# manhofer/Line3Dpp

Measured on AMD Instinct MI355X. Metric: M segment-pair scores/sec, higher is better.
Workload: dtype f64

## Files before the change

line3dpp_amd/csrc/k_affinity.hip:

```cpp
#include "l3d_dev.h"
#include "l3d_kernels.h"

namespace l3d {

namespace {

__device__ __forceinline__ float dist_p2l(const HypRec& s, const double* P) {
    const d3 p1{s.P1[0], s.P1[1], s.P1[2]}, dir{s.dir[0], s.dir[1], s.dir[2]}, p{P[0], P[1], P[2]};
    const d3 v = p - p1;
    const d3 h{p1.x + (((dir.x * v.x) * dir.x + (dir.x * v.y) * dir.y) + (dir.x * v.z) * dir.z),
               p1.y + (((dir.y * v.x) * dir.x + (dir.y * v.y) * dir.y) + (dir.y * v.z) * dir.z),
               p1.z + (((dir.z * v.x) * dir.x + (dir.z * v.y) * dir.y) + (dir.z * v.z) * dir.z)};
    return (float)norm(h - p);
}

__device__ __forceinline__ float expf_ref(float y) { return (float)exp((double)y); }

__device__ __forceinline__ float sim_affinity(const HypRec& h1, const HypRec& h2, float k1, float md1, float k2,
                                              float md2, float med_scene_depth_lines, float two_sigA_sqr) {
    if (h1.length < kEps || h2.length < kEps) return 0.0f;
    const float dot_p = (float)dot(d3{h1.dir[0], h1.dir[1], h1.dir[2]}, d3{h2.dir[0], h2.dir[1], h2.dir[2]});
    float angle = (float)(acos((double)fmaxf(fminf(dot_p, 1.0f), -1.0f)) / M_PI * 180.0f);
    if (angle > 90.0f) angle = 180.0f - angle;
    const float y_a = -angle * angle / two_sigA_sqr;
    float cutoff1 = md1, cutoff2 = md2;
    if (med_scene_depth_lines > kEps) {
        cutoff1 = fminf(cutoff1, med_scene_depth_lines);
        cutoff2 = fminf(cutoff2, med_scene_depth_lines);
    }
    const float d11 = dist_p2l(h2, h1.P1), d12 = dist_p2l(h2, h1.P2);
    const float d21 = dist_p2l(h1, h2.P1), d22 = dist_p2l(h1, h2.P2);
    const float sig11 = (h1.m.dp1 > cutoff1) ? cutoff1 * k1 : h1.m.dp1 * k1;
    const float sig12 = (h1.m.dp2 > cutoff1) ? cutoff1 * k1 : h1.m.dp2 * k1;
    const float reg11 = 2.0f * sig11 * sig11, reg12 = 2.0f * sig12 * sig12;
    const float sig21 = (h2.m.dp1 > cutoff2) ? cutoff2 * k2 : h2.m.dp1 * k2;
    const float sig22 = (h2.m.dp2 > cutoff2) ? cutoff2 * k2 : h2.m.dp2 * k2;
    const float reg21 = 2.0f * sig21 * sig21, reg22 = 2.0f * sig22 * sig22;
    const float y_p1 = fminf(-d11 * d11 / reg11, -d12 * d12 / reg12);
    const float y_p2 = fminf(-d21 * d21 / reg21, -d22 * d22 / reg22);
    return expf_ref(fminf(y_a, fminf(y_p1, y_p2)));
}

}

__global__ void k_aff_sim(uint32_t N, uint32_t lo, uint32_t hi, const uint32_t* __restrict__ surv_sg,
                          const uint32_t* __restrict__ surv_tg,
                          const int32_t* __restrict__ hyp_of_seg, const HypRec* __restrict__ hyps,
                          const ViewAff* __restrict__ va, const float* __restrict__ medians,
                          const float* __restrict__ msdl_ptr, float two_sigA_sqr, float* __restrict__ simv,
                          int32_t* __restrict__ cand_a, int32_t* __restrict__ cand_b) {
    const uint32_t c = blockIdx.x * blockDim.x + threadIdx.x;
    if (c >= N) return;
    const int32_t ha = hyp_of_seg[surv_sg[c]], hb = hyp_of_seg[surv_tg[c]];
    cand_a[c] = ha;
    cand_b[c] = hb;
    if (c < lo || c >= hi) return;
    float sim = 0.0f;
    if (ha >= 0 && hb >= 0) {
        const uint32_t v1 = hyps[ha].view, v2 = hyps[hb].view;
        sim = sim_affinity(hyps[ha], hyps[hb], va[v1].k, medians[v1], va[v2].k, medians[v2], *msdl_ptr, two_sigA_sqr);
    }
    simv[c] = sim;
}

__global__ void k_aff_flag(uint32_t N, const uint32_t* __restrict__ surv_off, const uint32_t* __restrict__ surv_sg,
                           const uint32_t* __restrict__ surv_tg, const float* __restrict__ simv,
                           const int32_t* __restrict__ cand_a, const int32_t* __restrict__ cand_b,
                           uint32_t* __restrict__ flag, uint32_t* __restrict__ first_touch, uint32_t H,
                           uint32_t* __restrict__ touch_flag) {
    const uint32_t c = blockIdx.x * blockDim.x + threadIdx.x;
    if (c < H) first_touch[c] = kEmpty;
    if (c < N) { touch_flag[2 * c] = 0; touch_flag[2 * c + 1] = 0; }
    if (c == 0) touch_flag[2 * (size_t)N] = 0;
    if (c >= N) return;
    uint32_t f = 0;
    if (simv[c] > kMinAffinity) {
        f = 1;
        if (cand_b[c] < cand_a[c]) {
            const uint32_t sg = surv_sg[c], tg = surv_tg[c];
            for (uint32_t i = surv_off[tg]; i < surv_off[tg + 1]; ++i) {
                if (surv_tg[i] == sg) {
                    if (simv[i] > kMinAffinity) f = 0;
                    break;
                }
            }
        }
    }
    flag[c] = f;
}

__global__ void k_fill_u32(uint32_t* p, uint32_t n, uint32_t val) {
    const uint32_t i = blockIdx.x * blockDim.x + threadIdx.x;
    if (i < n) p[i] = val;
}

__global__ void k_aff_touch(uint32_t N, const uint32_t* __restrict__ flag, const uint32_t* __restrict__ epos,
                            const int32_t* __restrict__ cand_a, const int32_t* __restrict__ cand_b,
                            uint32_t* __restrict__ first_touch) {
    const uint32_t c = blockIdx.x * blockDim.x + threadIdx.x;
    if (c >= N || !flag[c]) return;
    const uint32_t k = epos[c];
    atomicMin(&first_touch[cand_a[c]], 2u * k);
    atomicMin(&first_touch[cand_b[c]], 2u * k + 1u);
}

__global__ void k_aff_mark(uint32_t H, const uint32_t* __restrict__ first_touch, uint32_t* __restrict__ touch_flag) {
    const uint32_t h = blockIdx.x * blockDim.x + threadIdx.x;
    if (h >= H) return;
    const uint32_t p = first_touch[h];
    if (p != kEmpty) touch_flag[p] = 1u;
}

struct CLEdgeDev { int32_t i, j; float w; };
struct Seg2D { uint32_t cam, seg; };

__global__ void k_aff_emit(uint32_t N, const uint32_t* __restrict__ flag, const uint32_t* __restrict__ epos,
                           const int32_t* __restrict__ cand_a, const int32_t* __restrict__ cand_b,
                           const float* __restrict__ simv, const uint32_t* __restrict__ first_touch,
                           const uint32_t* __restrict__ touch_rank, const HypRec* __restrict__ hyps,
                           CLEdgeDev* __restrict__ edges, Seg2D* __restrict__ local2global) {
    const uint32_t c = blockIdx.x * blockDim.x + threadIdx.x;
    if (c >= N || !flag[c]) return;
    const uint32_t k = epos[c];
    const int32_t ha = cand_a[c], hb = cand_b[c];
    const uint32_t ta = first_touch[ha], tb = first_touch[hb];
    const int32_t id1 = (int32_t)touch_rank[ta], id2 = (int32_t)touch_rank[tb];
    const float w = simv[c];
    edges[2 * k] = CLEdgeDev{id1, id2, w};
    edges[2 * k + 1] = CLEdgeDev{id2, id1, w};
    if (ta == 2u * k) local2global[id1] = Seg2D{hyps[ha].m.src_cam, hyps[ha].m.src_seg};
    if (tb == 2u * k + 1u) local2global[id2] = Seg2D{hyps[hb].m.src_cam, hyps[hb].m.src_seg};
}

__device__ __forceinline__ float dist_p2l_2d(const d3& line, double px, double py) {
    const float den = sqrtf((float)(line.x * line.x + line.y * line.y));
    return (float)fabs(((line.x * px + line.y * py) + line.z) / (double)den);
}
__device__ __forceinline__ bool on_seg_2d(double p1x, double p1y, double p2x, double p2y, double xx, double xy) {
    return ((p1x - xx) * (p2x - xx) + (p1y - xy) * (p2y - xy)) < kEps;
}
template <int PASS>
__global__ __launch_bounds__(256) void k_collin(const ViewDev* __restrict__ views, const uint32_t* __restrict__ seg_base,
                                                float collin_t, uint32_t* __restrict__ cnt,
                                                const uint32_t* __restrict__ coll_off, uint32_t* __restrict__ coll_idx) {
    __shared__ float4 tile[256];
    const ViewDev& v = views[blockIdx.y];
    const uint32_t M = v.M;
    if (blockIdx.x * blockDim.x >= M) return;
    const uint32_t r = blockIdx.x * blockDim.x + threadIdx.x;
    const bool act = r < M;
    const float4 l1 = act ? v.seg4[r] : make_float4(0, 0, 0, 0);
    const d3 p0{(double)l1.x, (double)l1.y, 1.0}, p1{(double)l1.z, (double)l1.w, 1.0};
    const d3 line1 = cross(p0, p1);
    uint32_t n = 0;
    uint32_t* out = (PASS == 1 && act) ? coll_idx + coll_off[seg_base[blockIdx.y] + r] : nullptr;
    for (uint32_t c0 = 0; c0 < M; c0 += 256) {
        __syncthreads();
        if (c0 + threadIdx.x < M) tile[threadIdx.x] = v.seg4[c0 + threadIdx.x];
        __syncthreads();
        const uint32_t ce = min(256u, M - c0);
        if (!act) continue;
        for (uint32_t k = 0; k < ce; ++k) {
            const uint32_t c = c0 + k;
            if (c == r) continue;
            const float4 l2 = tile[k];
            const d3 q0{(double)l2.x, (double)l2.y, 1.0}, q1{(double)l2.z, (double)l2.w, 1.0};
            if (on_seg_2d(p0.x, p0.y, p1.x, p1.y, q0.x, q0.y) || on_seg_2d(p0.x, p0.y, p1.x, p1.y, q1.x, q1.y) ||
                on_seg_2d(q0.x, q0.y, q1.x, q1.y, p0.x, p0.y) || on_seg_2d(q0.x, q0.y, q1.x, q1.y, p1.x, p1.y))
                continue;
            const d3 line2 = cross(q0, q1);
            const float d1 = fmaxf(dist_p2l_2d(line1, q0.x, q0.y), dist_p2l_2d(line1, q1.x, q1.y));
            const float d2 = fmaxf(dist_p2l_2d(line2, p0.x, p0.y), dist_p2l_2d(line2, p1.x, p1.y));
            if (fmaxf(d1, d2) < collin_t) {
                if (PASS == 1) out[n] = c;
                ++n;
            }
        }
    }
    if (PASS == 0 && act) cnt[seg_base[blockIdx.y] + r] = n;
}

template <int MODE>
__global__ void k_aff_coll_count(uint32_t n_items, const uint32_t* __restrict__ surv_tg, const float* __restrict__ simv,
                                 const HypRec* __restrict__ hyps, const uint32_t* __restrict__ seg_base,
                                 const uint32_t* __restrict__ coll_off, uint32_t* __restrict__ cnt) {
    const uint32_t t = blockIdx.x * blockDim.x + threadIdx.x;
    if (t >= n_items) return;
    uint32_t g;
    if (MODE == 0) { if (!(simv[t] > kMinAffinity)) { cnt[t] = 0; return; } g = surv_tg[t]; }
    else g = seg_base[hyps[t].view] + hyps[t].m.src_seg;
    cnt[t] = coll_off[g + 1] - coll_off[g];
}
template <int MODE>
__global__ void k_aff_coll_sim(uint32_t n_items, const uint32_t* __restrict__ surv_sg, const uint32_t* __restrict__ surv_tg,
                               const int32_t* __restrict__ hyp_of_seg, const HypRec* __restrict__ hyps,
                               const ViewDev* __restrict__ views, const uint32_t* __restrict__ seg_base,
                               const uint32_t* __restrict__ gseg_view, const uint32_t* __restrict__ coll_off,
                               const uint32_t* __restrict__ coll_idx, const uint32_t* __restrict__ item_off,
                               const ViewAff* __restrict__ va, const float* __restrict__ medians,
                               const float* __restrict__ msdl_ptr, float two_sigA_sqr, uint32_t* __restrict__ out_seg,
                               float* __restrict__ out_sim) {
    const uint32_t t = blockIdx.x * blockDim.x + threadIdx.x;
    if (t >= n_items) return;
    const uint32_t ob = item_off[t], on = item_off[t + 1] - ob;
    if (!on) return;
    int32_t ha; uint32_t g;
    if (MODE == 0) { ha = hyp_of_seg[surv_sg[t]]; g = surv_tg[t]; }
    else { ha = (int32_t)t; g = seg_base[hyps[t].view] + hyps[t].m.src_seg; }
    const uint32_t vi = gseg_view[g], base = seg_base[vi], cb = coll_off[g];
    for (uint32_t k = 0; k < on; ++k) {
        const uint32_t x = base + coll_idx[cb + k];
        const int32_t hb = hyp_of_seg[x];
        float sim = 0.0f;
        if (ha >= 0 && hb >= 0) {
            const uint32_t v1 = hyps[ha].view, v2 = hyps[hb].view;
            sim = sim_affinity(hyps[ha], hyps[hb], va[v1].k, medians[v1], va[v2].k, medians[v2], *msdl_ptr, two_sigA_sqr);
        }
        out_seg[ob + k] = x;
        out_sim[ob + k] = sim;
    }
}

static inline dim3 grid1(uint32_t n, uint32_t b = 256) { return dim3((n + b - 1) / b); }

hipError_t launch_aff_sim(uint32_t N, uint32_t lo, uint32_t hi, const uint32_t* surv_sg, const uint32_t* surv_tg, const int32_t* hyp_of_seg,
                          const HypRec* hyps, const ViewAff* va, const float* medians, const float* msdl,
                          float two_sigA_sqr, float* simv, int32_t* ca, int32_t* cb, hipStream_t st) {
    if (!N) return hipSuccess;
    hipLaunchKernelGGL(k_aff_sim, grid1(N, 128), dim3(128), 0, st, N, lo, hi, surv_sg, surv_tg, hyp_of_seg, hyps, va, medians,
                       msdl, two_sigA_sqr, simv, ca, cb);
    return hipGetLastError();
}
hipError_t launch_aff_flag(uint32_t N, const uint32_t* surv_off, const uint32_t* surv_sg, const uint32_t* surv_tg,
                           const float* simv, const int32_t* ca, const int32_t* cb, uint32_t* flag,
                           uint32_t* first_touch, uint32_t H, uint32_t* touch_flag, hipStream_t st) {
    if (!N) return hipSuccess;
    hipLaunchKernelGGL(k_aff_flag, grid1(std::max(N, H)), dim3(256), 0, st, N, surv_off, surv_sg, surv_tg, simv, ca, cb,
                       flag, first_touch, H, touch_flag);
    return hipGetLastError();
}
hipError_t launch_fill_u32(uint32_t* p, uint32_t n, uint32_t val, hipStream_t st) {
    if (!n) return hipSuccess;
    hipLaunchKernelGGL(k_fill_u32, grid1(n), dim3(256), 0, st, p, n, val);
    return hipGetLastError();
}
hipError_t launch_aff_touch(uint32_t N, const uint32_t* flag, const uint32_t* epos, const int32_t* ca,
                            const int32_t* cb, uint32_t* first_touch, hipStream_t st) {
    if (!N) return hipSuccess;
    hipLaunchKernelGGL(k_aff_touch, grid1(N), dim3(256), 0, st, N, flag, epos, ca, cb, first_touch);
    return hipGetLastError();
}
hipError_t launch_aff_mark(uint32_t H, const uint32_t* first_touch, uint32_t* touch_flag, hipStream_t st) {
    if (!H) return hipSuccess;
    hipLaunchKernelGGL(k_aff_mark, grid1(H), dim3(256), 0, st, H, first_touch, touch_flag);
    return hipGetLastError();
}
hipError_t launch_aff_emit(uint32_t N, const uint32_t* flag, const uint32_t* epos, const int32_t* ca,
                           const int32_t* cb, const float* simv, const uint32_t* first_touch,
                           const uint32_t* touch_rank, const HypRec* hyps, void* edges, void* local2global,
                           hipStream_t st) {
    if (!N) return hipSuccess;
    hipLaunchKernelGGL(k_aff_emit, grid1(N), dim3(256), 0, st, N, flag, epos, ca, cb, simv, first_touch, touch_rank,
                       hyps, (CLEdgeDev*)edges, (Seg2D*)local2global);
    return hipGetLastError();
}

}

namespace l3d {
hipError_t launch_collin(int pass, const ViewDev* views, uint32_t n_views, uint32_t max_M, const uint32_t* seg_base,
                         float collin_t, uint32_t* cnt, const uint32_t* coll_off, uint32_t* coll_idx, hipStream_t st) {
    if (!n_views || !max_M) return hipSuccess;
    const dim3 g((max_M + 255) / 256, n_views);
    if (pass == 0) hipLaunchKernelGGL((k_collin<0>), g, dim3(256), 0, st, views, seg_base, collin_t, cnt, coll_off, coll_idx);
    else hipLaunchKernelGGL((k_collin<1>), g, dim3(256), 0, st, views, seg_base, collin_t, cnt, coll_off, coll_idx);
    return hipGetLastError();
}
hipError_t launch_aff_coll_count(int mode, uint32_t n_items, const uint32_t* surv_tg, const float* simv,
                                 const HypRec* hyps, const uint32_t* seg_base, const uint32_t* coll_off, uint32_t* cnt,
                                 hipStream_t st) {
    if (!n_items) return hipSuccess;
    const dim3 g((n_items + 255) / 256);
    if (mode == 0) hipLaunchKernelGGL((k_aff_coll_count<0>), g, dim3(256), 0, st, n_items, surv_tg, simv, hyps, seg_base, coll_off, cnt);
    else hipLaunchKernelGGL((k_aff_coll_count<1>), g, dim3(256), 0, st, n_items, surv_tg, simv, hyps, seg_base, coll_off, cnt);
    return hipGetLastError();
}
hipError_t launch_aff_coll_sim(int mode, uint32_t n_items, const uint32_t* surv_sg, const uint32_t* surv_tg,
                               const int32_t* hyp_of_seg, const HypRec* hyps, const ViewDev* views,
                               const uint32_t* seg_base, const uint32_t* gseg_view, const uint32_t* coll_off,
                               const uint32_t* coll_idx, const uint32_t* item_off, const ViewAff* va,
                               const float* medians, const float* msdl, float two_sigA_sqr, uint32_t* out_seg,
                               float* out_sim, hipStream_t st) {
    if (!n_items) return hipSuccess;
    const dim3 g((n_items + 127) / 128);
    if (mode == 0)
        hipLaunchKernelGGL((k_aff_coll_sim<0>), g, dim3(128), 0, st, n_items, surv_sg, surv_tg, hyp_of_seg, hyps, views,
                           seg_base, gseg_view, coll_off, coll_idx, item_off, va, medians, msdl, two_sigA_sqr, out_seg, out_sim);
    else
        hipLaunchKernelGGL((k_aff_coll_sim<1>), g, dim3(128), 0, st, n_items, surv_sg, surv_tg, hyp_of_seg, hyps, views,
                           seg_base, gseg_view, coll_off, coll_idx, item_off, va, medians, msdl, two_sigA_sqr, out_seg, out_sim);
    return hipGetLastError();
}
}


namespace l3d {
namespace { __global__ void k_warm_affinity() {} }
hipError_t warm_affinity(hipStream_t st) {
    hipLaunchKernelGGL(k_warm_affinity, dim3(1), dim3(64), 0, st);
    return hipGetLastError();
}
}
```

line3dpp_amd/csrc/k_lists.hip:

```cpp
#include <algorithm>
#include <cstdlib>
#include <type_traits>

#include "l3d_dev.h"
#include "l3d_kernels.h"
#include "l3d_lists.h"

constexpr uint32_t kLists4Grid = 512;

namespace l3d {

namespace {

#define L3D_LDS __attribute__((address_space(3)))

__device__ __forceinline__ uint32_t lane_id() { return threadIdx.x & 63u; }

template <int WPL>
__device__ __forceinline__ void group_barrier() {
    if (WPL == 1) {
        __builtin_amdgcn_fence(__ATOMIC_RELEASE, "wavefront");
        __builtin_amdgcn_wave_barrier();
        __builtin_amdgcn_fence(__ATOMIC_ACQUIRE, "wavefront");
    } else {
        __syncthreads();
    }
}

template <int WPL>
__device__ __forceinline__ uint32_t group_scan(uint32_t v, uint32_t& total, uint32_t* red);
template <int WPL>
__device__ __forceinline__ uint32_t group_count(bool f, uint32_t& total, uint32_t* red) {
    if (WPL == 1) {
        const uint64_t m = __builtin_amdgcn_ballot_w64(f);
        total = (uint32_t)__popcll(m);
        return (uint32_t)__popcll(m & ((1ull << lane_id()) - 1ull));
    }
    return group_scan<WPL>(f ? 1u : 0u, total, red);
}

template <int WPL>
__device__ __forceinline__ uint32_t group_scan(uint32_t v, uint32_t& total, uint32_t* red) {
    const uint32_t lane = lane_id();
    uint32_t x = v;
#pragma unroll
    for (int d = 1; d < 64; d <<= 1) { const uint32_t y = __shfl_up(x, d); if (lane >= (uint32_t)d) x += y; }
    if (WPL == 1) {
        total = __shfl(x, 63);
        return x - v;
    }
    const uint32_t wave = threadIdx.x >> 6;
    __syncthreads();
    if (lane == 63) red[wave] = x;
    __syncthreads();
    uint32_t before = 0, tot = 0;
#pragma unroll
    for (uint32_t w = 0; w < (uint32_t)WPL; ++w) { const uint32_t c = red[w]; before += w < wave ? c : 0u; tot += c; }
    total = tot;
    return before + x - v;
}

template <int WPL>
__device__ __forceinline__ uint32_t group_max(uint32_t v, uint32_t* red) {
    uint32_t x = v;
#pragma unroll
    for (int d = 32; d > 0; d >>= 1) x = max(x, (uint32_t)__shfl_xor(x, d));
    if (WPL == 1) return x;
    const uint32_t wave = threadIdx.x >> 6;
    __syncthreads();
    if (lane_id() == 0) red[wave] = x;
    __syncthreads();
    uint32_t m = 0;
#pragma unroll
    for (uint32_t w = 0; w < (uint32_t)WPL; ++w) m = max(m, red[w]);
    return m;
}

__device__ __forceinline__ uint32_t f2ord(float f) {
    const uint32_t u = __float_as_uint(f);
    return (u & 0x80000000u) ? ~u : (u | 0x80000000u);
}
__device__ __forceinline__ float ord2f(uint32_t o) {
    return __uint_as_float((o & 0x80000000u) ? (o & 0x7FFFFFFFu) : ~o);
}

__device__ __forceinline__ bool sim_decide(const d3 dira, bool zeroa, float adp1, float adp2, float reg1, float reg2,
                                           const d3 dirb, bool zerob, float bdp1, float bdp2, const SimConst sc) {
    if (zeroa || zerob) return false;
    const float d1 = adp1 - bdp1, d2 = adp2 - bdp2;
// ... 862 lines not shown
                __hip_atomic_store(&positive[h.ref], (uint8_t)1, __ATOMIC_RELAXED, __HIP_MEMORY_SCOPE_AGENT);
                changed[sweep] = 1;
                break;
            }
        }
    }
}

constexpr uint32_t kMaxReplicas = 16;
__global__ void k_hyp_scores(const ListPools lp, const uint8_t* __restrict__ positive,
                             const uint32_t* __restrict__ gseg_view, Slot* __restrict__ slots,
                             const uint8_t* __restrict__ pair_present, uint32_t* __restrict__ max_score_bits) {
    const uint32_t pool = lp.pool0 + blockIdx.y, k = blockIdx.x * blockDim.x + threadIdx.x;
    const bool active = !(lp.flags[0] | lp.flags[2]) && k < min(lp.cnt[pool * 16 + 1], lp.hcap);
    float score3D = 0.0f;
    uint32_t view = kEmpty;
    if (active) {
        HypHdr& h = lp.hyps[pool * lp.hcap + k];
        const bool inv = (h.pair_flags & kHypInv) != 0;
        const bool exists = !inv || positive[h.ref] != 0;
        float cur = 0.0f;
        uint32_t cur_cam = kEmpty;
        if (exists) {
            const uint32_t n = h.edge_cnt, e0 = h.edge_begin;
            for (uint32_t e = 0; e < n; e += 4) {
                EdgeRec ed[4]; bool ok[4];
#pragma unroll
                for (uint32_t i = 0; i < 4; ++i) ed[i] = lp.edges[e0 + min(e + i, n - 1)];
#pragma unroll
                for (uint32_t i = 0; i < 4; ++i) ok[i] = e + i < n && (!(ed[i].j_cam & kEdgeInv) || positive[ed[i].ref_j] != 0);
#pragma unroll
                for (uint32_t i = 0; i < 4; ++i) {
                    if (!ok[i]) continue;
                    if (ed[i].tv_j == cur_cam) {
                        if (ed[i].sim > cur) { score3D -= cur; score3D += ed[i].sim; cur = ed[i].sim; }
                    } else {
                        score3D += ed[i].sim; cur = ed[i].sim; cur_cam = ed[i].tv_j;
                    }
                }
            }
        }
        h.score3D = score3D;
        h.state = exists ? kHypExists : 0u;
        if (exists && !inv && (!pair_present || pair_present[h.pair_flags & 0x7FFFFFFFu])) slots[h.ref].score3D = score3D;
        view = gseg_view[h.g];
    }
    uint64_t todo = __builtin_amdgcn_ballot_w64(score3D > 0.0f);
    while (todo) {
        const uint32_t leader = (uint32_t)__builtin_ctzll(todo);
        const uint32_t lv = __builtin_amdgcn_readlane(view, leader);
        const bool mine = score3D > 0.0f && view == lv;
        float mx = mine ? score3D : 0.0f;
#pragma unroll
        for (int d = 32; d > 0; d >>= 1) mx = fmaxf(mx, __shfl_xor(mx, d));
        if (lane_id() == leader) {
            uint32_t* p = &max_score_bits[lv * kMaxReplicas + (pool & (kMaxReplicas - 1))];
            if (__float_as_uint(mx) > *(volatile uint32_t*)p) atomicMax(p, __float_as_uint(mx));
        }
        todo &= ~__builtin_amdgcn_ballot_w64(mine);
    }
}

__global__ void k_hyp_filter(const ListPools lp, const uint32_t* __restrict__ gseg_view,
                             const uint32_t* __restrict__ max_score_bits, uint32_t* __restrict__ kept_cnt,
                             unsigned long long* __restrict__ best_pack) {
    const uint32_t pool = lp.pool0 + blockIdx.y, k = blockIdx.x * blockDim.x + threadIdx.x;
    if ((lp.flags[0] | lp.flags[2]) || k >= min(lp.cnt[pool * 16 + 1], lp.hcap)) return;
    HypHdr& h = lp.hyps[pool * lp.hcap + k];
    uint32_t mx = 0;
    {
        const uint32_t* p = max_score_bits + (size_t)gseg_view[h.g] * kMaxReplicas;
#pragma unroll
        for (uint32_t r = 0; r < kMaxReplicas; ++r) mx = max(mx, p[r]);
    }
    const float lim = kMinBestScorePerc * __uint_as_float(mx);
    const float s = h.score3D;
    if ((h.state & kHypExists) && s > 0.0f && s > lim) {
        h.state |= kHypKeep;
        atomicAdd(&kept_cnt[h.g], 1u);
        atomicMax(&best_pack[h.g], ((unsigned long long)__float_as_uint(s) << 32) | (0xFFFFFFFFu - h.canon));
    }
}

__global__ void k_seg_filter(uint32_t g0, uint32_t g1, const uint32_t* __restrict__ kept_cnt,
                             const unsigned long long* __restrict__ best_pack, unsigned long long* __restrict__ cnt64) {
    const uint32_t g = g0 + blockIdx.x * blockDim.x + threadIdx.x;
    if (g >= g1) return;
    const bool ok = __uint_as_float((uint32_t)(best_pack[g] >> 32)) > kMinBestScore3D;
    cnt64[g] = ok ? ((1ull << 32) | kept_cnt[g]) : 0ull;
}

__device__ __forceinline__ void make_match(const ViewDev* views, const PairDesc* pairs, uint32_t view, uint32_t seg,
                                           const HypHdr& h, Match& m, uint32_t& tgt_view, uint32_t& tgt_seg) {
    const bool inv = (h.pair_flags & kHypInv) != 0;
    const PairDesc& pd = pairs[h.pair_flags & 0x7FFFFFFFu];
    tgt_view = inv ? pd.src : pd.tgt;
    tgt_seg = h.tgt_seg;
    m.src_cam = views[view].cam; m.src_seg = seg;
    m.tgt_cam = views[tgt_view].cam; m.tgt_seg = tgt_seg;
    m.overlap = h.overlap; m.score3D = h.score3D;
    m.dp1 = h.dp1; m.dp2 = h.dp2;
    m.dq1 = h.oq1; m.dq2 = h.oq2;
}

__global__ void k_seg_write(uint32_t g0, uint32_t g1, unsigned long long base64, const ViewDev* __restrict__ views, const PairDesc* __restrict__ pairs,
                            const uint32_t* __restrict__ seg_base, const uint32_t* __restrict__ gseg_view,
                            const unsigned long long* __restrict__ off64s, const unsigned long long* __restrict__ best_pack,
                            const uint32_t* __restrict__ seg_of_g, const ListPools lp, const Slot* __restrict__ slots,
                            uint32_t* __restrict__ surv_off, uint32_t* __restrict__ hyp_off, Match* __restrict__ surv,
                            uint32_t* __restrict__ surv_tg, uint32_t* __restrict__ surv_sg,
                            int32_t* __restrict__ hyp_of_seg, HypRec* __restrict__ hyps, float* __restrict__ depths) {
    const uint32_t t = blockIdx.x * blockDim.x + threadIdx.x;
    const bool pass_ok = !(lp.flags[0] | lp.flags[2]);
    if (t <= g1 - g0) {
        const uint32_t gs = g0 + t;
        const unsigned long long o = off64s[gs] + base64;
        surv_off[gs] = (uint32_t)o; hyp_off[gs] = (uint32_t)(o >> 32);
        if (gs < g1) hyp_of_seg[gs] = ((off64s[gs + 1] >> 32) != (off64s[gs] >> 32) && pass_ok) ? (int32_t)(uint32_t)(o >> 32) : -1;
    }
    if (!pass_ok) return;
    const uint32_t pq = t / lp.hcap, k = t - pq * lp.hcap, pool = lp.pool0 + pq;
    if (pq >= lp.npools || k >= min(lp.cnt[pool * 16 + 1], lp.hcap)) return;
    const uint32_t hi = pool * lp.hcap + k;
    const HypHdr& h = lp.hyps[hi];
    if (!(h.state & kHypKeep)) return;
    const uint32_t g = h.g;
    if ((off64s[g + 1] >> 32) == (off64s[g] >> 32)) return;
    const unsigned long long o = off64s[g] + base64;
    const uint32_t view = gseg_view[g], seg = g - seg_base[view];
    const SegHdr sh = lp.segs[seg_of_g[g]];
    uint32_t w = (uint32_t)o;
    for (uint32_t y = sh.hyp_begin; y < hi; ++y) w += (lp.hyps[y].state & kHypKeep) ? 1u : 0u;
    Match m; uint32_t tv, tseg;
    make_match(views, pairs, view, seg, h, m, tv, tseg);
    surv_tg[w] = seg_base[tv] + tseg;
    surv_sg[w] = g;
    surv[w] = m;
    if (h.canon == 0xFFFFFFFFu - (uint32_t)best_pack[g]) {
        const uint32_t hx = (uint32_t)(o >> 32);
        const ViewDev& v = views[view];
        HypRec r;
        const SegX& sx = v.segx[seg];
        const Seg3 s3 = unproject(v.C, sx.r1, sx.r2, h.dp1, h.dp2);
        r.P1[0] = s3.P1.x; r.P1[1] = s3.P1.y; r.P1[2] = s3.P1.z;
        r.P2[0] = s3.P2.x; r.P2[1] = s3.P2.y; r.P2[2] = s3.P2.z;
        r.dir[0] = s3.dir.x; r.dir[1] = s3.dir.y; r.dir[2] = s3.dir.z;
        r.length = s3.length;
        r.valid = s3.length > 0.0f ? 1u : 0u;
        r.m = m;
        r.view = view; r.pad = 0;
        hyps[hx] = r;
        depths[2 * hx] = h.dp1;
        depths[2 * hx + 1] = h.dp2;
    }
}

std::atomic<uint64_t> g_csr_global_launches{0};

hipError_t launch_pair_csr(const PairDesc* pairs, uint32_t n_pairs, uint32_t max_Mt, const PairCsr* pair_poff,
                           const uint32_t* inv_tgt, uint32_t tgt16, uint32_t* poff, uint32_t* refs,
                           uint32_t* dummy, uint32_t tgt_v0, uint32_t tgt_v1, uint64_t max_pair_slots,
                           const uint32_t* row_start, hipStream_t st) {
    if (!n_pairs) return hipSuccess;
    const bool force_global = std::getenv("L3D_CSR_GLOBAL") != nullptr;
    const uint32_t lds_segs = force_global ? 0u : kCsrLdsSegs;
    const size_t lds = ((size_t)std::min(max_Mt, lds_segs) + 64) * 4;
    static const hipError_t attr_rc = [] {
        const int mx = (int)(((size_t)kCsrLdsSegs + 64) * 4);
        hipError_t e = hipFuncSetAttribute((const void*)k_pair_csr<true, true, false>, hipFuncAttributeMaxDynamicSharedMemorySize, mx);
        if (e == hipSuccess) e = hipFuncSetAttribute((const void*)k_pair_csr<true, false, false>, hipFuncAttributeMaxDynamicSharedMemorySize, mx);
        return e;
    }();
    if (attr_rc != hipSuccess) return attr_rc;
    if (tgt16 && !force_global && max_Mt <= lds_segs) {
        const size_t cur_bytes = ((size_t)lds_segs_round(max_Mt) + 64) * 4;
        const size_t two = 78 * 1024, one = 156 * 1024 - 4096;
        const size_t want = (size_t)(0.6 * (double)max_pair_slots) * 4 + 4096;
        const size_t budget = cur_bytes + want <= two ? two : one;
        size_t cap = (budget - cur_bytes) / 4;
        cap = std::min<size_t>(cap, (size_t)std::max<uint64_t>(max_pair_slots, 1024));
        static const hipError_t attr2 = hipFuncSetAttribute((const void*)k_pair_csr<true, true, true>, hipFuncAttributeMaxDynamicSharedMemorySize, 156 * 1024);
        if (attr2 != hipSuccess) return attr2;
        hipLaunchKernelGGL((k_pair_csr<true, true, true>), dim3(n_pairs), dim3(kCsrBlock), cur_bytes + cap * 4, st, pairs, 0u, pair_poff, inv_tgt,
                           poff, refs, dummy, tgt_v0, tgt_v1, lds_segs, (uint32_t)cap, row_start);
        return hipGetLastError();
    }
#define L3D_CSR(T16)                                                                                                      \
    do {                                                                                                                  \
        hipLaunchKernelGGL((k_pair_csr<true, T16, false>), dim3(n_pairs), dim3(kCsrBlock), lds, st, pairs, 0u, pair_poff, inv_tgt, \
                           poff, refs, dummy, tgt_v0, tgt_v1, lds_segs, 0u, row_start);                                   \
        if (max_Mt > lds_segs) {  \
            hipLaunchKernelGGL((k_pair_csr<false, T16, false>), dim3(n_pairs), dim3(kCsrBlock), 0, st, pairs, 0u, pair_poff, inv_tgt, \
                               poff, refs, dummy, tgt_v0, tgt_v1, lds_segs, 0u, row_start);                               \
            g_csr_global_launches.fetch_add(1, std::memory_order_relaxed);                                                \
        }                                                                                                                 \
    } while (0)
    if (tgt16) L3D_CSR(true); else L3D_CSR(false);
// ... 4 lines not shown
__global__ void k_publish_flags(const ListPools lp) {
    if (threadIdx.x < 4) lp.cnt[lp.pool0 * 16 + 8 + threadIdx.x] = lp.flags[threadIdx.x];
    if (threadIdx.x == 4) lp.cnt[lp.pool0 * 16 + 12] = lp.flags[6];
}

__global__ void k_merge_flags(const ListPools lp, uint32_t world) {
    const uint32_t ppr = kListPools / world;
    uint32_t f0 = 0, f2 = 0;
    for (uint32_t r = 0; r < world; ++r) { f0 |= lp.cnt[(size_t)r * ppr * 16 + 8]; f2 |= lp.cnt[(size_t)r * ppr * 16 + 10]; }
    if (f0) lp.flags[0] = 1;
    if (f2) lp.flags[2] = 1;
}

__global__ void k_seg_index(const ListPools lp, uint32_t* __restrict__ seg_of_g) {
    if (lp.flags[0] | lp.flags[2]) return;
    const uint32_t pool = lp.pool0 + blockIdx.y, k = blockIdx.x * blockDim.x + threadIdx.x;
    if (k >= min(lp.cnt[pool * 16 + 2], lp.scap)) return;
    seg_of_g[lp.segs[pool * lp.scap + k].g] = pool * lp.scap + k;
}
hipError_t launch_seg_index(ListPools lp, uint32_t* seg_of_g, uint32_t G, uint32_t world, hipStream_t st) {
    hipLaunchKernelGGL(k_merge_flags, dim3(1), dim3(1), 0, st, lp, world ? world : 1u);
    hipLaunchKernelGGL(k_seg_index, dim3((lp.scap + 255) / 256, lp.npools), dim3(256), 0, st, lp, seg_of_g);
    return hipGetLastError();
}

constexpr uint32_t kLists2Grid = 16384;
hipError_t launch_lists(uint32_t v0, uint32_t nv, uint32_t max_M, const ViewDev* views, const PairDesc* pairs,
                        const ListView* lviews, const OutPair* opairs, const InPair* ipairs, const uint32_t* gseg_view,
                        const uint32_t* poff, const uint32_t* inv, const float2* hyp_p, const float2* hyp_q, const Slot* slots, uint32_t uniform_K,
                        SimConst sc, ListPools lp, uint32_t* seg_of_g, HugeScratchArgs hsa, hipStream_t st) {
    if (!nv || !max_M) return hipSuccess;
    const bool wide = hsa.mean_list > 96;
#define L3D_LISTS(B)                                                                                                       \
    do {                                                                                                                   \
        const size_t lds1 = ListCfg<1, B>::BYTES, lds2 = ListCfg<2, B>::BYTES, lds4 = ListCfg<4, B>::BYTES;                \
        hipError_t e = hipFuncSetAttribute((const void*)k_lists<1, B>, hipFuncAttributeMaxDynamicSharedMemorySize, (int)lds1); \
        if (e != hipSuccess) return e;                                                                                     \
        e = hipFuncSetAttribute((const void*)k_lists<2, B>, hipFuncAttributeMaxDynamicSharedMemorySize, (int)lds2);        \
        if (e != hipSuccess) return e;                                                                                     \
        e = hipFuncSetAttribute((const void*)k_lists<4, B>, hipFuncAttributeMaxDynamicSharedMemorySize, (int)lds4);        \
        if (e != hipSuccess) return e;                                                                                     \
        for (uint32_t a = 0; a < nv; a += 65535u) {                                                      \
            const uint32_t n = nv - a < 65535u ? nv - a : 65535u;                                                          \
            hipLaunchKernelGGL((k_lists<1, B>), dim3(max_M, n), dim3(64), lds1, st, views, pairs, lviews, opairs, ipairs,  \
                               gseg_view, poff, inv, hyp_p, hyp_q, uniform_K, lp, v0 + a);                                        \
        }                                                                                                                  \
           \
        hipLaunchKernelGGL((k_lists<2, B>), dim3(kLists2Grid), dim3(128), lds2, st, views, pairs, lviews, opairs, ipairs, \
                           gseg_view, poff, inv, hyp_p, hyp_q, uniform_K, lp, 0u);                                                \
            \
            \
        if (hsa.run_tier4)                                                                                                 \
        hipLaunchKernelGGL((k_lists<4, B>), dim3(kLists4Grid), dim3(256), lds4, st, views, pairs, lviews, opairs, ipairs, \
                           gseg_view, poff, inv, hyp_p, hyp_q, uniform_K, lp, 0u);                                                \
    } while (0)
    if (wide) L3D_LISTS(256); else L3D_LISTS(128);
#undef L3D_LISTS
    HugeScratch hs;
    hs.d1 = hsa.f32; hs.d2 = hsa.f32 + hsa.cap;
    hs.tv = hsa.u32; hs.ref = hsa.u32 + hsa.cap; hs.pf = hsa.u32 + 2 * (size_t)hsa.cap;
    hs.key = hsa.u64; hs.cap = hsa.cap;
    if (hsa.run_huge)
        hipLaunchKernelGGL(k_lists_huge, dim3(256), dim3(256), 0, st, views, pairs, lviews, opairs, ipairs, gseg_view, poff,
                           inv, hyp_p, hyp_q, lp, hs);
    hipLaunchKernelGGL(k_cand_exact, dim3((lp.ccap + 255) / 256, lp.npools), dim3(256), 0, st, views, pairs, gseg_view, sc, lp);
    hipLaunchKernelGGL(k_edges, dim3((lp.scap + kEdgesSplit - 1) / kEdgesSplit, lp.npools), dim3(64), 0, st, views, pairs,
                       gseg_view, slots, lp, seg_of_g);
    if (lp.npools < kListPools) hipLaunchKernelGGL(k_publish_flags, dim3(1), dim3(64), 0, st, lp);
    return hipGetLastError();
}

static dim3 hyp_grid(const ListPools& lp) { return dim3((lp.hcap + 255) / 256, lp.npools); }

hipError_t launch_chain_sweep(ListPools lp, uint8_t* positive, uint32_t* changed, uint32_t sweep, uint32_t* undecided, hipStream_t st) {
    if (sweep == 0) hipLaunchKernelGGL(k_chain_sweep, hyp_grid(lp), dim3(256), 0, st, lp, positive, changed, undecided);
    else hipLaunchKernelGGL(k_chain_sweep_list, dim3(kChainListBlocks, lp.npools), dim3(256), 0, st, lp, positive, changed, sweep, undecided);
    return hipGetLastError();
}
hipError_t launch_hyp_scores(ListPools lp, const uint8_t* positive, const uint32_t* gseg_view, Slot* slots,
                             const uint8_t* pair_present, uint32_t* max_score_bits, hipStream_t st) {
    hipLaunchKernelGGL(k_hyp_scores, hyp_grid(lp), dim3(256), 0, st, lp, positive, gseg_view, slots, pair_present, max_score_bits);
    return hipGetLastError();
}
hipError_t launch_hyp_filter(ListPools lp, uint32_t g0, uint32_t g1, const uint32_t* gseg_view, const uint32_t* max_score_bits,
                             uint32_t* kept_cnt, unsigned long long* best_pack, unsigned long long* cnt64,
                             hipStream_t st) {
    hipLaunchKernelGGL(k_hyp_filter, hyp_grid(lp), dim3(256), 0, st, lp, gseg_view, max_score_bits, kept_cnt, best_pack);
    if (g1 > g0) hipLaunchKernelGGL(k_seg_filter, dim3((g1 - g0 + 255) / 256), dim3(256), 0, st, g0, g1, kept_cnt, best_pack, cnt64);
    return hipGetLastError();
}
hipError_t launch_seg_write(uint32_t g0, uint32_t g1, unsigned long long base64, const ViewDev* views, const PairDesc* pairs, const uint32_t* seg_base,
                            const uint32_t* gseg_view, const unsigned long long* off64s,
                            const unsigned long long* best_pack, const uint32_t* seg_of_g, ListPools lp,
                            const Slot* slots, uint32_t* surv_off, uint32_t* hyp_off, Match* surv, uint32_t* surv_tg,
                            uint32_t* surv_sg, int32_t* hyp_of_seg, HypRec* hyps, float* depths, hipStream_t st) {
    const uint64_t n_thr = std::max<uint64_t>((uint64_t)(g1 - g0) + 1, (uint64_t)lp.npools * lp.hcap);
    hipLaunchKernelGGL(k_seg_write, dim3((uint32_t)((n_thr + 255) / 256)), dim3(256), 0, st, g0, g1, base64, views, pairs, seg_base, gseg_view,
                       off64s, best_pack, seg_of_g, lp, slots, surv_off, hyp_off, surv, surv_tg, surv_sg, hyp_of_seg,
                       hyps, depths);
    return hipGetLastError();
}

}


namespace l3d {
namespace { __global__ void k_warm_lists() {} }
hipError_t warm_lists(hipStream_t st) {
    hipLaunchKernelGGL(k_warm_lists, dim3(1), dim3(64), 0, st);
    return hipGetLastError();
}
}
```

line3dpp_amd/csrc/k_scan.hip:

```cpp
#include "l3d_dev.h"
#include "l3d_kernels.h"

namespace l3d {

namespace {

constexpr uint32_t kScanBlock = 1024, kScanItems = 4, kScanTile = kScanBlock * kScanItems;
constexpr unsigned long long kAgg = 1ull << 32, kIncl = 2ull << 32;

template <class T>
__device__ __forceinline__ T block_exclusive_scan(T v, T* wsum , T& block_total) {
    const uint32_t tid = threadIdx.x, lane = tid & 63u, wave = tid >> 6;
    T x = v;
#pragma unroll
    for (int d = 1; d < 64; d <<= 1) {
        const T y = __shfl_up(x, d);
        if (lane >= (uint32_t)d) x += y;
    }
    if (lane == 63) wsum[wave] = x;
    __syncthreads();
    if (tid == 0) {
        T acc = 0;
        for (uint32_t w = 0; w < kScanBlock / 64; ++w) { const T t = wsum[w]; wsum[w] = acc; acc += t; }
        wsum[16] = acc;
    }
    __syncthreads();
    block_total = wsum[16];
    return wsum[wave] + x - v;
}

__device__ __forceinline__ uint32_t wave_sum(uint32_t v) {
#pragma unroll
    for (int d = 32; d > 0; d >>= 1) v += __shfl_xor(v, d);
    return v;
}

template <class T>
__global__ __launch_bounds__(kScanBlock) void k_scan(const T* __restrict__ in, uint32_t n, T* __restrict__ out,
                                                     T* __restrict__ total_out, unsigned long long* __restrict__ ws) {
    constexpr uint32_t LANES = sizeof(T) / 4;
    __shared__ T wsum[17];
    __shared__ T s_prefix;
    __shared__ uint32_t s_last, s_tile;
    const uint32_t nb = gridDim.x, tid = threadIdx.x, lane = tid & 63u;
    if (tid == 0) s_tile = (uint32_t)__hip_atomic_fetch_add(&ws[1], 1ull, __ATOMIC_RELAXED, __HIP_MEMORY_SCOPE_AGENT);
    __syncthreads();
    const uint32_t tile = s_tile;
    const uint32_t base = tile * kScanTile + tid * kScanItems;
    T a[kScanItems];
    T v = 0;
#pragma unroll
    for (uint32_t k = 0; k < kScanItems; ++k) { a[k] = (base + k < n) ? in[base + k] : (T)0; v += a[k]; }
    T agg;
    T ex = block_exclusive_scan(v, wsum, agg);
    unsigned long long* state = ws + 2;
    if (tid < 64) {
        if (lane < LANES)
            __hip_atomic_store(&state[(size_t)tile * LANES + lane],
                               (tile == 0 ? kIncl : kAgg) | (uint32_t)((unsigned long long)agg >> (32 * lane)),
                               __ATOMIC_RELAXED, __HIP_MEMORY_SCOPE_AGENT);
        unsigned long long prefix = 0;
        if (tile > 0) {
#pragma unroll
            for (uint32_t l = 0; l < LANES; ++l) {
                uint32_t acc = 0;
                for (int idx = (int)tile - 1;; idx -= 64) {
                    const int t = idx - (int)lane;
                    unsigned long long s = kIncl;
                    if (t >= 0) {
                        do s = __hip_atomic_load(&state[(size_t)t * LANES + l], __ATOMIC_RELAXED, __HIP_MEMORY_SCOPE_AGENT);
                        while ((s >> 32) == 0);
                    }
                    const uint64_t incl = __builtin_amdgcn_ballot_w64((s >> 32) == 2);
                    if (incl) {
                        const uint32_t first = (uint32_t)__builtin_ctzll(incl);
                        acc += wave_sum(lane <= first ? (uint32_t)s : 0u);
                        break;
                    }
                    acc += wave_sum((uint32_t)s);
                }
                prefix |= (unsigned long long)acc << (32 * l);
            }
            if (lane < LANES)
                __hip_atomic_store(&state[(size_t)tile * LANES + lane],
                                   kIncl | (uint32_t)((prefix + (unsigned long long)agg) >> (32 * lane)),
                                   __ATOMIC_RELAXED, __HIP_MEMORY_SCOPE_AGENT);
        }
        if (lane == 0) s_prefix = (T)prefix;
    }
    __syncthreads();
    ex += s_prefix;
#pragma unroll
    for (uint32_t k = 0; k < kScanItems; ++k) {
        if (base + k < n) out[base + k] = ex;
        ex += a[k];
    }
    if (tile == nb - 1 && tid == 0) {
        const T total = s_prefix + agg;
        out[n] = total;
        if (total_out) *total_out = total;
    }
    __syncthreads();
    if (tid == 0) s_last = __hip_atomic_fetch_add(&ws[0], 1ull, __ATOMIC_ACQ_REL, __HIP_MEMORY_SCOPE_AGENT) == nb - 1;
    __syncthreads();
    if (s_last) {
        for (uint32_t i = tid; i < nb * LANES; i += kScanBlock)
            __hip_atomic_store(&state[i], 0ull, __ATOMIC_RELAXED, __HIP_MEMORY_SCOPE_AGENT);
        if (tid == 0) {
            __hip_atomic_store(&ws[0], 0ull, __ATOMIC_RELAXED, __HIP_MEMORY_SCOPE_AGENT);
            __hip_atomic_store(&ws[1], 0ull, __ATOMIC_RELAXED, __HIP_MEMORY_SCOPE_AGENT);
        }
    }
}

template <class T>
hipError_t launch(const T* in, uint32_t n, T* out, unsigned long long* ws, T* total, hipStream_t st) {
    const uint32_t nb = std::max(1u, (n + kScanTile - 1) / kScanTile);
    hipLaunchKernelGGL((k_scan<T>), dim3(nb), dim3(kScanBlock), 0, st, in, n, out, total, ws);
    return hipGetLastError();
}

}

size_t scan_ws_words(size_t n, uint32_t bytes_per_element) { return 4 + (n / kScanTile + 1) * (bytes_per_element / 4); }

hipError_t launch_scan(const uint32_t* in, uint32_t n, uint32_t* out, unsigned long long* ws, uint32_t* total, hipStream_t st) {
    return launch<uint32_t>(in, n, out, ws, total, st);
}
hipError_t launch_scan64(const unsigned long long* in, uint32_t n, unsigned long long* out, unsigned long long* ws,
                         unsigned long long* total, hipStream_t st) {
    return launch<unsigned long long>(in, n, out, ws, total, st);
}

}


namespace l3d {
namespace { __global__ void k_warm_scan() {} }
hipError_t warm_scan(hipStream_t st) {
    hipLaunchKernelGGL(k_warm_scan, dim3(1), dim3(64), 0, st);
    return hipGetLastError();
}
}
```

line3dpp_amd/csrc/l3d_access.hip:

```cpp
#include "l3d_ctx.h"
#include "l3d_lsd.h"

using namespace l3d;

extern "C" {

int l3d_synchronize(l3d_ctx* c) {
    if (!c) return fail(L3D_ERR_ARG, "null argument");
    L3D_HIP_CHECK(hipStreamSynchronize(c->stream));
    return L3D_OK;
}

int l3d_pair_tests(l3d_ctx* c, uint64_t* n) {
    if (!c || !n) return fail(L3D_ERR_ARG, "null argument");
    *n = c->pair_tests;
    return L3D_OK;
}

static int fetch_host_offsets(l3d_ctx* c) {
    if (c->host_offsets_valid) return L3D_OK;
    c->h_surv_off.assign((size_t)c->G + 1, 0);
    c->h_hyp_off.assign((size_t)c->G + 1, 0);
    L3D_HIP_CHECK(hipStreamSynchronize(c->stream));
    L3D_HIP_CHECK(hipMemcpy(c->h_surv_off.data(), c->d_surv_off.p, ((size_t)c->G + 1) * 4, hipMemcpyDeviceToHost));
// ... 52 lines not shown

int l3d_num_best(l3d_ctx* c, uint32_t* n) {
    if (!c || !n) return fail(L3D_ERR_ARG, "null argument");
    *n = c->state == l3d_ctx::MATCHED ? c->n_hyps : 0;
    return L3D_OK;
}

int l3d_get_best(l3d_ctx* c, l3d_segment2d* seg2d, l3d_segment3d* seg3d, l3d_match* best) {
    if (!c) return fail(L3D_ERR_ARG, "null argument");
    if (c->state != l3d_ctx::MATCHED) return fail(L3D_ERR_STATE, "no matches yet");
    (void)hipSetDevice(c->device);
    std::vector<HypRec> h(c->n_hyps);
    if (c->n_hyps) L3D_HIP_CHECK(hipMemcpy(h.data(), c->d_hyps.p, h.size() * sizeof(HypRec), hipMemcpyDeviceToHost));
    for (size_t i = 0; i < h.size(); ++i) {
        if (seg2d) { seg2d[i].camID_ = h[i].m.src_cam; seg2d[i].segID_ = h[i].m.src_seg; }
        if (seg3d) {
            std::memcpy(seg3d[i].P1, h[i].P1, 24); std::memcpy(seg3d[i].P2, h[i].P2, 24);
            std::memcpy(seg3d[i].dir, h[i].dir, 24);
            seg3d[i].length_ = h[i].length; seg3d[i].valid_ = h[i].valid;
        }
        if (best) std::memcpy(&best[i], &h[i].m, sizeof(l3d_match));
    }
    return L3D_OK;
}

int l3d_view_info(l3d_ctx* c, uint32_t camID, float* k, float* median_depth) {
    if (!c) return fail(L3D_ERR_ARG, "null argument");
    auto f = c->views.find(camID);
    if (f == c->views.end()) return fail(L3D_ERR_ARG, "unknown camera ID");
    if (k) *k = f->second->k;
    if (median_depth) *median_depth = f->second->median_depth;
    return L3D_OK;
}

int l3d_translation(l3d_ctx* c, double t[3]) {
    if (!c || !t) return fail(L3D_ERR_ARG, "null argument");
    t[0] = c->translation.x; t[1] = c->translation.y; t[2] = c->translation.z;
    return L3D_OK;
}

int l3d_num_affinity(l3d_ctx* c, uint32_t* n_edges, uint32_t* n_rows) {
    if (!c) return fail(L3D_ERR_ARG, "null argument");
    if (!c->affinity_done) return fail(L3D_ERR_STATE, "l3d_compute_affinity has not run");
    if (n_edges) *n_edges = c->aff_n_edges;
    if (n_rows) *n_rows = c->aff_n_rows;
    return L3D_OK;
}

int l3d_get_affinity(l3d_ctx* c, l3d_cledge* edges, l3d_segment2d* l2g, float* msdl) {
    if (!c) return fail(L3D_ERR_ARG, "null argument");
    if (!c->affinity_done) return fail(L3D_ERR_STATE, "l3d_compute_affinity has not run");
    { std::lock_guard<std::recursive_mutex> lk(c->mu); const int rc = ensure_affinity_host(c); if (rc) return rc; }
    if (edges && !c->edges.empty()) std::memcpy(edges, c->edges.data(), c->edges.size() * sizeof(l3d_cledge));
    if (l2g && !c->l2g.empty()) std::memcpy(l2g, c->l2g.data(), c->l2g.size() * sizeof(l3d_segment2d));
    if (msdl) *msdl = c->med_scene_depth_lines;
    return L3D_OK;
}

int l3d_get_sparse_matrix(l3d_ctx* c, int sort_by_row, l3d_float4* entries, int32_t* start_indices) {
    if (!c) return fail(L3D_ERR_ARG, "null argument");
    if (!c->affinity_done) return fail(L3D_ERR_STATE, "l3d_compute_affinity has not run");
    { std::lock_guard<std::recursive_mutex> lk(c->mu); const int rc = ensure_affinity_host(c); if (rc) return rc; }
    std::vector<l3d_cledge> e = c->edges;
    if (sort_by_row)
        std::stable_sort(e.begin(), e.end(), [](const l3d_cledge& a, const l3d_cledge& b) {
            return a.i_ < b.i_ || (a.i_ == b.i_ && a.j_ < b.j_); });
    else
        std::stable_sort(e.begin(), e.end(), [](const l3d_cledge& a, const l3d_cledge& b) {
            return a.j_ < b.j_ || (a.j_ == b.j_ && a.i_ < b.i_); });
    if (start_indices) for (size_t i = 0; i < c->l2g.size(); ++i) start_indices[i] = -1;
    int cur = -1;
    for (size_t pos = 0; pos < e.size(); ++pos) {
        if (entries) entries[pos] = l3d_float4{(float)e[pos].i_, (float)e[pos].j_, e[pos].w_, 0.0f};
        const int rc = sort_by_row ? e[pos].i_ : e[pos].j_;
        if (rc != cur) { if (start_indices) start_indices[rc] = (int)pos; cur = rc; }
    }
    return L3D_OK;
}

unsigned long long l3d_debug_counter(const char* name) {
    if (name && std::string(name) == "csr_global_launches") return g_csr_global_launches.load(std::memory_order_relaxed);
    if (name && std::string(name) == "knn_replay_calls") return g_knn_replay_calls.load(std::memory_order_relaxed);
    if (name && std::string(name) == "keep_all_repeats") return g_keep_all_repeats.load(std::memory_order_relaxed);
    if (name && std::string(name) == "lsd_images_detected") return g_lsd_images_detected.load(std::memory_order_relaxed);
    if (name && std::string(name) == "lsd_cache_loads") return g_lsd_cache_loads.load(std::memory_order_relaxed);
    return ~0ull;
}

int l3d_set_timing_level(l3d_ctx* c, int level) {
    if (!c || level < 0 || level > 2) return fail(L3D_ERR_ARG, "l3d_set_timing_level: level 0, 1 or 2");
    std::lock_guard<std::recursive_mutex> lk(c->mu);
    c->timing_level = level;
    return L3D_OK;
}

int l3d_get_timings(l3d_ctx* c, l3d_timings* t) {
    if (!c || !t) return fail(L3D_ERR_ARG, "null argument");
    *t = c->tm;
    return L3D_OK;
}

}
```

line3dpp_amd/csrc/l3d_affinity_host.hip:

```cpp
#include "l3d_ctx.h"

namespace l3d {

static int affinity_collinear(l3d_ctx* c) {
    hipStream_t st = c->stream;
    const uint32_t V = (uint32_t)c->order.size(), G = c->G, N = c->n_surv, H = c->n_hyps;
    uint32_t max_M = 0;
    for (auto* v : c->order) max_M = std::max(max_M, v->M);
    L3D_HIP_CHECK(c->d_coll_cnt.reserve(G + 1)); L3D_HIP_CHECK(c->d_coll_off.reserve(G + 1));
    L3D_HIP_CHECK(launch_collin(0, c->d_views.p, V, max_M, c->d_seg_base.p, c->collinearity_t, c->d_coll_cnt.p, nullptr,
                                nullptr, st));
    L3D_HIP_CHECK(launch_scan(c->d_coll_cnt.p, G, c->d_coll_off.p, c->d_scan_ws.p, c->d_scal.p + 9, st));
    uint32_t n_coll = 0;
    L3D_HIP_CHECK(hipStreamSynchronize(st));
    L3D_HIP_CHECK(hipMemcpy(&n_coll, c->d_scal.p + 9, 4, hipMemcpyDeviceToHost));
    L3D_HIP_CHECK(c->d_coll_idx.reserve(std::max<uint32_t>(n_coll, 1)));
    L3D_HIP_CHECK(launch_collin(1, c->d_views.p, V, max_M, c->d_seg_base.p, c->collinearity_t, nullptr, c->d_coll_off.p,
                                c->d_coll_idx.p, st));
    std::vector<uint32_t> off[2], seg[2];
    std::vector<float> sim[2];
    const uint32_t n_items[2] = {N, H};
    for (int mode = 0; mode < 2; ++mode) {
        const uint32_t n = n_items[mode];
        L3D_HIP_CHECK(c->d_item_cnt.reserve(n + 1)); L3D_HIP_CHECK(c->d_item_off.reserve(n + 1));
// ... 30 lines not shown
    for (uint32_t g = 0; g < G; ++g) if (hyp_of_seg[g] >= 0) seg_of_hyp[(uint32_t)hyp_of_seg[g]] = g;
    std::unordered_set<uint64_t> used;
    std::vector<int32_t> local_id(G, -1);
    std::vector<uint32_t> row_seg;
    auto unused = [&](uint32_t a, uint32_t b) {
        const uint64_t key = a < b ? ((uint64_t)a << 32) | b : ((uint64_t)b << 32) | a;
        return used.insert(key).second;
    };
    auto get_id = [&](uint32_t g) {
        if (local_id[g] < 0) { local_id[g] = (int32_t)row_seg.size(); row_seg.push_back(g); }
        return local_id[g];
    };
    c->edges.clear();
    auto push = [&](int32_t i, int32_t j, float w) {
        c->edges.push_back(l3d_cledge{i, j, w}); c->edges.push_back(l3d_cledge{j, i, w});
    };
    for (uint32_t h = 0; h < H; ++h) {
        const uint32_t a = seg_of_hyp[h];
        if (a == kEmpty) continue;
        int32_t id1 = -1;
        bool found_aff = false;
        for (uint32_t p = surv_off[a]; p < surv_off[a + 1]; ++p) {
            const uint32_t b = surv_tg[p];
            if (simv[p] > kMinAffinity && unused(a, b)) {
                if (id1 < 0) id1 = get_id(a);
                const int32_t id2 = get_id(b);
                push(id1, id2, simv[p]);
                found_aff = true;
                for (uint32_t k = off[0][p]; k < off[0][p + 1]; ++k)
                    if (sim[0][k] > kMinAffinity && unused(a, seg[0][k])) push(id1, get_id(seg[0][k]), sim[0][k]);
            }
        }
        if (found_aff && id1 >= 0)
            for (uint32_t k = off[1][h]; k < off[1][h + 1]; ++k)
                if (sim[1][k] > kMinAffinity && unused(a, seg[1][k])) push(id1, get_id(seg[1][k]), sim[1][k]);
    }
    c->l2g.resize(row_seg.size());
    for (size_t r = 0; r < row_seg.size(); ++r) {
        const uint32_t g = row_seg[r];
        const uint32_t vi = (uint32_t)(std::upper_bound(c->seg_base.begin(), c->seg_base.end(), g) - c->seg_base.begin()) - 1;
        c->l2g[r].camID_ = c->order[vi]->cam; c->l2g[r].segID_ = g - c->seg_base[vi];
    }
    c->aff_n_edges = (uint32_t)c->edges.size(); c->aff_n_rows = (uint32_t)c->l2g.size(); c->aff_host_valid = true;
    L3D_HIP_CHECK(c->d_edges.reserve(std::max<size_t>(c->edges.size(), 1)));
    if (!c->edges.empty())
        L3D_HIP_CHECK(hipMemcpyAsync(c->d_edges.p, c->edges.data(), c->edges.size() * sizeof(l3d_cledge),
                                     hipMemcpyHostToDevice, st));
    return L3D_OK;
}

static int affinity_prepare(l3d_ctx* c) {
    (void)hipSetDevice(c->device);
    hipStream_t st = c->stream;
    const uint32_t V = (uint32_t)c->order.size();
    c->edges.clear(); c->l2g.clear();
    c->aff_n_edges = 0; c->aff_n_rows = 0; c->aff_host_valid = true;
    std::vector<float> sd;
    for (auto* v : c->order) if (v->median_depth > kEps) sd.push_back(v->median_depth);
    if (!sd.empty()) { std::sort(sd.begin(), sd.end()); c->med_scene_depth_lines = sd[sd.size() / 2]; }
    else c->med_scene_depth_lines = 0.0f;
    std::vector<ViewAff> va(V + 1);
    for (uint32_t vi = 0; vi < V; ++vi) { va[vi].k = c->order[vi]->k; va[vi].pad = 0; }
    va[V].k = c->med_scene_depth_lines; va[V].pad = 0;
    const uint32_t N = c->n_surv, H = c->n_hyps;
    L3D_HIP_CHECK(c->d_scal.reserve(16));
    L3D_HIP_CHECK(c->d_scan_ws.reserve_zeroed(scan_ws_words((size_t)c->G + 2 * (size_t)N, 4), st));
    if (c->ev_on(6)) L3D_HIP_CHECK(hipEventRecord(c->ev[6], st));
    if (N > 0 && H > 0) {
        L3D_HIP_CHECK(c->d_vaff.reserve(V + 1));
        L3D_HIP_CHECK(c->d_simv.reserve(N)); L3D_HIP_CHECK(c->d_ca.reserve(N)); L3D_HIP_CHECK(c->d_cb.reserve(N));
        L3D_HIP_CHECK(c->d_flag.reserve(N + 1)); L3D_HIP_CHECK(c->d_epos.reserve(N + 1));
        L3D_HIP_CHECK(c->d_first_touch.reserve(H));
        L3D_HIP_CHECK(c->d_scan_ws.reserve_zeroed(scan_ws_words(2 * (size_t)N, 4), st));
        L3D_HIP_CHECK(upload_table(c->d_vaff, c->h_vaff, va.data(), ((size_t)V + 1) * sizeof(ViewAff), c->up_vaff, st));
    }
    return L3D_OK;
}

static int affinity_sim(l3d_ctx* c, uint32_t lo, uint32_t hi) {
    const uint32_t V = (uint32_t)c->order.size(), N = c->n_surv, H = c->n_hyps;
    if (!(N > 0 && H > 0)) return L3D_OK;
    L3D_HIP_CHECK(launch_aff_sim(N, lo, hi, c->d_surv_sg.p, c->d_surv_tg.p, c->d_hyp_of_seg.p, c->d_hyps.p, c->d_vaff.p,
                                 (c->d_med + 8), (const float*)(c->d_vaff.p + V), c->two_sigA_sqr, c->d_simv.p, c->d_ca.p, c->d_cb.p,
                                 c->stream));
    return L3D_OK;
}

static int affinity_rest(l3d_ctx* c) {
    hipStream_t st = c->stream;
    const uint32_t N = c->n_surv, H = c->n_hyps;
    bool counts_pending = false;
    if (N > 0 && H > 0) {
        if (c->collinearity_t > (float)kEps) {
            const int rc = affinity_collinear(c);
            if (rc) return rc;
            if (c->ev_on(7)) L3D_HIP_CHECK(hipEventRecord(c->ev[7], st));
            L3D_HIP_CHECK(hipStreamSynchronize(st));
            c->tm.affinity_ms = ev_ms(c, 6, 7);
            c->affinity_done = true;
            return L3D_OK;
        }
        L3D_HIP_CHECK(c->d_touch_flag.reserve(2 * (size_t)N + 1));
        L3D_HIP_CHECK(launch_aff_flag(N, c->d_surv_off.p, c->d_surv_sg.p, c->d_surv_tg.p, c->d_simv.p, c->d_ca.p,
                                      c->d_cb.p, c->d_flag.p, c->d_first_touch.p, H, c->d_touch_flag.p, st));
        L3D_HIP_CHECK(launch_scan(c->d_flag.p, N, c->d_epos.p, c->d_scan_ws.p, c->d_scal.p + 3, st));
        {
            L3D_HIP_CHECK(c->d_touch_flag.reserve(2 * (size_t)N + 1));
            L3D_HIP_CHECK(c->d_touch_rank.reserve(2 * (size_t)N + 1));
            L3D_HIP_CHECK(c->d_edges.reserve(2 * (size_t)N));
            L3D_HIP_CHECK(c->d_l2g.reserve(H));
            L3D_HIP_CHECK(launch_aff_touch(N, c->d_flag.p, c->d_epos.p, c->d_ca.p, c->d_cb.p, c->d_first_touch.p, st));
            L3D_HIP_CHECK(launch_aff_mark(H, c->d_first_touch.p, c->d_touch_flag.p, st));
            L3D_HIP_CHECK(launch_scan(c->d_touch_flag.p, 2 * N, c->d_touch_rank.p, c->d_scan_ws.p, c->d_scal.p + 4, st));
            L3D_HIP_CHECK(launch_aff_emit(N, c->d_flag.p, c->d_epos.p, c->d_ca.p, c->d_cb.p, c->d_simv.p,
                                          c->d_first_touch.p, c->d_touch_rank.p, c->d_hyps.p, c->d_edges.p,
                                          c->d_l2g.p, st));
            L3D_HIP_CHECK(c->h_cnt.reserve(16));
            L3D_HIP_CHECK(hipMemcpyAsync(c->h_cnt.p + 12, c->d_scal.p + 3, 8, hipMemcpyDeviceToHost, st));
            counts_pending = true;
        }
    }
    if (c->ev_on(7)) L3D_HIP_CHECK(hipEventRecord(c->ev[7], st));
    L3D_HIP_CHECK(hipStreamSynchronize(st));
    if (counts_pending) { c->aff_n_edges = 2 * c->h_cnt.p[12]; c->aff_n_rows = c->h_cnt.p[13]; c->aff_host_valid = false; }
    c->tm.affinity_ms = ev_ms(c, 6, 7);
    c->affinity_done = true;
    return L3D_OK;
}

int affinity_core(l3d_ctx* c) {
    int rc = affinity_prepare(c);
    if (rc == L3D_OK) rc = affinity_sim(c, 0u, c->n_surv);
    if (rc == L3D_OK) rc = affinity_rest(c);
    return rc;
}

int ensure_affinity_host(l3d_ctx* c) {
    if (c->aff_host_valid) return L3D_OK;
    (void)hipSetDevice(c->device);
    c->edges.resize(c->aff_n_edges);
    c->l2g.resize(c->aff_n_rows);
    L3D_HIP_CHECK(hipStreamSynchronize(c->stream));
    if (c->aff_n_edges)
        L3D_HIP_CHECK(hipMemcpy(c->edges.data(), c->d_edges.p, (size_t)c->aff_n_edges * sizeof(l3d_cledge), hipMemcpyDeviceToHost));
    if (c->aff_n_rows)
        L3D_HIP_CHECK(hipMemcpy(c->l2g.data(), c->d_l2g.p, (size_t)c->aff_n_rows * sizeof(l3d_segment2d), hipMemcpyDeviceToHost));
    c->aff_host_valid = true;
    return L3D_OK;
}

}

using namespace l3d;

extern "C" {

int l3d_compute_affinity(l3d_ctx* c) {
    if (!c) return fail(L3D_ERR_ARG, "null argument");
    std::lock_guard<std::recursive_mutex> lk(c->mu);
    if (c->state != l3d_ctx::MATCHED) return fail(L3D_ERR_STATE, "matchImages must precede the affinity step");
    if (c->aff_shard_open) return fail(L3D_ERR_STATE, "a sharded affinity fill is open: l3d_affinity_shard_finish (or _abort) first");
    translate(*c);
    const int rc = affinity_core(c);
    untranslate(*c);
    return rc;
}

int l3d_affinity_shard_begin(l3d_ctx* c, uint32_t rank, uint32_t world, void** simv, uint64_t* first, uint64_t* count) {
    if (!c || !simv || !first || !count) return fail(L3D_ERR_ARG, "null argument");
    std::lock_guard<std::recursive_mutex> lk(c->mu);
    if (c->state != l3d_ctx::MATCHED) return fail(L3D_ERR_STATE, "matchImages must precede the affinity step");
    if (c->aff_shard_open) return fail(L3D_ERR_STATE, "l3d_affinity_shard_begin: a sharded affinity fill is already open (views translated)");
    if (world < 2 || rank >= world || c->aff_parts_world != world || c->tail_base_n.size() != (size_t)world + 1 ||
        c->tail_base_n[world] != c->n_surv)
        return fail(L3D_ERR_STATE, "l3d_affinity_shard_begin follows a call closed by l3d_tail_shard_commit with the same world size");
    if (c->collinearity_t > (float)kEps)
        return fail(L3D_ERR_LIMIT, "the links to collinear segments are sequential by definition (line3D.cc:1904-1974): use l3d_compute_affinity");
    translate(*c);
    int rc = affinity_prepare(c);
    if (rc == L3D_OK) rc = affinity_sim(c, c->tail_base_n[rank], c->tail_base_n[rank + 1]);
    if (rc == L3D_OK && !c->exch_ordered && hipStreamSynchronize(c->stream) != hipSuccess) rc = fail(L3D_ERR_HIP, "l3d_affinity_shard_begin: stream synchronisation failed");
    if (rc != L3D_OK) { untranslate(*c); return rc; }
    *simv = c->d_simv.p;
    for (uint32_t r = 0; r < world; ++r) { first[r] = c->tail_base_n[r]; count[r] = c->tail_base_n[r + 1] - c->tail_base_n[r]; }
    c->aff_shard_open = true;
    return L3D_OK;
}

int l3d_affinity_shard_finish(l3d_ctx* c) {
    if (!c) return fail(L3D_ERR_ARG, "null argument");
    std::lock_guard<std::recursive_mutex> lk(c->mu);
    if (c->state != l3d_ctx::MATCHED || !c->aff_shard_open)
        return fail(L3D_ERR_STATE, "l3d_affinity_shard_finish follows l3d_affinity_shard_begin and the exchange of the similarities");
    c->aff_shard_open = false;
    const int rc = affinity_rest(c);
    untranslate(*c);
    return rc;
}

int l3d_affinity_shard_abort(l3d_ctx* c) {
    if (!c) return fail(L3D_ERR_ARG, "null argument");
    std::lock_guard<std::recursive_mutex> lk(c->mu);
    if (!c->aff_shard_open) return L3D_OK;
// ... 67 lines not shown
```

line3dpp_amd/csrc/l3d_api.hip:

```cpp
#include <thread>

#include "l3d_ctx.h"

namespace l3d {

static thread_local std::string g_err;
void set_error(const std::string& s) { g_err = s; }
const char* last_error_cstr() { return g_err.c_str(); }

int fail(int code, const std::string& msg) { set_error(msg); return code; }

void init_view(HostView& v, const double K[9], const double R[9], const double t[3]) {
    std::memcpy(v.K.m, K, 72);
    std::memcpy(v.R.m, R, 72);
    v.t = d3{t[0], t[1], t[2]};
    v.pp = d3{v.K.m[2], v.K.m[5], 1.0};
    v.Kinv = m3_inv(v.K);
    v.Rt = m3_t(v.R);
    v.RtKinv = m3_mul(v.Rt, v.Kinv);
    v.C = mul33(v.Rt.m, d3{-1.0 * v.t.x, -1.0 * v.t.y, -1.0 * v.t.z});
}

void translate_view(HostView& v, const d3& d) {
    v.C = v.C + d;
// ... 170 lines not shown
struct CachedBlock { void* p; size_t bytes; int device; bool pinned; };
std::mutex g_cache_mu;
std::vector<CachedBlock> g_cache;
size_t g_cache_bytes[2] = {0, 0};
constexpr size_t kCacheMaxBlocks = 512;
constexpr size_t kCacheMaxPinned = (size_t)1 << 30;
thread_local int g_release_synced = 0;
size_t cache_max_device_bytes() {
    static const size_t cap = [] {
        if (const char* e = std::getenv("L3D_CACHE_MAX_MB")) return (size_t)std::strtoull(e, nullptr, 10) << 20;
        size_t fr = 0, tot = 0;
        if (hipMemGetInfo(&fr, &tot) != hipSuccess || !tot) { (void)hipGetLastError(); return (size_t)16 << 30; }
        return tot / 4;
    }();
    return cap;
}
}
ReleaseSynced::ReleaseSynced() { ++g_release_synced; }
ReleaseSynced::~ReleaseSynced() { --g_release_synced; }
void* block_cache_take(bool pinned, size_t bytes, size_t* got_bytes) {
    if (!bytes) return nullptr;
    int dev = 0;
    (void)hipGetDevice(&dev);
    std::lock_guard<std::mutex> lk(g_cache_mu);
    size_t best = g_cache.size();
    for (size_t i = 0; i < g_cache.size(); ++i) {
        const CachedBlock& b = g_cache[i];
        if (b.pinned != pinned || (!pinned && b.device != dev) || b.bytes < bytes || b.bytes > 2 * bytes + (64u << 10)) continue;
        if (best == g_cache.size() || b.bytes < g_cache[best].bytes) best = i;
    }
    if (best == g_cache.size()) return nullptr;
    const CachedBlock b = g_cache[best];
    g_cache[best] = g_cache.back(); g_cache.pop_back();
    g_cache_bytes[pinned] -= b.bytes;
    *got_bytes = b.bytes;
    return b.p;
}
bool block_cache_give(bool pinned, void* p, size_t bytes) {
    static const bool off = std::getenv("L3D_NO_BLOCK_CACHE") != nullptr;
    if (off || !p || !bytes) return false;
    int dev = 0;
    (void)hipGetDevice(&dev);
    const size_t cap = pinned ? kCacheMaxPinned : cache_max_device_bytes();
    {
        std::lock_guard<std::mutex> lk(g_cache_mu);
        if (g_cache.size() >= kCacheMaxBlocks || g_cache_bytes[pinned] + bytes > cap) return false;
    }
    if (!g_release_synced && hipDeviceSynchronize() != hipSuccess) { (void)hipGetLastError(); return false; }
    std::lock_guard<std::mutex> lk(g_cache_mu);
    if (g_cache.size() >= kCacheMaxBlocks || g_cache_bytes[pinned] + bytes > cap) return false;
    g_cache.push_back(CachedBlock{p, bytes, dev, pinned});
    g_cache_bytes[pinned] += bytes;
    return true;
}
size_t block_cache_trim(int kind) {
    std::vector<CachedBlock> out;
    {
        std::lock_guard<std::mutex> lk(g_cache_mu);
        for (size_t i = 0; i < g_cache.size();) {
            if (kind < 0 || (int)g_cache[i].pinned == kind) {
                out.push_back(g_cache[i]); g_cache_bytes[g_cache[i].pinned] -= g_cache[i].bytes;
                g_cache[i] = g_cache.back(); g_cache.pop_back();
            } else ++i;
        }
    }
    size_t freed = 0;
    int cur = 0;
    (void)hipGetDevice(&cur);
    for (const CachedBlock& b : out) {
        if (b.pinned) (void)hipHostFree(b.p);
        else { (void)hipSetDevice(b.device); (void)hipFree(b.p); }
        freed += b.bytes;
    }
    if (!out.empty()) (void)hipSetDevice(cur);
    return freed;
}

float ev_ms(hipEvent_t a, hipEvent_t b) {
    float ms = 0;
    (void)hipEventElapsedTime(&ms, a, b);
    return ms;
}
std::atomic<uint64_t> g_keep_all_repeats{0};
std::atomic<uint64_t> g_knn_replay_calls{0};

float ev_ms(const ::l3d_ctx* c, int a, int b) { return c->ev_on(a) && c->ev_on(b) ? ev_ms(c->ev[a], c->ev[b]) : 0.0f; }

}

using namespace l3d;

extern "C" {

const char* l3d_last_error(void) { return g_err.c_str(); }
#ifndef L3D_BUILD_ID
#define L3D_BUILD_ID "unknown"
#endif
const char* l3d_build_info(void) { return "libl3dpp_hip gfx950 hip fp-contract=off build=" L3D_BUILD_ID; }

uint64_t l3d_trim_cache(void) { return (uint64_t)block_cache_trim(-1); }

l3d_ctx* l3d_create(int device, void* stream) {
    if (hipSetDevice(device) != hipSuccess) { set_error("hipSetDevice failed: no usable HIP device"); return nullptr; }
    auto* c = new l3d_ctx();
    c->device = device;
    c->stream = (hipStream_t)stream;
    orientation_thresholds(c->orient_lo, c->orient_hi);
    c->use_cull = std::getenv("L3D_NO_CULL") == nullptr;
    for (auto& e : c->ev)
        if (hipEventCreate(&e) != hipSuccess) { set_error("hipEventCreate failed"); delete c; return nullptr; }
    static std::mutex warm_mu;
    static std::set<int> warmed;
    bool need_warm = !std::getenv("L3D_NO_WARMUP");
    if (need_warm) { std::lock_guard<std::mutex> lk(warm_mu); need_warm = warmed.count(device) == 0; }
    if (need_warm) {
        hipStream_t st = c->stream;
        DevBuf<uint32_t> d; PinnedBuf<uint32_t> h;
        constexpr size_t kWarmWords = (1u << 20) / 4;
        bool ok = d.reserve(kWarmWords) == hipSuccess && h.reserve(kWarmWords) == hipSuccess;
        ok = ok && hipMemsetAsync(d.p, 0, kWarmWords * 4, st) == hipSuccess;
        const size_t sizes[] = {64, 1024, 4096, 16384, 65536, 262144, (size_t)1 << 20};
        for (size_t bytes : sizes) {
            ok = ok && hipMemcpyAsync(d.p, h.p, bytes, hipMemcpyHostToDevice, st) == hipSuccess && hipStreamSynchronize(st) == hipSuccess;
            ok = ok && hipMemcpyAsync(h.p, d.p, bytes, hipMemcpyDeviceToHost, st) == hipSuccess && hipStreamSynchronize(st) == hipSuccess;
        }
        for (int rep = 0; rep < 2; ++rep)
            for (size_t bytes : sizes) {
                ok = ok && hipMemsetAsync(d.p, 0, kWarmWords * 4, st) == hipSuccess;
                ok = ok && hipMemcpyAsync(h.p, d.p, bytes, hipMemcpyDeviceToHost, st) == hipSuccess;
                ok = ok && hipMemsetAsync(d.p, 0, kWarmWords * 4, st) == hipSuccess;
                ok = ok && hipMemcpyAsync(d.p, h.p, bytes, hipMemcpyHostToDevice, st) == hipSuccess;
            }
        ok = ok && warm_match(st) == hipSuccess && warm_lists(st) == hipSuccess && warm_scan(st) == hipSuccess &&
             warm_views(st) == hipSuccess && warm_affinity(st) == hipSuccess && warm_rdd(st) == hipSuccess;
        const bool drained_ok = hipStreamSynchronize(st) == hipSuccess;
        ok = ok && drained_ok;
        { const ReleaseSynced drained; d.release(); h.release(); }
        if (!ok) { set_error("start-up launches failed: no usable HIP device"); l3d_destroy(c); return nullptr; }
        { std::lock_guard<std::mutex> lk(warm_mu); warmed.insert(device); }
    }
    return c;
}

void l3d_destroy(l3d_ctx* c) {
    if (!c) return;
    (void)hipSetDevice(c->device);
    (void)hipStreamSynchronize(c->stream);
    const ReleaseSynced drained;
    for (auto& kv : c->views) {
        HostView& v = *kv.second;
        v.d_seg4.release(); v.d_segf.release();
    }
    c->d_views.release(); c->d_pairs.release(); c->d_work.release(); c->d_slots.release(); c->d_slot_idx.release();
    c->h_views.release(); c->h_pairs.release(); c->h_cull.release(); c->h_work.release();
    c->h_segb.release(); c->h_cnt.release(); c->h_fin.release();
    c->d_poff.release(); c->d_csr_dummy.release(); c->d_pair_present.release(); c->d_cnt64.release(); c->d_off64s.release(); c->d_scan_ws.release();
    c->d_huge_u64.release(); c->d_inv_refs.release(); c->d_lzero.release(); c->d_list2.release(); c->d_list4.release(); c->d_listH.release();
    c->d_seg_of_g.release(); c->d_huge_u32.release(); c->d_huge_f32.release(); c->d_ledges.release(); c->d_lhyps.release();
    c->d_lsegs.release(); c->d_lcands.release(); c->d_lchdrs.release(); c->d_ltab.release(); c->h_ltab.release();
    c->d_cull.release(); c->d_src_perm.release(); c->d_tgt_perm.release(); c->d_src_band.release();
    c->d_chunk_band.release(); c->d_cull_keys.release(); c->d_tgt_sf.release(); c->d_tgt_band.release(); c->d_tgt_s4.release(); c->d_tgt_sd.release();
    c->d_row_counts.release(); c->d_keep_rec.release(); c->d_row_start.release(); c->d_slot_row.release(); c->d_keep_info.release(); c->d_row_pair.release(); c->d_blk_row.release(); c->h_keep_info.release();
    c->d_seg_base.release(); c->d_gseg_view.release();
    c->d_scal.release();
    c->d_surv_off.release(); c->d_hyp_off.release();
    c->d_surv_tg.release(); c->d_surv_sg.release();
    c->d_inv_tgt.release(); c->d_hyp_p.release(); c->d_hyp_q.release(); c->d_gsegx.release(); c->d_gsegd32.release();
    c->d_tie_count.release(); c->d_tie_list.release(); c->d_tie_heap.release(); c->d_item_bucket.release(); c->d_item_order.release(); c->d_order_done.release();
    c->d_coll_cnt.release(); c->d_coll_off.release(); c->d_coll_idx.release(); c->d_item_cnt.release();
    c->d_item_off.release(); c->d_item_seg.release(); c->d_item_sim.release();
    c->d_surv.release();
    c->d_hyp_of_seg.release(); c->d_depths.release(); c->d_med = nullptr; c->d_hyps.release();
    c->d_vaff.release(); c->d_simv.release(); c->h_vaff.release(); c->d_ca.release(); c->d_cb.release();
    c->d_flag.release(); c->d_epos.release(); c->d_first_touch.release(); c->d_touch_flag.release();
    c->d_touch_rank.release(); c->d_edges.release(); c->d_l2g.release();
    c->d_lopt.release(); c->h_lopt.release();
    for (auto& e : c->ev) if (e) (void)hipEventDestroy(e);
    for (auto& e : c->lo_ev) if (e) (void)hipEventDestroy(e);
    delete c;
}

int l3d_slots_exchanged(l3d_ctx* c) {
    if (!c) return fail(L3D_ERR_ARG, "null argument");
    if (c->state != l3d_ctx::BEGUN) return fail(L3D_ERR_STATE, "l3d_match_begin must precede l3d_slots_exchanged");
    std::fill(c->pair_done.begin(), c->pair_done.end(), 1);
    return L3D_OK;
}

int l3d_set_brute_force(l3d_ctx* c, int on) {
    if (!c) return L3D_ERR_ARG;
    c->brute = on != 0;
    return L3D_OK;
}

static int add_view(l3d_ctx* c, uint32_t camID, const float* segs4, uint32_t M, const double K[9], const double R[9],
                    const double t[3], uint32_t width, uint32_t height, float median_depth, const uint32_t* neighbors,
                    uint32_t n_neighbors, bool by_worldpoints);

int l3d_add_view(l3d_ctx* c, uint32_t camID, const float* segs4, uint32_t M, const double K[9], const double R[9],
                 const double t[3], uint32_t width, uint32_t height, float median_depth, const uint32_t* neighbors,
                 uint32_t n_neighbors) {
    return add_view(c, camID, segs4, M, K, R, t, width, height, median_depth, neighbors, n_neighbors, false);
}
int l3d_add_view_worldpoints(l3d_ctx* c, uint32_t camID, const float* segs4, uint32_t M, const double K[9],
                             const double R[9], const double t[3], uint32_t width, uint32_t height, float median_depth,
                             const uint32_t* worldpoints, uint32_t n_worldpoints) {
    return add_view(c, camID, segs4, M, K, R, t, width, height, median_depth, worldpoints, n_worldpoints, true);
}
int l3d_get_visual_neighbors(l3d_ctx* c, uint32_t camID, uint32_t* out, uint32_t cap, uint32_t* n) {
    if (!c || !n) return fail(L3D_ERR_ARG, "null argument");
    std::lock_guard<std::recursive_mutex> lk(c->mu);
    auto it = c->views.find(camID);
    if (it == c->views.end()) return fail(L3D_ERR_ARG, "unknown camera ID");
    *n = (uint32_t)it->second->visual_nbrs.size();
    uint32_t i = 0;
    if (out) for (uint32_t o : it->second->visual_nbrs) { if (i < cap) out[i] = o; ++i; }
    return L3D_OK;
}

static int add_view(l3d_ctx* c, uint32_t camID, const float* segs4, uint32_t M, const double K[9], const double R[9],
                    const double t[3], uint32_t width, uint32_t height, float median_depth, const uint32_t* neighbors,
                    uint32_t n_neighbors, bool by_worldpoints) {
    if (!c || !K || !R || !t) return fail(L3D_ERR_ARG, "null argument");
    std::lock_guard<std::recursive_mutex> lk(c->mu);
    if (std::max(width, height) < 800) return fail(L3D_ERR_IMAGE_SMALL, "image is too small for reliable results");
    if (c->views.count(camID)) return fail(L3D_ERR_ID_IN_USE, "camera ID already in use");
    if (n_neighbors == 0 || !neighbors)
        return fail(L3D_ERR_NO_NEIGHBORS, by_worldpoints ? "view has no worldpoints" : "view has no visual neighbors");
    if (M == 0 || !segs4) return fail(L3D_ERR_NO_SEGMENTS, "no line segments");
    if (M >= (1u << 23)) return fail(L3D_ERR_LIMIT, "more than 2^23 segments per view");
    (void)hipSetDevice(c->device);
    auto v = std::make_unique<HostView>();
    v->cam = camID; v->M = M;
    v->segs.assign(segs4, segs4 + 4 * (size_t)M);
    for (float x : v->segs) v->coord_max = std::isfinite(x) ? std::fmax(v->coord_max, (double)std::fabs(x)) : INFINITY;
    v->width = width; v->height = height;
    v->initial_median_depth = (float)std::fmax(std::fabs(median_depth), kEps);
    init_view(*v, K, R, t);
    if (by_worldpoints) { v->by_worldpoints = true; v->worldpoints.assign(neighbors, neighbors + n_neighbors); }
    else v->fixed_nbrs.assign(neighbors, neighbors + n_neighbors);
    L3D_HIP_CHECK(v->d_seg4.reserve(M));
    L3D_HIP_CHECK(v->d_segf.reserve(M));
    L3D_HIP_CHECK(hipMemcpy(v->d_seg4.p, v->segs.data(), (size_t)M * 16, hipMemcpyHostToDevice));
    c->views_avg_depths.push_back((float)std::fmax(median_depth, kEps));
    c->views[camID] = std::move(v);
    c->order.clear();
    for (auto& kv : c->views) { kv.second->index = (uint32_t)c->order.size(); c->order.push_back(kv.second.get()); }
    c->state = l3d_ctx::IDLE;
    c->affinity_done = false;
    return L3D_OK;
}

void abort_match(l3d_ctx* c) {
    (void)hipStreamSynchronize(c->stream);
    untranslate(*c);
    c->timing_pending = false; c->pending_launches = 0;
    c->state = l3d_ctx::IDLE;
// ... 232 lines not shown
    }
    L3D_HIP_CHECK(c->d_tgt_band.reserve(std::max<uint64_t>(ct_off, 1)));
    L3D_HIP_CHECK(c->d_chunk_band.reserve(std::max<uint32_t>(cc_off, 1)));
    L3D_HIP_CHECK(c->d_cull_keys.reserve(std::max<uint64_t>(ck_off, 1)));
    if (c->ev_on(1)) L3D_HIP_CHECK(hipEventRecord(c->ev[1], c->stream));
    g_trace.mark("begin: tables uploaded, pools reserved");
    c->tm = l3d_timings{};
    c->state = l3d_ctx::BEGUN;
    return L3D_OK;
}

int l3d_num_pairs(l3d_ctx* c, uint32_t* n) {
    if (!c || !n) return fail(L3D_ERR_ARG, "null argument");
    *n = (uint32_t)c->pairs.size();
    return L3D_OK;
}

int l3d_get_pairs(l3d_ctx* c, uint32_t* s, uint32_t* t, uint64_t* off) {
    if (!c) return fail(L3D_ERR_ARG, "null argument");
    for (size_t i = 0; i < c->pairs.size(); ++i) {
        if (s) s[i] = c->pair_src_cam[i];
        if (t) t[i] = c->pair_tgt_cam[i];
        if (off) off[i] = c->pairs[i].slot_off;
    }
    return L3D_OK;
}

void collect_match_timing(l3d_ctx* c) {
    if (!c->timing_pending) return;
    c->tm.match_kernel_ms += ev_ms(c, 4, 5);
    c->tm.cull_prepare_ms += ev_ms(c, 8, 4);
    c->tm.match_kernel_launches += c->pending_launches;
    c->timing_pending = false; c->pending_launches = 0;
}

static int run_match_kernel(l3d_ctx* c, int mode, uint32_t first, uint32_t count) {
    size_t n_work = 0;
    uint32_t maxK = 0, maxM = 0, maxMt = 0;
    const bool hot = mode == 0 && !c->brute && !c->knn_replay;
    const uint32_t tile = hot ? c->tile_rows : 0u;
    const uint32_t layout = hot ? c->layout_rows : 0u;
    const uint32_t rows_per_item = layout ? layout : (uint32_t)kMatchRows;
    auto items_of = [&](uint32_t Ms) { return layout ? tile_src_cap(Ms, layout) / layout : (Ms + kMatchRows - 1) / kMatchRows; };
    for (uint32_t p = first; p < first + count; ++p) n_work += items_of(c->pairs[p].Ms);
    if (!n_work) return L3D_OK;
    for (uint32_t p = first; p < first + count; ++p) {
        const PairDesc& pd = c->pairs[p];
        maxK = std::max(maxK, pd.K);
        if (c->cull[p].enabled) maxM = std::max(maxM, std::max(pd.Ms, pd.Mt));
        maxMt = std::max(maxMt, pd.Mt);
    }
    const bool replay_all = mode == 0 && c->knn_replay;
    if (!replay_all && match_lds_bytes(mode, maxK, false, match_waves_per_group(mode, c->brute, (uint32_t)n_work), c->brute, tile,
                                       match_row_cache(mode, c->brute, (uint32_t)n_work, tile)) > 160 * 1024)
        return fail(L3D_ERR_LIMIT, "kNN too large for the LDS top-K table");
    L3D_HIP_CHECK(c->d_work.reserve(n_work));
    if (!(c->work_key.version == c->pairs_version && c->work_key.first == first && c->work_key.count == count &&
          c->work_key.dev == (const void*)c->d_work.p && c->work_key.rows == rows_per_item && c->work_key.items == n_work)) {
        L3D_HIP_CHECK(c->h_work.reserve(n_work));
        WorkItem* work = c->h_work.p;
        size_t w = 0;
        for (uint32_t p = first; p < first + count; ++p)
            for (uint32_t k = 0, n = items_of(c->pairs[p].Ms); k < n; ++k) work[w++] = WorkItem{p, k * rows_per_item};
        L3D_HIP_CHECK(hipMemcpyAsync(c->d_work.p, work, n_work * sizeof(WorkItem), hipMemcpyHostToDevice, c->stream));
        c->work_key.version = c->pairs_version; c->work_key.first = first; c->work_key.count = count;
        c->work_key.dev = c->d_work.p; c->work_key.rows = rows_per_item; c->work_key.items = n_work;
    }
    if (c->ev_on(8)) L3D_HIP_CHECK(hipEventRecord(c->ev[8], c->stream));
    CullPools pools{c->d_cull.p, c->d_src_perm.p, c->d_src_band.p, c->d_tgt_perm.p, c->d_tgt_sf.p, c->d_tgt_band.p,
                    c->d_chunk_band.p, c->d_cull_keys.p};
    pools.tgt_s4 = c->d_tgt_s4.p; pools.tgt_sd = c->d_tgt_sd.p; pools.padded_rows = layout;
    const bool keep_all_unculled = std::getenv("L3D_KEEPALL_NO_CULL") != nullptr;
    if (c->brute || !maxM || mode == 2 || (mode == 1 && keep_all_unculled)) pools.cull = nullptr;
    else {
        if (!tile && !replay_all && n_work > kMatchOrderMinItems && n_work <= kMatchOrderMaxItems) {
            L3D_HIP_CHECK(c->d_item_bucket.reserve(n_work)); L3D_HIP_CHECK(c->d_item_order.reserve(n_work));
            if (!c->d_order_done.p) {
                L3D_HIP_CHECK(c->d_order_done.reserve(1));
                L3D_HIP_CHECK(hipMemsetAsync(c->d_order_done.p, 0, 4, c->stream));
            }
            pools.item_bucket = c->d_item_bucket.p; pools.item_order = c->d_item_order.p;
            pools.order_done = c->d_order_done.p;
            pools.w_base = c->cull[first].w_item0; pools.cost_max = maxMt;
        }
        L3D_HIP_CHECK(launch_cull_prepare(c->d_views.p, c->d_pairs.p, first, count, maxM, pools, layout, c->stream));
        L3D_HIP_CHECK(launch_order_items(c->d_pairs.p, first, count, maxMt, pools, (uint32_t)n_work, c->stream));
    }
    if (c->ev_on(4)) L3D_HIP_CHECK(hipEventRecord(c->ev[4], c->stream));
    const bool ix16 = maxMt < 65536u && maxK < 32768u;
    OrientFuse of{mode == 0 ? c->d_inv_tgt.p : nullptr, c->tgt16, OrientThr{c->orient_lo, c->orient_hi}, nullptr, nullptr, 0u, nullptr, nullptr,
                  mode == 0 ? c->d_hyp_p.p : nullptr, mode == 0 ? c->d_hyp_q.p : nullptr};
    if (mode == 1 && c->ragged) { of.keep_rec = c->d_keep_rec.p; of.keep_cap = c->keep_cap; }
    uint32_t tie_stride = 0;
    if (mode == 0) {
        uint32_t mt = 0;
        for (auto& pd : c->pairs) mt = std::max(mt, pd.Mt);
        tie_stride = std::max(mt, 1u);
        if (!c->d_tie_count.p) {
            L3D_HIP_CHECK(c->d_tie_count.reserve(4));
            L3D_HIP_CHECK(hipMemsetAsync(c->d_tie_count.p, 0, 16, c->stream));
        }
        L3D_HIP_CHECK(c->d_tie_list.reserve(std::max<uint32_t>(c->n_rows_total, 1)));
        L3D_HIP_CHECK(c->d_tie_heap.reserve(2 * (size_t)match_tied_grid(tie_stride) * tie_stride));
        of.tie_count = c->d_tie_count.p + (c->tie_seq & 1u); of.tie_next = c->d_tie_count.p + ((c->tie_seq + 1) & 1u);
        of.tie_total = c->d_tie_count.p + 2; ++c->tie_seq;
        of.tie_list = c->d_tie_list.p; of.tie_cap = c->n_rows_total;
    }
    if (replay_all) {
        uint32_t maxMs = 0;
        for (uint32_t p = first; p < first + count; ++p) maxMs = std::max(maxMs, c->pairs[p].Ms);
        L3D_HIP_CHECK(launch_queue_all_rows(c->d_pairs.p, first, count, maxMs, c->pairs[first].row_off, of, c->stream));
    } else
    L3D_HIP_CHECK(launch_match_pairs(mode, c->brute, c->d_views.p, c->d_pairs.p, c->d_work.p, (uint32_t)n_work, maxK,
                                     c->d_slots.p, c->d_row_counts.p, c->epipolar_overlap, pools, of, ix16, tile, c->stream));
    if (c->ev_on(5)) L3D_HIP_CHECK(hipEventRecord(c->ev[5], c->stream));
    if (mode == 0) {
        L3D_HIP_CHECK(launch_match_tied_rows(c->d_views.p, c->d_pairs.p, c->d_slots.p, maxK, c->epipolar_overlap, of, pools,
                                             c->d_tie_heap.p, tie_stride, c->stream));
        for (uint32_t p = first; p < first + count; ++p) c->pair_counted[p] = 1;
    }
    if (pools.cull)
        for (uint32_t p = first; p < first + count; ++p) c->tm.culled_pairs += c->cull[p].enabled;
    c->timing_pending = true; c->pending_launches += 1;
    return L3D_OK;
}

static int match_pairs_impl(l3d_ctx* c, uint32_t first, uint32_t count, bool sync);

static constexpr int kKeepAllTwoPass = -1000;
static constexpr uint64_t kKeepScratchMax = 48ull << 30;
static int keep_all_single_pass(l3d_ctx* c, uint32_t first, uint32_t count) {
    const uint32_t P = (uint32_t)c->pairs.size(), R = c->n_rows_total;
    if (!P || !R) return kKeepAllTwoPass;
    hipStream_t st = c->stream;
    if (!c->keep_cap) {
        const char* e = std::getenv("L3D_KEEPALL_CAP");
        c->keep_cap = e && std::atoi(e) > 0 ? (uint32_t)std::atoi(e) : 96u;
    }
    L3D_HIP_CHECK(c->d_row_start.reserve((size_t)R + 3));
    L3D_HIP_CHECK(c->d_keep_info.reserve(P)); L3D_HIP_CHECK(c->d_row_pair.reserve(R)); L3D_HIP_CHECK(c->h_keep_info.reserve(P));
    L3D_HIP_CHECK(c->d_scan_ws.reserve_zeroed(scan_ws_words((size_t)R + 1, 4), st));
    const uint4* info = c->h_keep_info.p;
    c->ragged = true;
    auto outputs = [&](uint64_t ns) -> hipError_t {
        hipError_t e = c->d_slots.reserve(ns);
        if (e == hipSuccess) e = c->d_slot_row.reserve(ns);
        if (e == hipSuccess) e = c->d_inv_tgt.reserve(ns);
        if (e == hipSuccess) e = c->d_hyp_p.reserve(ns);
        if (e == hipSuccess) e = c->d_hyp_q.reserve(ns);
        return e;
    };
    auto assemble = [&](uint64_t cap) -> hipError_t {
        OrientFuse of{c->d_inv_tgt.p, c->tgt16, OrientThr{c->orient_lo, c->orient_hi}, nullptr, nullptr, 0u, nullptr, nullptr,
                      c->d_hyp_p.p, c->d_hyp_q.p};
        of.keep_rec = c->d_keep_rec.p; of.keep_cap = c->keep_cap; of.slot_row = c->d_slot_row.p;
        return launch_keep_assemble(c->d_views.p, c->d_pairs.p, R, cap, c->d_row_start.p, c->d_row_pair.p, c->d_blk_row.p, c->d_row_start.p + R + 2, c->d_slots.p, of, st);
    };
    const uint64_t guess = std::min<uint64_t>(std::max<uint64_t>(c->keep_last_total + c->keep_last_total / 8 + (1u << 16), (uint64_t)R * 16), 0xFFFFFFFFull);
    L3D_HIP_CHECK(outputs(guess));
    uint64_t cap = std::min<uint64_t>({c->d_slots.cap, c->d_slot_row.cap, c->d_hyp_p.cap, c->d_hyp_q.cap,
                                       c->d_inv_tgt.cap * (c->tgt16 ? 2u : 1u), (size_t)0xFFFFFFFFull});
    cap = std::min<uint64_t>(cap, guess + guess / 2);
    for (int attempt = 0;; ++attempt) {
        if ((uint64_t)R * c->keep_cap * sizeof(Slot) > kKeepScratchMax || attempt > 2) { c->ragged = false; return kKeepAllTwoPass; }
        L3D_HIP_CHECK(c->d_keep_rec.reserve((size_t)R * c->keep_cap));
        const uint32_t n_blk = (uint32_t)(std::min<uint64_t>((uint64_t)R * c->keep_cap, 1ull << 32) / kKeepBlock) + 2;
// ... 210 lines not shown
```

line3dpp_amd/csrc/l3d_ctx.h:

```cpp
#pragma once
#include <algorithm>
#include <chrono>
#include <cstdio>
#include <cstdlib>
#include <fstream>
#include <memory>
#include <mutex>
#include <sstream>
#include <unordered_set>

#include "l3d_host.h"
#include "l3d_lists.h"
#include "l3d_recon.h"

struct l3d_ctx;

namespace l3d {

size_t scan_ws_words(size_t n, uint32_t bytes_per_element);
hipError_t launch_scan(const uint32_t* in, uint32_t n, uint32_t* out, unsigned long long* ws, uint32_t* total, hipStream_t);
hipError_t launch_collin(int pass, const ViewDev* views, uint32_t n_views, uint32_t max_M, const uint32_t* seg_base,
                         float collin_t, uint32_t* cnt, const uint32_t* coll_off, uint32_t* coll_idx, hipStream_t);
hipError_t launch_aff_coll_count(int mode, uint32_t n_items, const uint32_t* surv_tg, const float* simv, const HypRec*,
                                 const uint32_t* seg_base, const uint32_t* coll_off, uint32_t* cnt, hipStream_t);
hipError_t launch_aff_coll_sim(int mode, uint32_t n_items, const uint32_t* surv_sg, const uint32_t* surv_tg,
                               const int32_t* hyp_of_seg, const HypRec*, const ViewDev*, const uint32_t* seg_base,
                               const uint32_t* gseg_view, const uint32_t* coll_off, const uint32_t* coll_idx,
                               const uint32_t* item_off, const ViewAff*, const float* medians, const float* msdl,
                               float two_sigA_sqr, uint32_t* out_seg, float* out_sim, hipStream_t);
hipError_t launch_seam_entries(uint32_t n, const float4* m4, const float2* rt, const ViewDev*, float k, DEntry*, hipStream_t);
hipError_t launch_seam_all_present(uint32_t G, const uint32_t* off, const uint32_t* boff, uint64_t* bits, hipStream_t);
hipError_t launch_seam_scores_out(uint32_t n, const DEntry*, float* scores, hipStream_t);
hipError_t launch_fill_gseg_view(const uint32_t* seg_base, uint32_t V, uint32_t max_M, uint32_t* gseg_view, hipStream_t);
hipError_t launch_orient_pairs(const ViewDev*, const PairDesc*, uint32_t n_pairs, uint64_t max_slots, Slot* slots,
                               uint32_t* inv_tgt, uint32_t tgt16, float2* hyp_p, float2* hyp_q, double thr_lo, double thr_hi, hipStream_t);
hipError_t launch_bits_len(uint32_t G, const uint32_t* off, uint32_t* len, uint32_t* long_list, uint32_t* n_long,
                           hipStream_t);
hipError_t launch_support_long(uint32_t n_long, const uint32_t* long_list, const uint32_t* off, const uint32_t* boff,
                               const DEntry*, uint64_t* bits, const ViewDev*, const uint32_t* gseg_view, SimConst,
                               hipStream_t);
hipError_t launch_support_all(uint32_t g0, uint32_t G, const uint32_t* off, const uint32_t* boff, const DEntry*, uint64_t* bits,
                              const ViewDev*, const uint32_t* seg_base, const uint32_t* gseg_view, SimConst, hipStream_t);
hipError_t launch_score_all(uint32_t g0, uint32_t G, const uint32_t* off, const uint32_t* boff, const uint32_t* gseg_view, DEntry*,
                            const uint64_t* bits, Slot*, uint32_t* max_score_bits, const ViewDev*, const uint32_t* seg_base,
                            SimConst, hipStream_t);
hipError_t launch_median_all(uint32_t V, const float* depths, const uint32_t* hyp_off, const uint32_t* seg_base,
                             const uint32_t* tie_total, uint32_t* tie_out, float* out, const uint32_t* rb_src,
                             uint32_t* rb_host, uint32_t rb_words, uint32_t* rb_count, hipStream_t, uint32_t v0 = 0);
hipError_t launch_aff_sim(uint32_t N, uint32_t lo, uint32_t hi, const uint32_t* surv_sg, const uint32_t* surv_tg, const int32_t* hyp_of_seg,
                          const HypRec*, const ViewAff*, const float* medians, const float* msdl, float two_sigA_sqr,
                          float* simv, int32_t* ca, int32_t* cb, hipStream_t);
hipError_t launch_aff_flag(uint32_t N, const uint32_t* surv_off, const uint32_t* surv_sg, const uint32_t* surv_tg,
                           const float* simv, const int32_t* ca, const int32_t* cb, uint32_t* flag,
                           uint32_t* first_touch, uint32_t H, uint32_t* touch_flag, hipStream_t);
hipError_t launch_fill_u32(uint32_t*, uint32_t n, uint32_t val, hipStream_t);
hipError_t launch_aff_touch(uint32_t N, const uint32_t* flag, const uint32_t* epos, const int32_t* ca,
                            const int32_t* cb, uint32_t* first_touch, hipStream_t);
hipError_t launch_aff_mark(uint32_t H, const uint32_t* first_touch, uint32_t* touch_flag, hipStream_t);
hipError_t launch_aff_emit(uint32_t N, const uint32_t* flag, const uint32_t* epos, const int32_t* ca,
                           const int32_t* cb, const float* simv, const uint32_t* first_touch,
                           const uint32_t* touch_rank, const HypRec*, void* edges, void* local2global, hipStream_t);

hipError_t warm_affinity(hipStream_t); hipError_t warm_lists(hipStream_t); hipError_t warm_match(hipStream_t);
hipError_t warm_rdd(hipStream_t); hipError_t warm_scan(hipStream_t); hipError_t warm_views(hipStream_t);

int fail(int code, const std::string& msg);
const char* last_error_cstr();
void init_view(HostView& v, const double K[9], const double R[9], const double t[3]);
void translate_view(HostView& v, const d3& d);
d3 scene_translation(const std::vector<HostView*>& order);
void neighbors_from_worldpoints(const std::map<uint32_t, HostView*>& views, uint32_t num_neighbors);
void translate(::l3d_ctx& c);
void untranslate(::l3d_ctx& c);
void make_cull(const double F[9], double ws, double hs, double wt, double ht, PairCull& pc);
void pair_baseline(const d3& Cs, const d3& Ct, PairDesc& pd);
void orientation_thresholds(double& lo, double& hi);
SimConst sim_thresholds(float two_sigA_sqr);
struct HostTrace {
    bool on = std::getenv("L3D_TRACE") != nullptr;
    std::chrono::steady_clock::time_point t0 = std::chrono::steady_clock::now();
    std::vector<std::pair<double, const char*>> marks;
    void mark(const char* what) {
        if (!on) return;
        marks.emplace_back(std::chrono::duration<double, std::micro>(std::chrono::steady_clock::now() - t0).count(), what);
    }
    void flush() {
        for (auto& m : marks) std::fprintf(stderr, "[l3d trace] %9.1f us  %s\n", m.first, m.second);
        marks.clear();
    }
};
extern HostTrace g_trace;

float ev_ms(hipEvent_t a, hipEvent_t b);
float ev_ms(const ::l3d_ctx* c, int a, int b);
int affinity_core(::l3d_ctx* c);
int ensure_affinity_host(::l3d_ctx* c);
std::string output_filename(::l3d_ctx* c, int max_image_width);
int line_opt(::l3d_ctx* c, const std::map<uint32_t, const HostView*>& views, std::vector<ReconCluster>& clusters, uint32_t max_iter);
bool line_to_cayley(const d3& P1, const d3& P2, double x[4]);
bool cayley_to_segment(const double x[4], const d3& P1_old, const d3& P2_old, d3& P1, d3& P2);

}

extern "C" void abort_match(::l3d_ctx* c);
extern "C" void collect_match_timing(::l3d_ctx* c);

using namespace l3d;

struct l3d_ctx {
    int device = 0;
    hipStream_t stream = nullptr;
    std::recursive_mutex mu;
    std::map<uint32_t, std::unique_ptr<HostView>> views;
    std::vector<HostView*> order;
    std::vector<float> views_avg_depths;
    float sigma_p = 2.5f, sigma_a = 10.0f, two_sigA_sqr = 200.0f, epipolar_overlap = 0.25f;
    float const_regularization_depth = -1.0f, med_scene_depth = (float)kEps, med_scene_depth_lines = 0.0f;
    int kNN = 10, num_neighbors = 10;
    bool fixed3Dregularizer = false;
    bool brute = false;
    bool knn_replay = false;
    double orient_lo = -1.0, orient_hi = 1.0;
    d3 translation{0, 0, 0};
    enum { IDLE, BEGUN, MATCHED } state = IDLE;
    bool affinity_done = false;
    std::vector<PairDesc> pairs;
    std::vector<uint32_t> pair_src_cam, pair_tgt_cam;
    std::vector<char> pair_done;
    DevBuf<uint8_t> d_pair_present;
    uint64_t n_slots = 0, pair_tests = 0;
    uint32_t n_rows_total = 0;
    DevBuf<ViewDev> d_views;
    DevBuf<PairDesc> d_pairs;
    DevBuf<WorkItem> d_work;
    DevBuf<Slot> d_slots;
    DevBuf<uint32_t> d_slot_idx;
    std::vector<PairCull> cull;
    DevBuf<PairCull> d_cull;
    DevBuf<uint32_t> d_src_perm, d_tgt_perm;
    DevBuf<float2> d_src_band, d_chunk_band, d_tgt_band;
    DevBuf<float4> d_tgt_sf, d_tgt_s4;
    DevBuf<SegD32> d_tgt_sd;
    DevBuf<uint32_t> d_item_bucket, d_item_order, d_order_done;
    DevBuf<uint64_t> d_cull_keys;
    bool use_cull = true;
    unsigned visibility_t = 3;
    bool perform_rdd = false;
    uint32_t aff_n_edges = 0, aff_n_rows = 0;
    bool aff_host_valid = true;
    PinnedBuf<uint32_t> h_cnt;
    std::vector<uint8_t> pair_counted;
    DevBuf<SegX> d_gsegx;
    DevBuf<SegD32> d_gsegd32;
    float collinearity_t = -1.0f;
    DevBuf<uint32_t> d_coll_cnt, d_coll_off, d_coll_idx, d_item_cnt, d_item_off, d_item_seg;
    DevBuf<float> d_item_sim;
    PinnedBuf<ViewDev> h_views;
    PinnedBuf<PairDesc> h_pairs;
    PinnedBuf<PairCull> h_cull;
    PinnedBuf<WorkItem> h_work;
    UploadTag up_views, up_pairs, up_cull, up_seg_base, up_ltab;
    std::vector<unsigned char> begin_sig; bool begin_sig_valid = false;
    uint64_t cull_tot[4] = {0, 0, 0, 0};
    uint32_t layout_rows = 0;
    uint32_t tile_rows = 0;
    uint64_t pairs_version = 0;
    struct { uint64_t version = ~0ull; uint32_t first = 0, count = 0, rows = 0; size_t items = 0; const void* dev = nullptr; } work_key;
    PinnedBuf<uint32_t> h_segb;
    const void* gseg_view_for = nullptr;
    bool timing_pending = false;
    uint32_t pending_launches = 0;
    DevBuf<uint32_t> d_row_counts;
    bool ragged = false;
    uint32_t keep_cap = 0;
    DevBuf<Slot> d_keep_rec;
    DevBuf<uint32_t> d_row_pair, d_blk_row;
    DevBuf<uint32_t> d_row_start, d_slot_row;
    DevBuf<uint4> d_keep_info;
    std::vector<uint64_t> pair_nslots;
    uint64_t keep_last_total = 0;
    PinnedBuf<uint4> h_keep_info;
    uint64_t pair_slots(uint32_t p) const { return ragged ? pair_nslots[p] : (uint64_t)pairs[p].Ms * pairs[p].K; }
    DevBuf<uint32_t> d_tie_count;
    uint32_t tie_seq = 0;
    DevBuf<uint2> d_tie_list;
    DevBuf<uint64_t> d_tie_heap;
    uint32_t G = 0, n_ents = 0, n_surv = 0, n_hyps = 0;
    std::vector<uint32_t> seg_base;
    DevBuf<uint32_t> d_seg_base, d_gseg_view, d_scal;
    DevBuf<uint32_t> d_surv_off, d_hyp_off, d_surv_tg, d_surv_sg;
    DevBuf<uint32_t> d_inv_tgt;
    DevBuf<float2> d_hyp_p, d_hyp_q;
    uint32_t tgt16 = 0;
    DevBuf<uint32_t> d_poff, d_csr_dummy;
    uint32_t poff_total = 0, n_in_pairs = 0;
    DevBuf<Match> d_surv;
    DevBuf<int32_t> d_hyp_of_seg;
    DevBuf<float> d_depths;
    float* d_med = nullptr;
    DevBuf<HypRec> d_hyps;
    DevBuf<unsigned long long> d_cnt64, d_off64s, d_scan_ws, d_huge_u64;
    DevBuf<uint32_t> d_inv_refs;
    DevBuf<uint32_t> d_lzero, d_list2, d_list4, d_listH, d_seg_of_g, d_huge_u32;
    DevBuf<float> d_huge_f32;
    DevBuf<EdgeRec> d_ledges;
    DevBuf<HypHdr> d_lhyps;
    DevBuf<SegHdr> d_lsegs;
    DevBuf<CandRec> d_lcands;
    DevBuf<CandHdr> d_lchdrs;
    uint32_t lp_ecap = 0, lp_hcap = 0, lp_scap = 0, lp_ccap = 0, huge_cap = 0;
    uint32_t lp_attempts = 0;
    bool huge_skip = false, huge_ran = true;
    bool list4_skip = false, list4_ran = true;
    struct PoolCaps { uint32_t e = 0, h = 0, s = 0, c = 0, huge = 0; bool huge_skip = false, list4_skip = false; } caps_saved[2];
    int caps_mode = 0;
    uint32_t chain_need = 8, chain_enqueued = 10;
    uint32_t chain_hist[4] = {6, 6, 6, 6}, chain_hist_at = 0;
    uint32_t shard_world = 0;
    uint32_t shard_rank = 0, shard_v0 = 0, shard_v1 = 0, shard_pool0 = 0, shard_ppr = 0;
    std::vector<uint32_t> tail_base_n, tail_base_h;
    bool tail_counted = false, tail_written = false;
    uint32_t shard_dep_rank0 = 0;
    bool exch_ordered = false;
    uint32_t aff_parts_world = 0;
    bool aff_shard_open = false;
    bool lists_ready = false, lists_prepared = false;
    PinnedBuf<uint32_t> h_fin;
    PinnedBuf<char> h_ltab;
    DevBuf<char> d_ltab;
    std::vector<uint32_t> h_surv_off, h_hyp_off;
    bool host_offsets_valid = false;
    DevBuf<ViewAff> d_vaff;
    DevBuf<float> d_simv;
    PinnedBuf<ViewAff> h_vaff; UploadTag up_vaff;
    DevBuf<int32_t> d_ca, d_cb;
    DevBuf<uint32_t> d_flag, d_epos, d_first_touch, d_touch_flag, d_touch_rank;
    DevBuf<l3d_cledge> d_edges;
    DevBuf<l3d_segment2d> d_l2g;
    std::vector<l3d_cledge> edges;
    std::vector<l3d_segment2d> l2g;
    std::vector<ReconLine> lines3D;
    bool lines_done = false;
    bool use_ceres = false;
    l3d_line_opt_summary lo_stats{};
    PinnedBuf<char> h_lopt;
    DevBuf<char> d_lopt;
    hipEvent_t lo_ev[2] = {};
    hipEvent_t ev[10] = {};
    int timing_level = 1;
    bool ev_on(int k) const { return timing_level >= 2 || (timing_level == 1 && (k == 4 || k == 5)); }
    l3d_timings tm{};
    std::vector<float> det_segs;
    std::vector<uint32_t> det_counts;
    std::vector<l3d_detect_stats> det_stats;
};
```

line3dpp_amd/csrc/l3d_kernels.h:

```cpp
#pragma once
#include <atomic>

#include "l3d_dev.h"

struct l3d_cledge;

namespace l3d {

extern std::atomic<uint64_t> g_knn_replay_calls;
extern std::atomic<uint64_t> g_keep_all_repeats;
extern std::atomic<uint64_t> g_csr_global_launches;

constexpr int kMatchRows = 64;
constexpr uint32_t kTileClasses = 5;
constexpr uint32_t kTileMinItems = 24;
__host__ __device__ constexpr uint32_t tile_classes(uint32_t Ms, uint32_t R) { return Ms / R < kTileMinItems ? 2u : kTileClasses; }
__host__ __device__ constexpr uint32_t tile_src_cap(uint32_t Ms, uint32_t R) {
    return ((Ms + tile_classes(Ms, R) * (R - 1) + R - 1) / R) * R;
}
constexpr uint64_t kMatchTileMaxItems = 2048;
uint32_t match_tile_rows(int mode, bool brute, uint64_t est_row_items);
uint32_t match_layout_rows(int mode, bool brute, uint32_t tile_rows);
struct WorkItem {
    uint32_t pair;
    uint32_t src0;
};

struct PairCull {
    double As[3], Bs[3];
    double At[3], Bt[3];
    uint64_t s_off;
    uint64_t t_off;
    uint32_t c_off;
    uint32_t enabled;
    uint64_t k_off;
    uint32_t w_item0;
    uint32_t sorted_copy;
};
constexpr uint32_t kSortedCopyMinSegs = 4096;
struct CullPools {
    const PairCull* cull;
    uint32_t* src_perm;
    float2* src_band;
    uint32_t* tgt_perm;
    float4* tgt_sf;
    float2* tgt_band;
    float2* chunk_band;
    uint64_t* big_keys;
    uint32_t* item_bucket;
    uint32_t* item_order;
    uint32_t* order_done;
    uint32_t w_base;
    uint32_t cost_max;
    float4* tgt_s4;
    SegD32* tgt_sd;
    uint32_t row_cache;
    uint32_t padded_rows;
};
constexpr uint32_t kOrderBuckets = 1024;
constexpr uint32_t kCullLdsSegs = 16384;
constexpr uint32_t kCullBandCacheSegs = 4096;
constexpr uint32_t kCullMaxSegs = 1u << 20;

struct OrientFuse {
    uint32_t* inv_tgt;
    uint32_t tgt16;
    OrientThr thr;
    uint32_t* tie_count;
    uint2* tie_list;
    uint32_t tie_cap;
    uint32_t* tie_next;
    uint32_t* tie_total;
    float2* hyp_p;
    float2* hyp_q;
    Slot* keep_rec;
    uint32_t keep_cap;
    uint32_t* slot_row;
};

size_t match_lds_bytes(int mode, uint32_t K, bool ix16 = false, uint32_t waves = 1, bool brute = false, uint32_t tile_rows = 0,
                       bool row_cache = false);
bool match_row_cache(int mode, bool brute, uint32_t nwork, uint32_t tile_rows);
constexpr uint32_t kMatchOrderMaxItems = 16384;
constexpr uint32_t kMatchOrderMinItems = 3584;
uint32_t match_waves_per_group(int mode, bool brute, uint32_t nwork);
hipError_t launch_cull_prepare(const ViewDev* views, const PairDesc* pairs, uint32_t first, uint32_t count,
                               uint32_t max_M, CullPools pools, uint32_t tile_rows, hipStream_t stream);
hipError_t launch_order_items(const PairDesc* pairs, uint32_t first, uint32_t count, uint32_t max_Mt, CullPools pools,
                              uint32_t nwork, hipStream_t stream);
hipError_t launch_match_pairs(int mode, bool brute, const ViewDev* views, const PairDesc* pairs,
                              const WorkItem* work, uint32_t nwork, uint32_t maxK, Slot* slots,
                              uint32_t* row_counts, float thr, CullPools pools, OrientFuse of, bool ix16,
                              uint32_t tile_rows, hipStream_t stream);
uint32_t match_tied_grid(uint32_t scratch_stride);
hipError_t launch_queue_all_rows(const PairDesc* pairs, uint32_t first, uint32_t count, uint32_t max_Ms, uint32_t list_base,
                                 OrientFuse of, hipStream_t stream);
hipError_t launch_match_tied_rows(const ViewDev* views, const PairDesc* pairs, Slot* slots, uint32_t maxK, float thr,
                                  OrientFuse of, CullPools cp, uint64_t* scratch, uint32_t scratch_stride,
                                  hipStream_t stream);
hipError_t launch_pack_slot_idx(const Slot* slots, uint32_t* idx, uint64_t lo, uint64_t hi, hipStream_t stream);
hipError_t launch_expand_slot_idx(const ViewDev* views, const PairDesc* pairs, uint32_t first, uint32_t count,
                                  uint32_t max_row_slots, const uint32_t* idx, Slot* slots, OrientFuse of,
                                  hipStream_t stream);
constexpr uint32_t kKeepBlock = 1024;
hipError_t launch_keep_pair_info(const PairDesc* pairs, uint32_t n_pairs, const uint32_t* row_counts, const uint32_t* row_start,
                                 uint4* info, uint32_t* row_pair, uint32_t* blk_row, uint32_t n_blk, uint32_t* longest, hipStream_t stream);
hipError_t launch_keep_assemble(const ViewDev* views, const PairDesc* pairs, uint32_t n_rows, uint64_t slot_cap, const uint32_t* row_start,
                                const uint32_t* row_pair, const uint32_t* blk_row, const uint32_t* longest, Slot* slots, OrientFuse of,
                                hipStream_t stream);
hipError_t launch_prep_views(const ViewDev* views, uint32_t n_views, uint32_t max_M, hipStream_t stream);

struct InvRec; struct ListPools; struct PairCsr;
struct HugeScratchArgs { float* f32; uint32_t* u32; uint64_t* u64; uint32_t cap; uint32_t mean_list; uint32_t run_huge; uint32_t run_tier4; };
hipError_t launch_scan64(const unsigned long long* in, uint32_t n, unsigned long long* out, unsigned long long* tmp,
                         unsigned long long* total, hipStream_t st);
hipError_t launch_pair_csr(const PairDesc* pairs, uint32_t n_pairs, uint32_t max_Mt, const PairCsr* pair_csr,
                           const uint32_t* inv_tgt, uint32_t tgt16, uint32_t* poff, uint32_t* refs,
                           uint32_t* dummy, uint32_t tgt_v0, uint32_t tgt_v1, uint64_t max_pair_slots,
                           const uint32_t* row_start, hipStream_t st);
hipError_t launch_seg_index(ListPools lp, uint32_t* seg_of_g, uint32_t G, uint32_t world, hipStream_t st);
struct ListView; struct OutPair; struct InPair;
hipError_t launch_lists(uint32_t v0, uint32_t nv, uint32_t max_M, const ViewDev* views, const PairDesc* pairs,
                        const ListView* lviews, const OutPair* opairs, const InPair* ipairs, const uint32_t* gseg_view,
                        const uint32_t* poff, const uint32_t* inv_refs, const float2* hyp_p, const float2* hyp_q,
                        const Slot* slots, uint32_t uniform_K,
                        SimConst sc, ListPools lp, uint32_t* seg_of_g, HugeScratchArgs hsa, hipStream_t st);
hipError_t launch_chain_sweep(ListPools lp, uint8_t* positive, uint32_t* changed, uint32_t sweep, uint32_t* undecided,
                              hipStream_t st);
hipError_t launch_hyp_scores(ListPools lp, const uint8_t* positive, const uint32_t* gseg_view, Slot* slots,
                             const uint8_t* pair_present, uint32_t* max_score_bits, hipStream_t st);
hipError_t launch_hyp_filter(ListPools lp, uint32_t g0, uint32_t g1, const uint32_t* gseg_view, const uint32_t* max_score_bits,
                             uint32_t* kept_cnt, unsigned long long* best_pack, unsigned long long* cnt64,
                             hipStream_t st);
hipError_t launch_seg_write(uint32_t g0, uint32_t g1, unsigned long long base64, const ViewDev* views, const PairDesc* pairs, const uint32_t* seg_base,
                            const uint32_t* gseg_view, const unsigned long long* off64s,
                            const unsigned long long* best_pack, const uint32_t* seg_of_g, ListPools lp,
                            const Slot* slots, uint32_t* surv_off, uint32_t* hyp_off, Match* surv, uint32_t* surv_tg,
                            uint32_t* surv_sg, int32_t* hyp_of_seg, HypRec* hyps, float* depths, hipStream_t st);

size_t rdd_workspace_bytes(uint32_t nnz, uint32_t n_rows);
hipError_t launch_rdd(const struct ::l3d_cledge* edges_in, uint32_t nnz, uint32_t n_rows, uint32_t iterations,
                      struct ::l3d_cledge* edges_out, void* workspace, size_t workspace_bytes, hipStream_t stream);

struct TriArgs {
    const double* P;
    uint32_t n_cameras;
    uint64_t n_points;
    const uint64_t* off;
    const uint32_t* cam;
    const double* xy;
    double* X;
    uint8_t* valid;
};
constexpr size_t kTriLdsBytes = 32 * 1024;
hipError_t launch_triangulate(const TriArgs& t, hipStream_t st);

}
```

line3dpp_amd/csrc/l3d_phase_b.hip:

```cpp
#include "l3d_ctx.h"

extern "C" {

static int match_finish_impl(l3d_ctx* c);
static int lists_prepare(l3d_ctx* c, int caps_mode);
static int lists_reserve(l3d_ctx* c);
static int lists_run(l3d_ctx* c, uint32_t v0, uint32_t nv, uint32_t pool0, uint32_t npools);

static int lists_shard_impl(l3d_ctx* c, uint32_t rank, uint32_t world, int64_t view0, int64_t view1, void* slab_ptr[4],
                            uint64_t slab_bytes[4], void* full_ptr[4]) {
    if (!c || !slab_ptr || !slab_bytes || !full_ptr) return fail(L3D_ERR_ARG, "null argument");
    std::lock_guard<std::recursive_mutex> lk(c->mu);
    if (c->state != l3d_ctx::BEGUN) return fail(L3D_ERR_STATE, "l3d_match_begin must precede l3d_lists_shard");
    (void)hipSetDevice(c->device);
    const int rc = [&]() -> int {
        if (world == 0 || world > kListPools || rank >= world) return fail(L3D_ERR_ARG, "rank / world out of range");
        const uint32_t V = (uint32_t)c->order.size();
        uint32_t v0, v1;
        if (view0 >= 0) {
            if (view1 < view0 || (uint64_t)view1 > V) return fail(L3D_ERR_ARG, "view range out of bounds");
            v0 = (uint32_t)view0; v1 = (uint32_t)view1;
        } else {
            uint64_t G = 0;
            std::vector<uint64_t> base(V + 1, 0);
// ... 69 lines not shown
        while (v < n_views && std::fabs(acc + vcost[v] - target) <= std::fabs(acc - target)) { acc += vcost[v]; ++v; }
        view_bounds[r] = v;
    }
    view_bounds[world] = n_views;
    uint32_t p = 0;
    for (uint32_t r = 0; r <= world; ++r) {
        while (p < n_pairs && pair_src_view[p] < view_bounds[r]) ++p;
        pair_bounds[r] = p;
    }
    pair_bounds[world] = n_pairs;
    return L3D_OK;
}

int l3d_match_finish(l3d_ctx* c) {
    if (!c) return fail(L3D_ERR_ARG, "null argument");
    std::lock_guard<std::recursive_mutex> lk(c->mu);
    if (c->state != l3d_ctx::BEGUN) return fail(L3D_ERR_STATE, "l3d_match_begin must precede l3d_match_finish");
    (void)hipSetDevice(c->device);
    const int rc = match_finish_impl(c);
    if (rc == L3D_ERR_RETRY) return rc;
    if (rc != L3D_OK) {
        const std::string why = l3d_last_error();
        abort_match(c);
        set_error(why);
    }
    return rc;
}

static constexpr uint32_t kChainSweeps = 16;

static ListPools list_pools(l3d_ctx* c, uint32_t pool0 = 0, uint32_t npools = kListPools) {
    ListPools lp;
    lp.cnt = c->d_lzero.p; lp.edges = c->d_ledges.p; lp.hyps = c->d_lhyps.p; lp.segs = c->d_lsegs.p;
    lp.cands = c->d_lcands.p; lp.chdrs = c->d_lchdrs.p;
    lp.ecap = c->lp_ecap; lp.hcap = c->lp_hcap; lp.scap = c->lp_scap; lp.ccap = c->lp_ccap;
    lp.flags = c->d_lzero.p + kListPools * 16;
    lp.list2 = c->d_list2.p; lp.list4 = c->d_list4.p; lp.listH = c->d_listH.p;
    lp.pool0 = pool0; lp.npools = npools;
    lp.row_start = c->ragged ? c->d_row_start.p : nullptr; lp.slot_row = c->ragged ? c->d_slot_row.p : nullptr;
    static const bool no_stat = std::getenv("L3D_NO_LIST_STAT") != nullptr;
    lp.count_entries = no_stat ? 0u : 1u;
    return lp;
}

static unsigned long long* tot64_of(l3d_ctx* c) { return (unsigned long long*)c->d_med; }
static float* medians_of(l3d_ctx* c) { return c->d_med + 8; }
static size_t fin_med(uint32_t V) { return ((size_t)8 + V + 3) & ~(size_t)3; }
static constexpr size_t kFinHead = (size_t)kListPools * 16 + 96;

struct ZeroLayout { size_t flags, changed, med, max_score, kept, best, words; };
static ZeroLayout zero_layout(uint32_t V, uint32_t G);
static uint8_t* positive_of(l3d_ctx* c) {
    return (uint8_t*)(c->d_lzero.p + zero_layout((uint32_t)c->order.size(), c->G).words);
}
static ZeroLayout zero_layout(uint32_t V, uint32_t G) {
    ZeroLayout z;
    z.flags = (size_t)kListPools * 16; z.changed = z.flags + 32; z.med = z.changed + 64; z.max_score = z.med + fin_med(V);
    z.kept = z.max_score + ((size_t)V + 1) * 16;
    z.best = (z.kept + G + 1) & ~(size_t)1;
    z.words = z.best + 2 * (size_t)G + 2;
    return z;
}

static int lists_prepare(l3d_ctx* c, int caps_mode) {
    if (caps_mode != c->caps_mode) {
        c->caps_saved[c->caps_mode] = l3d_ctx::PoolCaps{c->lp_ecap, c->lp_hcap, c->lp_scap, c->lp_ccap, c->huge_cap, c->huge_skip, c->list4_skip};
        const l3d_ctx::PoolCaps& pc = c->caps_saved[caps_mode];
        c->lp_ecap = pc.e; c->lp_hcap = pc.h; c->lp_scap = pc.s; c->lp_ccap = pc.c; c->huge_cap = pc.huge; c->huge_skip = pc.huge_skip;
        c->list4_skip = pc.list4_skip;
        c->caps_mode = caps_mode;
    }
    if (caps_mode == 1) { c->huge_skip = false; c->list4_skip = false; }
    hipStream_t st = c->stream;
    const uint32_t V = (uint32_t)c->order.size(), P = (uint32_t)c->pairs.size();
    c->seg_base.assign(V + 1, 0);
    for (uint32_t vi = 0; vi < V; ++vi) c->seg_base[vi + 1] = c->seg_base[vi] + c->order[vi]->M;
    const uint32_t G = c->G = c->seg_base[V];
    uint64_t max_slots = 0;
    for (uint32_t p = 0; p < P; ++p) max_slots = std::max<uint64_t>(max_slots, c->pair_slots(p));
    if (2 * c->n_slots >= (1ull << 32)) return fail(L3D_ERR_LIMIT, "more than 2^32 hypotheses");
    L3D_HIP_CHECK(c->d_seg_base.reserve(V + 1)); L3D_HIP_CHECK(c->d_gseg_view.reserve(G + 1));
    L3D_HIP_CHECK(c->d_surv_off.reserve(G + 2)); L3D_HIP_CHECK(c->d_hyp_off.reserve(G + 2));
    L3D_HIP_CHECK(c->d_hyp_of_seg.reserve(G + 1));
    L3D_HIP_CHECK(c->d_cnt64.reserve(G + 2)); L3D_HIP_CHECK(c->d_off64s.reserve(G + 2));
    L3D_HIP_CHECK(c->d_scan_ws.reserve_zeroed(scan_ws_words(G, 8), st));
    L3D_HIP_CHECK(c->d_seg_of_g.reserve(G + 1)); L3D_HIP_CHECK(c->d_list2.reserve(G + 1)); L3D_HIP_CHECK(c->d_list4.reserve(G + 1)); L3D_HIP_CHECK(c->d_listH.reserve(G + 1));
    L3D_HIP_CHECK(c->d_hyps.reserve(std::max<uint32_t>(G, 1))); L3D_HIP_CHECK(c->d_depths.reserve(2 * (size_t)G + 2));
    L3D_HIP_CHECK(c->d_inv_refs.reserve(std::max<uint64_t>(c->n_slots, 1)));
    L3D_HIP_CHECK(c->d_inv_tgt.reserve(std::max<uint64_t>(c->n_slots, 1)));
    L3D_HIP_CHECK(c->d_hyp_p.reserve(std::max<uint64_t>(c->n_slots, 1))); L3D_HIP_CHECK(c->d_hyp_q.reserve(std::max<uint64_t>(c->n_slots, 1)));
    L3D_HIP_CHECK(c->h_fin.reserve(kFinHead + fin_med(V)));
    if (c->ev_on(6)) L3D_HIP_CHECK(hipEventRecord(c->ev[6], st));
    g_trace.mark("finish: reserves done");
    {
        bool sent = false;
        L3D_HIP_CHECK(upload_table(c->d_seg_base, c->h_segb, c->seg_base.data(), ((size_t)V + 1) * 4, c->up_seg_base, st, &sent));
        if (sent || c->gseg_view_for != (const void*)c->d_gseg_view.p) {
            uint32_t max_M = 0;
            for (auto* v : c->order) max_M = std::max(max_M, v->M);
            L3D_HIP_CHECK(launch_fill_gseg_view(c->d_seg_base.p, V, max_M, c->d_gseg_view.p, st));
            c->gseg_view_for = c->d_gseg_view.p;
        }
    }
    {
        static_assert(sizeof(ListView) == 32 && sizeof(OutPair) == 32 && sizeof(InPair) == 16 && sizeof(PairCsr) == 16, "table layout");
        uint32_t n_in = 0;
        for (uint32_t vi = 0; vi < V; ++vi) n_in += (uint32_t)c->order[vi]->in_pairs.size();
        const size_t o_in = ((size_t)V + P) * 32, o_pp = o_in + (size_t)n_in * 16;
        std::vector<char> table(o_pp + ((size_t)P + 1) * 16 + 32, 0);
        ListView* hv = (ListView*)table.data();
        OutPair* hp = (OutPair*)(table.data() + (size_t)V * 32);
        InPair* hi = (InPair*)(table.data() + o_in);
        PairCsr* hpp = (PairCsr*)(table.data() + o_pp);
        for (uint32_t p = 0; p < P; ++p) hpp[p] = PairCsr{kEmpty, 0u, 0u, 0u};
        uint32_t n = 0, ni = 0;
        uint64_t poff_total = 0;
        for (uint32_t vi = 0; vi < V; ++vi) {
            ListView& lv = hv[vi];
            lv = ListView{};
            lv.seg_base = c->seg_base[vi]; lv.M = c->order[vi]->M; lv.q0 = n; lv.k = c->order[vi]->k;
            for (uint32_t p : c->order[vi]->out_pairs) {
                const PairDesc& pd = c->pairs[p];
                OutPair op{};
                op.slot_off = pd.slot_off; op.tgt = pd.tgt; op.pair = p; op.K = pd.K; op.row_off = pd.row_off;
                hp[n++] = op;
            }
            lv.nq = n - lv.q0;
            lv.i0 = ni; lv.ni = (uint32_t)c->order[vi]->in_pairs.size(); lv.pbase = (uint32_t)poff_total;
            uint32_t q = 0;
            for (uint32_t p : c->order[vi]->in_pairs) {
                const PairDesc& pd = c->pairs[p];
                InPair ip{};
                ip.rec_base = (uint32_t)pd.slot_off; ip.src = pd.src; ip.pair = p;
                hpp[p] = PairCsr{(uint32_t)poff_total, lv.ni, q++, 0u};
                hi[ni++] = ip;
            }
            poff_total += ((uint64_t)lv.M + 1) * lv.ni;
            if (poff_total >= (1ull << 32)) return fail(L3D_ERR_LIMIT, "more than 2^32 per-pair CSR offsets in phase B");
        }
        c->poff_total = (uint32_t)poff_total; c->n_in_pairs = ni;
        L3D_HIP_CHECK(c->d_poff.reserve(std::max<uint64_t>(poff_total, 1)));
        L3D_HIP_CHECK(c->d_ltab.reserve(table.size()));
        L3D_HIP_CHECK(upload_table(c->d_ltab, c->h_ltab, table.data(), o_pp + (size_t)P * 16, c->up_ltab, st));
    }
    for (uint32_t p0 = 0; p0 < P;) {
        if (c->pair_counted[p0] || !c->pair_done[p0]) { ++p0; continue; }
        uint32_t p1 = p0;
        while (p1 < P && !c->pair_counted[p1] && c->pair_done[p1]) ++p1;
        L3D_HIP_CHECK(launch_orient_pairs(c->d_views.p, c->d_pairs.p + p0, p1 - p0, max_slots, c->d_slots.p, c->d_inv_tgt.p,
                                          c->tgt16, c->d_hyp_p.p, c->d_hyp_q.p, c->orient_lo, c->orient_hi, st));
        for (uint32_t p = p0; p < p1; ++p) c->pair_counted[p] = 1;
        p0 = p1;
    }
    if (!c->lp_ecap) {
        const double scale = [] { const char* e = std::getenv("L3D_POOL_SCALE"); const double v = e ? std::atof(e) : 1.0; return v > 0.0 ? v : 1.0; }();
        const double ns = scale * (double)c->n_slots;
        const double bytes1 = ns * (sizeof(EdgeRec) / 4.0 + sizeof(HypHdr) / 8.0 + sizeof(CandRec) / 2.0);
        const double gen = scale < 1.0 ? 1.0 : std::min(4.0, std::max(1.0, 4.0e9 / std::max(bytes1, 1.0)));
        c->lp_ecap = (uint32_t)std::max<double>(gen * ns / 4 / kListPools, scale < 1.0 ? 16 : 512);
        c->lp_hcap = (uint32_t)std::max<double>(gen * ns / 8 / kListPools, scale < 1.0 ? 16 : 256);
        c->lp_ccap = (uint32_t)std::max<double>(gen * ns / 2 / kListPools, scale < 1.0 ? 32 : 1024);
    }
    c->lp_scap = std::max<uint32_t>(c->lp_scap, G / kListPools + 64);
    if (!c->huge_cap) c->huge_cap = (uint32_t)std::min<uint64_t>(std::max<uint64_t>(c->n_slots / 16, 1u << 20), 1u << 30);
    return L3D_OK;
}

static int lists_reserve(l3d_ctx* c) {
    g_trace.mark("lists_reserve enter");
    const uint32_t V = (uint32_t)c->order.size();
    const ZeroLayout z = zero_layout(V, c->G);
    L3D_HIP_CHECK(c->d_lzero.reserve(z.words + 2 + (c->n_slots + 3) / 4));
    c->d_med = (float*)(c->d_lzero.p + z.med);
    L3D_HIP_CHECK(c->d_ledges.reserve((size_t)kListPools * c->lp_ecap));
    L3D_HIP_CHECK(c->d_lhyps.reserve((size_t)kListPools * c->lp_hcap));
    L3D_HIP_CHECK(c->d_lsegs.reserve((size_t)kListPools * c->lp_scap));
    L3D_HIP_CHECK(c->d_lchdrs.reserve((size_t)kListPools * c->lp_scap));
    L3D_HIP_CHECK(c->d_lcands.reserve((size_t)kListPools * c->lp_ccap));
    L3D_HIP_CHECK(c->d_huge_f32.reserve(2 * (size_t)c->huge_cap)); L3D_HIP_CHECK(c->d_huge_u32.reserve(3 * (size_t)c->huge_cap));
    L3D_HIP_CHECK(c->d_huge_u64.reserve(c->huge_cap));
    const size_t surv_cap = (size_t)kListPools * c->lp_hcap;
    L3D_HIP_CHECK(c->d_surv.reserve(surv_cap)); L3D_HIP_CHECK(c->d_surv_tg.reserve(surv_cap));
    L3D_HIP_CHECK(c->d_surv_sg.reserve(surv_cap));
    return L3D_OK;
}

static int lists_run(l3d_ctx* c, uint32_t v0, uint32_t nv, uint32_t pool0, uint32_t npools) {
    g_trace.mark("lists_run enter");
    hipStream_t st = c->stream;
    const uint32_t V = (uint32_t)c->order.size(), P = (uint32_t)c->pairs.size(), G = c->G;
    const ZeroLayout z = zero_layout(V, G);
    const ListPools lp = list_pools(c, pool0, npools);
    const SimConst simc = sim_thresholds(c->two_sigA_sqr);
    uint64_t max_slots = 0;
    for (uint32_t p = 0; p < P; ++p) max_slots = std::max<uint64_t>(max_slots, c->pair_slots(p));
    L3D_HIP_CHECK(hipMemsetAsync(c->d_lzero.p, 0, z.words * 4 + std::max<uint64_t>(c->n_slots, 1), st));
    g_trace.mark("zero block memset enqueued");
    const ListView* lviews = (const ListView*)c->d_ltab.p;
    const OutPair* opairs = (const OutPair*)(c->d_ltab.p + (size_t)V * 32);
    const InPair* ipairs = (const InPair*)(c->d_ltab.p + ((size_t)V + P) * 32);
    const PairCsr* pair_poff = (const PairCsr*)(c->d_ltab.p + ((size_t)V + P) * 32 + (size_t)c->n_in_pairs * 16);
    {
        uint32_t max_Mt = 0;
        for (auto& pd : c->pairs) if (pd.tgt > pd.src && pd.tgt >= v0 && pd.tgt < v0 + nv) max_Mt = std::max(max_Mt, pd.Mt);
        if (max_Mt) {
            if (max_Mt > 32768 || std::getenv("L3D_CSR_GLOBAL")) L3D_HIP_CHECK(c->d_csr_dummy.reserve((size_t)P * 64));
            L3D_HIP_CHECK(launch_pair_csr(c->d_pairs.p, P, max_Mt, pair_poff, c->d_inv_tgt.p, c->tgt16, c->d_poff.p, c->d_inv_refs.p,
                                          c->d_csr_dummy.p, v0, v0 + nv, max_slots, c->ragged ? c->d_row_start.p : nullptr, st));
        }
    }
    g_trace.mark("pair CSRs enqueued");
    const uint32_t mean_list = c->n_ents ? (uint32_t)(c->n_ents / std::max<uint32_t>(G, 1))
                                         : (uint32_t)(1.5 * (double)c->n_slots / std::max<uint32_t>(G, 1));
    const HugeScratchArgs hsa{c->d_huge_f32.p, c->d_huge_u32.p, (uint64_t*)c->d_huge_u64.p, c->huge_cap, mean_list,
                              c->huge_skip ? 0u : 1u, c->list4_skip ? 0u : 1u};
    c->huge_ran = !c->huge_skip; c->list4_ran = !c->list4_skip;
    uint32_t max_M = 0;
    for (uint32_t vi = v0; vi < v0 + nv; ++vi) max_M = std::max(max_M, c->order[vi]->M);
    L3D_HIP_CHECK(launch_lists(v0, nv, max_M, c->d_views.p, c->d_pairs.p, lviews, opairs, ipairs, c->d_gseg_view.p,
                               c->d_poff.p, c->d_inv_refs.p, c->d_hyp_p.p, c->d_hyp_q.p, c->d_slots.p, c->kNN > 0 ? (uint32_t)c->kNN : 0u, simc, lp,
                               c->d_seg_of_g.p, hsa, st));
    if (c->ev_on(9)) L3D_HIP_CHECK(hipEventRecord(c->ev[9], st));
    g_trace.mark("list pass enqueued");
    return L3D_OK;
}

struct TailShard { uint32_t v0, v1, g0, g1, pool0, npools; };
static TailShard whole_tail(const l3d_ctx* c) { return TailShard{0u, (uint32_t)c->order.size(), 0u, c->G, 0u, kListPools}; }

static int tail_count_run(l3d_ctx* c, bool fresh, const TailShard& ts) {
    g_trace.mark("tail_run enter");
    hipStream_t st = c->stream;
    const uint32_t V = (uint32_t)c->order.size(), G = c->G;
    const ZeroLayout z = zero_layout(V, G);
    const bool dep = ts.npools < kListPools && c->shard_world > 1 && c->shard_dep_rank0 <= c->shard_rank;
    const uint32_t cp0 = dep ? c->shard_dep_rank0 * c->shard_ppr : 0u, cp1 = dep ? (c->shard_rank + 1) * c->shard_ppr : kListPools;
    const ListPools lp = list_pools(c, cp0, cp1 - cp0), lps = list_pools(c, ts.pool0, ts.npools);
    uint32_t* changed = c->d_lzero.p + z.changed;
    uint32_t* max_score = c->d_lzero.p + z.max_score;
    uint32_t* kept = c->d_lzero.p + z.kept;
    unsigned long long* best = (unsigned long long*)(c->d_lzero.p + z.best);
    if (!fresh) L3D_HIP_CHECK(hipMemsetAsync(changed, 0, (z.words - z.changed) * 4, st));
    const uint32_t need = std::max(std::max(c->chain_hist[0], c->chain_hist[1]), std::max(c->chain_hist[2], c->chain_hist[3]));
    const uint32_t n_sweeps = std::min(kChainSweeps, std::max(4u, need + 3));
    c->chain_enqueued = n_sweeps;
    if (!fresh) L3D_HIP_CHECK(hipMemset2DAsync(c->d_lzero.p + 7, 64, 0, 4, kListPools, st));
    for (uint32_t s2 = 0; s2 < n_sweeps; ++s2)
        L3D_HIP_CHECK(launch_chain_sweep(lp, positive_of(c), changed, s2, c->d_surv_tg.p, st));
    g_trace.mark("chain sweeps enqueued");
    const uint8_t* present = nullptr;
    if (c->shard_world > 1) {
        L3D_HIP_CHECK(c->d_pair_present.reserve(std::max<size_t>(c->pair_done.size(), 1)));
        L3D_HIP_CHECK(hipMemcpyAsync(c->d_pair_present.p, c->pair_done.data(), c->pair_done.size(), hipMemcpyHostToDevice, st));
        present = c->d_pair_present.p;
    }
    L3D_HIP_CHECK(launch_hyp_scores(lps, positive_of(c), c->d_gseg_view.p, c->d_slots.p, present, max_score, st));
    g_trace.mark("hyp_scores enqueued");
    L3D_HIP_CHECK(launch_hyp_filter(lps, ts.g0, ts.g1, c->d_gseg_view.p, max_score, kept, best, c->d_cnt64.p, st));
    g_trace.mark("hyp_filter enqueued");
    L3D_HIP_CHECK(launch_scan64(c->d_cnt64.p + ts.g0, ts.g1 - ts.g0, c->d_off64s.p + ts.g0, c->d_scan_ws.p, tot64_of(c) + 1, st));
    g_trace.mark("scan enqueued");
    return L3D_OK;
}

static int tail_write_run(l3d_ctx* c, const TailShard& ts, unsigned long long base64, bool publish) {
    hipStream_t st = c->stream;
    const uint32_t V = (uint32_t)c->order.size(), G = c->G;
    const ZeroLayout z = zero_layout(V, G);
    const ListPools lps = list_pools(c, ts.pool0, ts.npools);
    unsigned long long* best = (unsigned long long*)(c->d_lzero.p + z.best);
    L3D_HIP_CHECK(launch_seg_write(ts.g0, ts.g1, base64, c->d_views.p, c->d_pairs.p, c->d_seg_base.p, c->d_gseg_view.p,
                                   c->d_off64s.p, best, c->d_seg_of_g.p, lps, c->d_slots.p, c->d_surv_off.p, c->d_hyp_off.p,
                                   c->d_surv.p, c->d_surv_tg.p, c->d_surv_sg.p, c->d_hyp_of_seg.p, c->d_hyps.p, c->d_depths.p, st));
    g_trace.mark("seg_write enqueued");
    void* h_dev = nullptr;
    L3D_HIP_CHECK(hipHostGetDevicePointer(&h_dev, c->h_fin.p, 0));
    L3D_HIP_CHECK(launch_median_all(ts.v1 - ts.v0, c->d_depths.p, c->d_hyp_off.p, c->d_seg_base.p,
                                    c->d_tie_count.p ? c->d_tie_count.p + 2 : nullptr, (uint32_t*)tot64_of(c), medians_of(c),
                                    c->d_lzero.p, publish ? (uint32_t*)h_dev : nullptr, (uint32_t)(kFinHead + fin_med(V)),
                                    c->d_lzero.p + z.flags + 16, st, ts.v0));
    g_trace.mark("median + read-back enqueued");
    return L3D_OK;
}

static int tail_run(l3d_ctx* c, bool fresh) {
    const TailShard ts = whole_tail(c);
    int rc = tail_count_run(c, fresh, ts);
    if (rc) return rc;
    rc = tail_write_run(c, ts, 0ull, true);
    if (rc) return rc;
    if (c->ev_on(7)) L3D_HIP_CHECK(hipEventRecord(c->ev[7], c->stream));
    g_trace.mark("tail enqueued");
    return L3D_OK;
}

static constexpr int kRetry = 1;
static int check_pass(l3d_ctx* c) {
    const uint32_t* h = c->h_fin.p;
    const uint32_t* hf = h + kListPools * 16;
    uint32_t fl[8];
    for (int k = 0; k < 8; ++k) fl[k] = hf[k];
    if (c->shard_world > 1) {
        const uint32_t ppr = kListPools / c->shard_world;
        for (uint32_t r = 0; r < c->shard_world; ++r)
            for (int k = 0; k < 4; ++k) fl[k] |= h[(size_t)r * ppr * 16 + 8 + k];
        fl[6] = 0;
        for (uint32_t r = 0; r < c->shard_world; ++r) fl[6] = std::max(fl[6], h[(size_t)r * ppr * 16 + 12]);
    }
    if (fl[1]) return fail(L3D_ERR_LIMIT, "a 2D segment has more than 65535 match hypotheses");
    const bool huge_missed = (fl[5] && !c->huge_ran) || (fl[4] && !c->list4_ran);
    c->huge_skip = fl[5] == 0 && c->shard_world <= 1;
    c->list4_skip = fl[4] == 0 && c->shard_world <= 1;
    if (huge_missed) { ++c->tm.pool_retries; return kRetry; }
    if (fl[3]) return fail(L3D_ERR_HIP, "internal error: hypothesis counters and slot flags disagree");
    if (fl[0] || fl[2]) {
        ++c->tm.pool_retries;
        if (++c->lp_attempts > 6) return fail(L3D_ERR_LIMIT, "phase-B pools keep overflowing");
        if (fl[0]) {
            uint32_t me = 0, mh = 0, ms = 0, mc = 0;
            for (uint32_t q = 0; q < kListPools; ++q) {
                me = std::max(me, h[q * 16]); mh = std::max(mh, h[q * 16 + 1]);
                ms = std::max(ms, std::max(h[q * 16 + 2], h[q * 16 + 4])); mc = std::max(mc, h[q * 16 + 3]);
            }
            const bool cands_over = mc > c->lp_ccap || ms > c->lp_scap;
            c->lp_ccap = std::max(c->lp_ccap, mc + mc / 2 + 64); c->lp_scap = std::max(c->lp_scap, ms + ms / 2 + 64);
            c->lp_ecap = std::max(cands_over ? 2 * c->lp_ecap : c->lp_ecap, me + me / 2 + 64);
            c->lp_hcap = std::max(cands_over ? 2 * c->lp_hcap : c->lp_hcap, mh + mh / 2 + 64);
        }
        if (fl[2]) c->huge_cap = (uint32_t)std::min<uint64_t>(std::max<uint64_t>(2ull * c->huge_cap, fl[6] + 1024ull), 1u << 31);
        return kRetry;
    }
    return L3D_OK;
}

static int finish_commit(l3d_ctx* c) {
    const uint32_t V = (uint32_t)c->order.size();
    const uint32_t* h = c->h_fin.p;
    const uint32_t* h0 = h + kFinHead;
    const uint32_t* changed = h + kListPools * 16 + 32;
    c->n_surv = h0[2]; c->n_hyps = h0[3];
    c->tm.tied_rows = h0[0];
    {
        uint64_t ents = 0, inv = 0, cands = 0, hdrs = 0;
        for (uint32_t q = 0; q < kListPools; ++q) { ents += h[q * 16 + 5]; inv += h[q * 16 + 6]; cands += h[q * 16 + 3]; hdrs += h[q * 16 + 1]; }
        c->n_ents = (uint32_t)std::min<uint64_t>(ents, 0xFFFFFFFFu);
        c->tm.list_entries = c->n_ents;
        c->tm.list_inverse = (uint32_t)std::min<uint64_t>(inv, 0xFFFFFFFFu);
        c->tm.list_candidates = (uint32_t)std::min<uint64_t>(cands, 0xFFFFFFFFu);
        c->tm.list_headers = (uint32_t)std::min<uint64_t>(hdrs, 0xFFFFFFFFu);
        c->tm.slots_lo = (uint32_t)c->n_slots; c->tm.slots_hi = (uint32_t)(c->n_slots >> 32);
    }
    for (uint32_t s2 = 0; s2 < c->chain_enqueued; ++s2) c->tm.chain_sweeps += changed[s2] ? 1u : 0u;
    c->chain_need = c->tm.chain_extra_rounds ? kChainSweeps : c->tm.chain_sweeps;
    c->chain_hist[c->chain_hist_at++ & 3u] = c->chain_need;
    {
        uint64_t ne = 0;
        uint32_t me = 0, mh = 0, ms = 0, mc = 0;
        for (uint32_t q = 0; q < kListPools; ++q) {
            ne += h[q * 16];
            me = std::max(me, h[q * 16]); mh = std::max(mh, h[q * 16 + 1]);
            ms = std::max(ms, std::max(h[q * 16 + 2], h[q * 16 + 4])); mc = std::max(mc, h[q * 16 + 3]);
        }
        c->tm.support_words = (uint32_t)ne;
        auto fit = [](uint32_t cap, uint32_t need, uint32_t lowest) {
            const uint32_t want = std::max(need + need / 4 + 64, lowest);
            return cap > want + want / 2 ? want : cap;
        };
        c->lp_ecap = fit(c->lp_ecap, me, 256); c->lp_hcap = fit(c->lp_hcap, mh, 128);
        c->lp_scap = fit(c->lp_scap, ms, 64); c->lp_ccap = fit(c->lp_ccap, mc, 512);
    }
    for (uint32_t vi = 0; vi < V; ++vi) c->order[vi]->median_depth = ((const float*)h0)[8 + vi];
    c->host_offsets_valid = false;
    if (c->timing_pending) {
        collect_match_timing(c);
        c->tm.match_pairs_ms += ev_ms(c, 2, 3);
    }
    c->tm.finish_ms = ev_ms(c, 6, 7);
    c->tm.lists_ms = ev_ms(c, 6, 9);
    c->tm.record_kbytes = (uint32_t)(((uint64_t)kListPools * ((uint64_t)c->lp_ecap * sizeof(EdgeRec) + (uint64_t)c->lp_hcap * sizeof(HypHdr) +
                                                              (uint64_t)c->lp_scap * sizeof(SegHdr) + 64)) >> 10);
    c->tm.begin_ms = ev_ms(c, 0, 1);
    untranslate(*c);
    c->state = l3d_ctx::MATCHED;
    c->shard_world = 0; c->lists_ready = false; c->lists_prepared = false;
    return L3D_OK;
}

static int tail_until_converged(l3d_ctx* c) {
    hipStream_t st = c->stream;
    int rc = tail_run(c, true);
    if (rc) return rc;
    g_trace.mark("phase B enqueued, waiting");
    L3D_HIP_CHECK(hipStreamSynchronize(st));
    g_trace.mark("phase B done");
    rc = check_pass(c);
    if (rc) return rc;
    while (c->h_fin.p[kListPools * 16 + 32 + c->chain_enqueued - 1]) {
        rc = tail_run(c, false);
        if (rc) return rc;
        L3D_HIP_CHECK(hipStreamSynchronize(st));
        ++c->tm.chain_extra_rounds;
    }
    return L3D_OK;
}

static int match_finish_impl(l3d_ctx* c) {
    int rc;
    if (c->lists_ready) {
        const ListPools lp = list_pools(c);
        L3D_HIP_CHECK(launch_seg_index(lp, c->d_seg_of_g.p, c->G, c->shard_world, c->stream));
        rc = tail_until_converged(c);
        if (rc == kRetry) { c->lists_ready = false; return fail(L3D_ERR_RETRY, "phase-B pools enlarged: repeat l3d_lists_shard and the exchange"); }
        if (rc) return rc;
        return finish_commit(c);
    }
    rc = lists_prepare(c, 0);
    if (rc) return rc;
    c->lp_attempts = 0;
    const uint32_t V = (uint32_t)c->order.size();
    for (;;) {
        rc = lists_reserve(c);
        if (rc) return rc;
        rc = lists_run(c, 0, V, 0, kListPools);
        if (rc) return rc;
        rc = tail_until_converged(c);
        if (rc == kRetry) continue;
        if (rc) return rc;
        break;
    }
    return finish_commit(c);
}

static int tail_count_until_converged(l3d_ctx* c, const TailShard& ts) {
    hipStream_t st = c->stream;
    const uint32_t V = (uint32_t)c->order.size();
    auto run = [&](bool fresh) -> int {
        const int rc = tail_count_run(c, fresh, ts);
        if (rc) return rc;
        L3D_HIP_CHECK(hipMemcpyAsync(c->h_fin.p, c->d_lzero.p, (kFinHead + fin_med(V)) * 4, hipMemcpyDeviceToHost, st));
        L3D_HIP_CHECK(hipStreamSynchronize(st));
        return L3D_OK;
    };
    int rc = run(true);
    if (rc) return rc;
    rc = check_pass(c);
    if (rc) return rc;
    while (c->h_fin.p[kListPools * 16 + 32 + c->chain_enqueued - 1]) {
        rc = run(false);
        if (rc) return rc;
        ++c->tm.chain_extra_rounds;
    }
    return L3D_OK;
}

static int close_failed_call(l3d_ctx* c, int rc) {
    if (rc != L3D_OK && rc != L3D_ERR_RETRY) {
        const std::string why = l3d_last_error();
        abort_match(c);
        set_error(why);
    }
    return rc;
}

int l3d_shard_options(l3d_ctx* c, uint32_t first_needed_rank, int exchanges_stream_ordered) {
    if (!c) return fail(L3D_ERR_ARG, "null argument");
    std::lock_guard<std::recursive_mutex> lk(c->mu);
    c->shard_dep_rank0 = first_needed_rank;
    c->exch_ordered = exchanges_stream_ordered != 0;
    return L3D_OK;
}

int l3d_tail_shard_count(l3d_ctx* c, uint32_t counts[2]) {
    if (!c || !counts) return fail(L3D_ERR_ARG, "null argument");
    std::lock_guard<std::recursive_mutex> lk(c->mu);
    if (c->state != l3d_ctx::BEGUN || !c->lists_ready || c->shard_world < 2)
        return fail(L3D_ERR_STATE, "l3d_tail_shard_count follows l3d_lists_shard* and the exchange of its slabs (world > 1)");
    (void)hipSetDevice(c->device);
    const int rc = [&]() -> int {
        if (c->shard_dep_rank0 > c->shard_rank) return fail(L3D_ERR_ARG, "l3d_shard_options: first_needed_rank lies above this rank");
        const ListPools lp = list_pools(c, c->shard_dep_rank0 * c->shard_ppr, (c->shard_rank + 1 - c->shard_dep_rank0) * c->shard_ppr);
        L3D_HIP_CHECK(launch_seg_index(lp, c->d_seg_of_g.p, c->G, c->shard_world, c->stream));
        const TailShard ts{c->shard_v0, c->shard_v1, c->seg_base[c->shard_v0], c->seg_base[c->shard_v1], c->shard_pool0, c->shard_ppr};
        const int r = tail_count_until_converged(c, ts);
        if (r == kRetry) { c->lists_ready = false; return fail(L3D_ERR_RETRY, "phase-B pools enlarged: repeat l3d_lists_shard and the exchange"); }
        if (r) return r;
        const uint32_t* med = c->h_fin.p + kFinHead;
        counts[0] = med[2]; counts[1] = med[3];
        c->tail_counted = true; c->tail_written = false;
        return L3D_OK;
    }();
    return close_failed_call(c, rc);
}

int l3d_tail_shard_layout(l3d_ctx* c, uint32_t world, const uint32_t* counts_all, const uint32_t* view_bounds, void* base_ptr[9],
                          uint64_t elt_bytes[9], uint64_t* first, uint64_t* count) {
    if (!c || !counts_all || !view_bounds || !base_ptr || !elt_bytes || !first || !count) return fail(L3D_ERR_ARG, "null argument");
    std::lock_guard<std::recursive_mutex> lk(c->mu);
    if (c->state != l3d_ctx::BEGUN || !c->tail_counted || world != c->shard_world)
        return fail(L3D_ERR_STATE, "l3d_tail_shard_layout follows l3d_tail_shard_count (same world size)");
    (void)hipSetDevice(c->device);
    const int rc = [&]() -> int {
        const uint32_t V = (uint32_t)c->order.size();
        if (view_bounds[0] != 0 || view_bounds[world] != V || view_bounds[c->shard_rank] != c->shard_v0 ||
            view_bounds[c->shard_rank + 1] != c->shard_v1)
            return fail(L3D_ERR_ARG, "view bounds do not match the list pass of this rank");
        c->tail_base_n.assign(world + 1, 0); c->tail_base_h.assign(world + 1, 0);
        uint64_t n = 0, h = 0;
        for (uint32_t r = 0; r < world; ++r) {
            if (view_bounds[r + 1] < view_bounds[r]) return fail(L3D_ERR_ARG, "view bounds are not ascending");
            c->tail_base_n[r] = (uint32_t)n; c->tail_base_h[r] = (uint32_t)h;
            n += counts_all[2 * r]; h += counts_all[2 * r + 1];
        }
        if (n >= (1ull << 32) || n > (uint64_t)kListPools * c->lp_hcap || h > c->G)
            return fail(L3D_ERR_LIMIT, "the ranks' counts exceed the output arrays");
        c->tail_base_n[world] = (uint32_t)n; c->tail_base_h[world] = (uint32_t)h;
        const uint32_t me = c->shard_rank;
        const TailShard ts{c->shard_v0, c->shard_v1, c->seg_base[c->shard_v0], c->seg_base[c->shard_v1], c->shard_pool0, c->shard_ppr};
        const int r2 = tail_write_run(c, ts, (unsigned long long)c->tail_base_n[me] | ((unsigned long long)c->tail_base_h[me] << 32), false);
        if (r2) return r2;
        if (!c->exch_ordered) L3D_HIP_CHECK(hipStreamSynchronize(c->stream));
        void* bp[9] = {c->d_surv.p, c->d_surv_tg.p, c->d_surv_sg.p, c->d_hyps.p, c->d_depths.p, c->d_surv_off.p, c->d_hyp_off.p,
                       c->d_hyp_of_seg.p, medians_of(c)};
        const uint64_t eb[9] = {sizeof(Match), 4, 4, sizeof(HypRec), 8, 4, 4, 4, 4};
        for (int k = 0; k < 9; ++k) { base_ptr[k] = bp[k]; elt_bytes[k] = eb[k]; }
        for (uint32_t r = 0; r < world; ++r) {
            const uint64_t g0 = c->seg_base[view_bounds[r]], g1 = c->seg_base[view_bounds[r + 1]], end = r + 1 == world ? 1 : 0;
            const uint64_t f[9] = {c->tail_base_n[r], c->tail_base_n[r], c->tail_base_n[r], c->tail_base_h[r], c->tail_base_h[r],
                                   g0, g0, g0, view_bounds[r]};
            const uint64_t m[9] = {counts_all[2 * r], counts_all[2 * r], counts_all[2 * r], counts_all[2 * r + 1], counts_all[2 * r + 1],
                                   g1 - g0 + end, g1 - g0 + end, g1 - g0, (uint64_t)view_bounds[r + 1] - view_bounds[r]};
            for (int k = 0; k < 9; ++k) { first[9 * r + k] = f[k]; count[9 * r + k] = m[k]; }
        }
        c->tail_written = true;
        return L3D_OK;
    }();
    return close_failed_call(c, rc);
}

int l3d_tail_shard_commit(l3d_ctx* c) {
    if (!c) return fail(L3D_ERR_ARG, "null argument");
    std::lock_guard<std::recursive_mutex> lk(c->mu);
    if (c->state != l3d_ctx::BEGUN || !c->tail_written)
        return fail(L3D_ERR_STATE, "l3d_tail_shard_commit follows l3d_tail_shard_layout and the exchange of the parts");
    (void)hipSetDevice(c->device);
    const int rc = [&]() -> int {
        const uint32_t V = (uint32_t)c->order.size(), world = c->shard_world;
        uint32_t* med = c->h_fin.p + kFinHead;
        if (c->ev_on(7)) L3D_HIP_CHECK(hipEventRecord(c->ev[7], c->stream));
        L3D_HIP_CHECK(hipMemcpyAsync(med, c->d_med, (8 + (size_t)V) * 4, hipMemcpyDeviceToHost, c->stream));
        L3D_HIP_CHECK(hipStreamSynchronize(c->stream));
        med[2] = c->tail_base_n[world]; med[3] = c->tail_base_h[world];
        c->tail_counted = false; c->tail_written = false;
        const int fr = finish_commit(c);
        if (fr == L3D_OK) c->aff_parts_world = world;
        return fr;
    }();
    return close_failed_call(c, rc);
}

}
```

Baseline: 991,600.

## Fuse scan producers and consumers into a functor-based decoupled-lookback scan

Introduces a generic scan-map kernel that takes a load functor and a store functor. The affinity flag, touch and mark steps and the segment gate and offset writes now run inside the scan's load and store phases instead of as separate kernels with intermediate arrays. Resetting first_touch moves into the similarity kernel, and the segment-offset writes move out of seg_write into the scan store. This cuts kernel launches and global round trips, at the cost of heavier scan kernels and atomicMin now running inside the scan store.

```diff
diff --git a/line3dpp_amd/csrc/k_affinity.hip b/line3dpp_amd/csrc/k_affinity.hip
--- a/line3dpp_amd/csrc/k_affinity.hip
+++ b/line3dpp_amd/csrc/k_affinity.hip
@@ -1,5 +1,6 @@
 #include "l3d_dev.h"
 #include "l3d_kernels.h"
+#include "l3d_scan.h"
 
 namespace l3d {
 
@@ -48,8 +49,10 @@
                           const int32_t* __restrict__ hyp_of_seg, const HypRec* __restrict__ hyps,
                           const ViewAff* __restrict__ va, const float* __restrict__ medians,
                           const float* __restrict__ msdl_ptr, float two_sigA_sqr, float* __restrict__ simv,
-                          int32_t* __restrict__ cand_a, int32_t* __restrict__ cand_b) {
+                          int32_t* __restrict__ cand_a, int32_t* __restrict__ cand_b,
+                          uint32_t* __restrict__ first_touch, uint32_t H) {
     const uint32_t c = blockIdx.x * blockDim.x + threadIdx.x;
+    if (c < H) first_touch[c] = kEmpty;
     if (c >= N) return;
     const int32_t ha = hyp_of_seg[surv_sg[c]], hb = hyp_of_seg[surv_tg[c]];
     cand_a[c] = ha;
@@ -63,53 +66,58 @@
     simv[c] = sim;
 }
 
-__global__ void k_aff_flag(uint32_t N, const uint32_t* __restrict__ surv_off, const uint32_t* __restrict__ surv_sg,
-                           const uint32_t* __restrict__ surv_tg, const float* __restrict__ simv,
-                           const int32_t* __restrict__ cand_a, const int32_t* __restrict__ cand_b,
-                           uint32_t* __restrict__ flag, uint32_t* __restrict__ first_touch, uint32_t H,
-                           uint32_t* __restrict__ touch_flag) {
-    const uint32_t c = blockIdx.x * blockDim.x + threadIdx.x;
-    if (c < H) first_touch[c] = kEmpty;
-    if (c < N) { touch_flag[2 * c] = 0; touch_flag[2 * c + 1] = 0; }
-    if (c == 0) touch_flag[2 * (size_t)N] = 0;
-    if (c >= N) return;
-    uint32_t f = 0;
-    if (simv[c] > kMinAffinity) {
-        f = 1;
+struct AffFlagLoad {
+    const uint32_t *surv_off, *surv_sg, *surv_tg;
+    const float* simv;
+    const int32_t *cand_a, *cand_b;
+    __device__ __forceinline__ uint32_t operator()(uint32_t c) const {
+        if (!(simv[c] > kMinAffinity)) return 0u;
         if (cand_b[c] < cand_a[c]) {
             const uint32_t sg = surv_sg[c], tg = surv_tg[c];
-            for (uint32_t i = surv_off[tg]; i < surv_off[tg + 1]; ++i) {
-                if (surv_tg[i] == sg) {
-                    if (simv[i] > kMinAffinity) f = 0;
-                    break;
-                }
-            }
+            for (uint32_t i = surv_off[tg]; i < surv_off[tg + 1]; ++i)
+                if (surv_tg[i] == sg) return simv[i] > kMinAffinity ? 0u : 1u;
         }
-    }
-    flag[c] = f;
-}
-
-__global__ void k_fill_u32(uint32_t* p, uint32_t n, uint32_t val) {
-    const uint32_t i = blockIdx.x * blockDim.x + threadIdx.x;
-    if (i < n) p[i] = val;
-}
-
-__global__ void k_aff_touch(uint32_t N, const uint32_t* __restrict__ flag, const uint32_t* __restrict__ epos,
-                            const int32_t* __restrict__ cand_a, const int32_t* __restrict__ cand_b,
-                            uint32_t* __restrict__ first_touch) {
-    const uint32_t c = blockIdx.x * blockDim.x + threadIdx.x;
-    if (c >= N || !flag[c]) return;
-    const uint32_t k = epos[c];
-    atomicMin(&first_touch[cand_a[c]], 2u * k);
-    atomicMin(&first_touch[cand_b[c]], 2u * k + 1u);
-}
-
-__global__ void k_aff_mark(uint32_t H, const uint32_t* __restrict__ first_touch, uint32_t* __restrict__ touch_flag) {
-    const uint32_t h = blockIdx.x * blockDim.x + threadIdx.x;
-    if (h >= H) return;
-    const uint32_t p = first_touch[h];
-    if (p != kEmpty) touch_flag[p] = 1u;
-}
+        return 1u;
+    }
+};
+struct AffTouchStore {
+    uint32_t *flag, *epos, *edge_cand, *first_touch;
+    const int32_t *cand_a, *cand_b;
+    uint32_t* n_edges;
+    __device__ __forceinline__ void operator()(uint32_t c, uint32_t k, uint32_t f) const {
+        flag[c] = f;
+        epos[c] = k;
+        if (!f) return;
+        edge_cand[k] = c;
+        atomicMin(&first_touch[cand_a[c]], 2u * k);
+        atomicMin(&first_touch[cand_b[c]], 2u * k + 1u);
+    }
+    __device__ __forceinline__ void total(uint32_t n, uint32_t t) const { epos[n] = t; *n_edges = t; }
+};
+
+struct AffMarkLoad {
+    const uint32_t *n_edges, *edge_cand, *first_touch;
+    const int32_t *cand_a, *cand_b;
+    __device__ __forceinline__ uint32_t operator()(uint32_t p) const {
+        const uint32_t k = p >> 1;
+        if (k >= *n_edges) return 0u;
+        const uint32_t c = edge_cand[k];
+        const int32_t h = (p & 1u) ? cand_b[c] : cand_a[c];
+        return first_touch[h] == p ? 1u : 0u;
+    }
+};
+struct AffRankStore {
+    uint32_t* touch_rank;
+    const uint32_t* n_edges;
+    uint32_t *n_rows, *host_cnt;
+    __device__ __forceinline__ void operator()(uint32_t p, uint32_t rank, uint32_t) const { touch_rank[p] = rank; }
+    __device__ __forceinline__ void total(uint32_t n, uint32_t t) const {
+        touch_rank[n] = t;
+        *n_rows = t;
+        host_cnt[0] = *n_edges;
+        host_cnt[1] = t;
+    }
+};
 
 struct CLEdgeDev { int32_t i, j; float w; };
 struct Seg2D { uint32_t cam, seg; };
@@ -225,35 +233,27 @@
 
 hipError_t launch_aff_sim(uint32_t N, uint32_t lo, uint32_t hi, const uint32_t* surv_sg, const uint32_t* surv_tg, const int32_t* hyp_of_seg,
                           const HypRec* hyps, const ViewAff* va, const float* medians, const float* msdl,
-                          float two_sigA_sqr, float* simv, int32_t* ca, int32_t* cb, hipStream_t st) {
+                          float two_sigA_sqr, float* simv, int32_t* ca, int32_t* cb, uint32_t* first_touch, uint32_t H,
+                          hipStream_t st) {
     if (!N) return hipSuccess;
-    hipLaunchKernelGGL(k_aff_sim, grid1(N, 128), dim3(128), 0, st, N, lo, hi, surv_sg, surv_tg, hyp_of_seg, hyps, va, medians,
-                       msdl, two_sigA_sqr, simv, ca, cb);
-    return hipGetLastError();
-}
-hipError_t launch_aff_flag(uint32_t N, const uint32_t* surv_off, const uint32_t* surv_sg, const uint32_t* surv_tg,
-                           const float* simv, const int32_t* ca, const int32_t* cb, uint32_t* flag,
-                           uint32_t* first_touch, uint32_t H, uint32_t* touch_flag, hipStream_t st) {
+    hipLaunchKernelGGL(k_aff_sim, grid1(std::max(N, H), 128), dim3(128), 0, st, N, lo, hi, surv_sg, surv_tg, hyp_of_seg, hyps, va, medians,
+                       msdl, two_sigA_sqr, simv, ca, cb, first_touch, H);
+    return hipGetLastError();
+}
+hipError_t launch_aff_edges(uint32_t N, const uint32_t* surv_off, const uint32_t* surv_sg, const uint32_t* surv_tg,
+                            const float* simv, const int32_t* ca, const int32_t* cb, uint32_t* flag, uint32_t* epos,
+                            uint32_t* edge_cand, uint32_t* first_touch, uint32_t* n_edges, unsigned long long* ws,
+                            hipStream_t st) {
     if (!N) return hipSuccess;
-    hipLaunchKernelGGL(k_aff_flag, grid1(std::max(N, H)), dim3(256), 0, st, N, surv_off, surv_sg, surv_tg, simv, ca, cb,
-                       flag, first_touch, H, touch_flag);
-    return hipGetLastError();
-}
-hipError_t launch_fill_u32(uint32_t* p, uint32_t n, uint32_t val, hipStream_t st) {
-    if (!n) return hipSuccess;
-    hipLaunchKernelGGL(k_fill_u32, grid1(n), dim3(256), 0, st, p, n, val);
-    return hipGetLastError();
-}
-hipError_t launch_aff_touch(uint32_t N, const uint32_t* flag, const uint32_t* epos, const int32_t* ca,
-                            const int32_t* cb, uint32_t* first_touch, hipStream_t st) {
+    return launch_scan_map<uint32_t>(AffFlagLoad{surv_off, surv_sg, surv_tg, simv, ca, cb}, N,
+                                     AffTouchStore{flag, epos, edge_cand, first_touch, ca, cb, n_edges}, ws, st);
+}
+hipError_t launch_aff_rows(uint32_t N, const uint32_t* n_edges, const uint32_t* edge_cand, const uint32_t* first_touch,
+                           const int32_t* ca, const int32_t* cb, uint32_t* touch_rank, uint32_t* n_rows,
+                           uint32_t* host_cnt, unsigned long long* ws, hipStream_t st) {
     if (!N) return hipSuccess;
-    hipLaunchKernelGGL(k_aff_touch, grid1(N), dim3(256), 0, st, N, flag, epos, ca, cb, first_touch);
-    return hipGetLastError();
-}
-hipError_t launch_aff_mark(uint32_t H, const uint32_t* first_touch, uint32_t* touch_flag, hipStream_t st) {
-    if (!H) return hipSuccess;
-    hipLaunchKernelGGL(k_aff_mark, grid1(H), dim3(256), 0, st, H, first_touch, touch_flag);
-    return hipGetLastError();
+    return launch_scan_map<uint32_t>(AffMarkLoad{n_edges, edge_cand, first_touch, ca, cb}, 2 * N,
+                                     AffRankStore{touch_rank, n_edges, n_rows, host_cnt}, ws, st);
 }
 hipError_t launch_aff_emit(uint32_t N, const uint32_t* flag, const uint32_t* epos, const int32_t* ca,
                            const int32_t* cb, const float* simv, const uint32_t* first_touch,
diff --git a/line3dpp_amd/csrc/k_lists.hip b/line3dpp_amd/csrc/k_lists.hip
--- a/line3dpp_amd/csrc/k_lists.hip
+++ b/line3dpp_amd/csrc/k_lists.hip
@@ -5,6 +5,7 @@
 #include "l3d_dev.h"
 #include "l3d_kernels.h"
 #include "l3d_lists.h"
+#include "l3d_scan.h"
 
 constexpr uint32_t kLists4Grid = 512;
 
@@ -1033,13 +1034,35 @@
     }
 }
 
-__global__ void k_seg_filter(uint32_t g0, uint32_t g1, const uint32_t* __restrict__ kept_cnt,
-                             const unsigned long long* __restrict__ best_pack, unsigned long long* __restrict__ cnt64) {
-    const uint32_t g = g0 + blockIdx.x * blockDim.x + threadIdx.x;
-    if (g >= g1) return;
-    const bool ok = __uint_as_float((uint32_t)(best_pack[g] >> 32)) > kMinBestScore3D;
-    cnt64[g] = ok ? ((1ull << 32) | kept_cnt[g]) : 0ull;
-}
+struct SegGateLoad {
+    uint32_t g0;
+    const uint32_t* kept_cnt;
+    const unsigned long long* best_pack;
+    __device__ __forceinline__ unsigned long long operator()(uint32_t i) const {
+        const uint32_t g = g0 + i;
+        const bool ok = __uint_as_float((uint32_t)(best_pack[g] >> 32)) > kMinBestScore3D;
+        return ok ? ((1ull << 32) | kept_cnt[g]) : 0ull;
+    }
+};
+struct SegOffsetsStore {
+    uint32_t g0;
+    const uint32_t* flags;
+    unsigned long long *off64s, *total_out;
+    uint32_t *surv_off, *hyp_off;
+    int32_t* hyp_of_seg;
+    __device__ __forceinline__ void operator()(uint32_t i, unsigned long long o, unsigned long long v) const {
+        const uint32_t gs = g0 + i;
+        const bool pass_ok = !(flags[0] | flags[2]);
+        off64s[gs] = o;
+        surv_off[gs] = (uint32_t)o; hyp_off[gs] = (uint32_t)(o >> 32);
+        hyp_of_seg[gs] = ((v >> 32) != 0 && pass_ok) ? (int32_t)(uint32_t)(o >> 32) : -1;
+    }
+    __device__ __forceinline__ void total(uint32_t n, unsigned long long t) const {
+        off64s[g0 + n] = t;
+        surv_off[g0 + n] = (uint32_t)t; hyp_off[g0 + n] = (uint32_t)(t >> 32);
+        *total_out = t;
+    }
+};
 
 __device__ __forceinline__ void make_match(const ViewDev* views, const PairDesc* pairs, uint32_t view, uint32_t seg,
                                            const HypHdr& h, Match& m, uint32_t& tgt_view, uint32_t& tgt_seg) {
@@ -1054,6 +1077,7 @@
     m.dq1 = h.oq1; m.dq2 = h.oq2;
 }
 
+template <bool SEGS>
 __global__ void k_seg_write(uint32_t g0, uint32_t g1, unsigned long long base64, const ViewDev* __restrict__ views, const PairDesc* __restrict__ pairs,
                             const uint32_t* __restrict__ seg_base, const uint32_t* __restrict__ gseg_view,
                             const unsigned long long* __restrict__ off64s, const unsigned long long* __restrict__ best_pack,
@@ -1063,7 +1087,7 @@
                             int32_t* __restrict__ hyp_of_seg, HypRec* __restrict__ hyps, float* __restrict__ depths) {
     const uint32_t t = blockIdx.x * blockDim.x + threadIdx.x;
     const bool pass_ok = !(lp.flags[0] | lp.flags[2]);
-    if (t <= g1 - g0) {
+    if (SEGS && t <= g1 - g0) {
         const uint32_t gs = g0 + t;
         const unsigned long long o = off64s[gs] + base64;
         surv_off[gs] = (uint32_t)o; hyp_off[gs] = (uint32_t)(o >> 32);
@@ -1234,22 +1258,35 @@
     hipLaunchKernelGGL(k_hyp_scores, hyp_grid(lp), dim3(256), 0, st, lp, positive, gseg_view, slots, pair_present, max_score_bits);
     return hipGetLastError();
 }
-hipError_t launch_hyp_filter(ListPools lp, uint32_t g0, uint32_t g1, const uint32_t* gseg_view, const uint32_t* max_score_bits,
-                             uint32_t* kept_cnt, unsigned long long* best_pack, unsigned long long* cnt64,
-                             hipStream_t st) {
+hipError_t launch_hyp_filter(ListPools lp, const uint32_t* gseg_view, const uint32_t* max_score_bits,
+                             uint32_t* kept_cnt, unsigned long long* best_pack, hipStream_t st) {
     hipLaunchKernelGGL(k_hyp_filter, hyp_grid(lp), dim3(256), 0, st, lp, gseg_view, max_score_bits, kept_cnt, best_pack);
-    if (g1 > g0) hipLaunchKernelGGL(k_seg_filter, dim3((g1 - g0 + 255) / 256), dim3(256), 0, st, g0, g1, kept_cnt, best_pack, cnt64);
     return hipGetLastError();
 }
-hipError_t launch_seg_write(uint32_t g0, uint32_t g1, unsigned long long base64, const ViewDev* views, const PairDesc* pairs, const uint32_t* seg_base,
+hipError_t launch_seg_offsets(ListPools lp, uint32_t g0, uint32_t g1, const uint32_t* kept_cnt, const unsigned long long* best_pack,
+                              unsigned long long* off64s, unsigned long long* total, unsigned long long* ws,
+                              uint32_t* surv_off, uint32_t* hyp_off, int32_t* hyp_of_seg, hipStream_t st) {
+    const SegGateLoad load{g0, kept_cnt, best_pack};
+    if (surv_off)
+        return launch_scan_map<unsigned long long>(load, g1 - g0, SegOffsetsStore{g0, lp.flags, off64s, total, surv_off, hyp_off, hyp_of_seg}, ws, st);
+    return launch_scan_map<unsigned long long>(load, g1 - g0, scanmap::StoreArray<unsigned long long>{off64s + g0, total}, ws, st);
+}
+hipError_t launch_seg_write(bool segments, uint32_t g0, uint32_t g1, unsigned long long base64, const ViewDev* views, const PairDesc* pairs, const uint32_t* seg_base,
                             const uint32_t* gseg_view, const unsigned long long* off64s,
                             const unsigned long long* best_pack, const uint32_t* seg_of_g, ListPools lp,
                             const Slot* slots, uint32_t* surv_off, uint32_t* hyp_off, Match* surv, uint32_t* surv_tg,
                             uint32_t* surv_sg, int32_t* hyp_of_seg, HypRec* hyps, float* depths, hipStream_t st) {
-    const uint64_t n_thr = std::max<uint64_t>((uint64_t)(g1 - g0) + 1, (uint64_t)lp.npools * lp.hcap);
-    hipLaunchKernelGGL(k_seg_write, dim3((uint32_t)((n_thr + 255) / 256)), dim3(256), 0, st, g0, g1, base64, views, pairs, seg_base, gseg_view,
-                       off64s, best_pack, seg_of_g, lp, slots, surv_off, hyp_off, surv, surv_tg, surv_sg, hyp_of_seg,
-                       hyps, depths);
+    const uint64_t n_hdr = (uint64_t)lp.npools * lp.hcap;
+    const uint64_t n_thr = segments ? std::max<uint64_t>((uint64_t)(g1 - g0) + 1, n_hdr) : std::max<uint64_t>(n_hdr, 1);
+    const dim3 grid((uint32_t)((n_thr + 255) / 256));
+    if (segments)
+        hipLaunchKernelGGL(k_seg_write<true>, grid, dim3(256), 0, st, g0, g1, base64, views, pairs, seg_base, gseg_view,
+                           off64s, best_pack, seg_of_g, lp, slots, surv_off, hyp_off, surv, surv_tg, surv_sg, hyp_of_seg,
+                           hyps, depths);
+    else
+        hipLaunchKernelGGL(k_seg_write<false>, grid, dim3(256), 0, st, g0, g1, base64, views, pairs, seg_base, gseg_view,
+                           off64s, best_pack, seg_of_g, lp, slots, surv_off, hyp_off, surv, surv_tg, surv_sg, hyp_of_seg,
+                           hyps, depths);
     return hipGetLastError();
 }
 
diff --git a/line3dpp_amd/csrc/k_scan.hip b/line3dpp_amd/csrc/k_scan.hip
--- a/line3dpp_amd/csrc/k_scan.hip
+++ b/line3dpp_amd/csrc/k_scan.hip
@@ -1,128 +1,19 @@
 #include "l3d_dev.h"
 #include "l3d_kernels.h"
+#include "l3d_scan.h"
 
 namespace l3d {
 
 namespace {
 
-constexpr uint32_t kScanBlock = 1024, kScanItems = 4, kScanTile = kScanBlock * kScanItems;
-constexpr unsigned long long kAgg = 1ull << 32, kIncl = 2ull << 32;
-
-template <class T>
-__device__ __forceinline__ T block_exclusive_scan(T v, T* wsum , T& block_total) {
-    const uint32_t tid = threadIdx.x, lane = tid & 63u, wave = tid >> 6;
-    T x = v;
-#pragma unroll
-    for (int d = 1; d < 64; d <<= 1) {
-        const T y = __shfl_up(x, d);
-        if (lane >= (uint32_t)d) x += y;
-    }
-    if (lane == 63) wsum[wave] = x;
-    __syncthreads();
-    if (tid == 0) {
-        T acc = 0;
-        for (uint32_t w = 0; w < kScanBlock / 64; ++w) { const T t = wsum[w]; wsum[w] = acc; acc += t; }
-        wsum[16] = acc;
-    }
-    __syncthreads();
-    block_total = wsum[16];
-    return wsum[wave] + x - v;
-}
-
-__device__ __forceinline__ uint32_t wave_sum(uint32_t v) {
-#pragma unroll
-    for (int d = 32; d > 0; d >>= 1) v += __shfl_xor(v, d);
-    return v;
-}
-
-template <class T>
-__global__ __launch_bounds__(kScanBlock) void k_scan(const T* __restrict__ in, uint32_t n, T* __restrict__ out,
-                                                     T* __restrict__ total_out, unsigned long long* __restrict__ ws) {
-    constexpr uint32_t LANES = sizeof(T) / 4;
-    __shared__ T wsum[17];
-    __shared__ T s_prefix;
-    __shared__ uint32_t s_last, s_tile;
-    const uint32_t nb = gridDim.x, tid = threadIdx.x, lane = tid & 63u;
-    if (tid == 0) s_tile = (uint32_t)__hip_atomic_fetch_add(&ws[1], 1ull, __ATOMIC_RELAXED, __HIP_MEMORY_SCOPE_AGENT);
-    __syncthreads();
-    const uint32_t tile = s_tile;
-    const uint32_t base = tile * kScanTile + tid * kScanItems;
-    T a[kScanItems];
-    T v = 0;
-#pragma unroll
-    for (uint32_t k = 0; k < kScanItems; ++k) { a[k] = (base + k < n) ? in[base + k] : (T)0; v += a[k]; }
-    T agg;
-    T ex = block_exclusive_scan(v, wsum, agg);
-    unsigned long long* state = ws + 2;
-    if (tid < 64) {
-        if (lane < LANES)
-            __hip_atomic_store(&state[(size_t)tile * LANES + lane],
-                               (tile == 0 ? kIncl : kAgg) | (uint32_t)((unsigned long long)agg >> (32 * lane)),
-                               __ATOMIC_RELAXED, __HIP_MEMORY_SCOPE_AGENT);
-        unsigned long long prefix = 0;
-        if (tile > 0) {
-#pragma unroll
-            for (uint32_t l = 0; l < LANES; ++l) {
-                uint32_t acc = 0;
-                for (int idx = (int)tile - 1;; idx -= 64) {
-                    const int t = idx - (int)lane;
-                    unsigned long long s = kIncl;
-                    if (t >= 0) {
-                        do s = __hip_atomic_load(&state[(size_t)t * LANES + l], __ATOMIC_RELAXED, __HIP_MEMORY_SCOPE_AGENT);
-                        while ((s >> 32) == 0);
-                    }
-                    const uint64_t incl = __builtin_amdgcn_ballot_w64((s >> 32) == 2);
-                    if (incl) {
-                        const uint32_t first = (uint32_t)__builtin_ctzll(incl);
-                        acc += wave_sum(lane <= first ? (uint32_t)s : 0u);
-                        break;
-                    }
-                    acc += wave_sum((uint32_t)s);
-                }
-                prefix |= (unsigned long long)acc << (32 * l);
-            }
-            if (lane < LANES)
-                __hip_atomic_store(&state[(size_t)tile * LANES + lane],
-                                   kIncl | (uint32_t)((prefix + (unsigned long long)agg) >> (32 * lane)),
-                                   __ATOMIC_RELAXED, __HIP_MEMORY_SCOPE_AGENT);
-        }
-        if (lane == 0) s_prefix = (T)prefix;
-    }
-    __syncthreads();
-    ex += s_prefix;
-#pragma unroll
-    for (uint32_t k = 0; k < kScanItems; ++k) {
-        if (base + k < n) out[base + k] = ex;
-        ex += a[k];
-    }
-    if (tile == nb - 1 && tid == 0) {
-        const T total = s_prefix + agg;
-        out[n] = total;
-        if (total_out) *total_out = total;
-    }
-    __syncthreads();
-    if (tid == 0) s_last = __hip_atomic_fetch_add(&ws[0], 1ull, __ATOMIC_ACQ_REL, __HIP_MEMORY_SCOPE_AGENT) == nb - 1;
-    __syncthreads();
-    if (s_last) {
-        for (uint32_t i = tid; i < nb * LANES; i += kScanBlock)
-            __hip_atomic_store(&state[i], 0ull, __ATOMIC_RELAXED, __HIP_MEMORY_SCOPE_AGENT);
-        if (tid == 0) {
-            __hip_atomic_store(&ws[0], 0ull, __ATOMIC_RELAXED, __HIP_MEMORY_SCOPE_AGENT);
-            __hip_atomic_store(&ws[1], 0ull, __ATOMIC_RELAXED, __HIP_MEMORY_SCOPE_AGENT);
-        }
-    }
-}
-
 template <class T>
 hipError_t launch(const T* in, uint32_t n, T* out, unsigned long long* ws, T* total, hipStream_t st) {
-    const uint32_t nb = std::max(1u, (n + kScanTile - 1) / kScanTile);
-    hipLaunchKernelGGL((k_scan<T>), dim3(nb), dim3(kScanBlock), 0, st, in, n, out, total, ws);
-    return hipGetLastError();
+    return launch_scan_map<T>(scanmap::LoadArray<T>{in}, n, scanmap::StoreArray<T>{out, total}, ws, st);
 }
 
 }
 
-size_t scan_ws_words(size_t n, uint32_t bytes_per_element) { return 4 + (n / kScanTile + 1) * (bytes_per_element / 4); }
+size_t scan_ws_words(size_t n, uint32_t bytes_per_element) { return 4 + (n / scanmap::kTile + 1) * (bytes_per_element / 4); }
 
 hipError_t launch_scan(const uint32_t* in, uint32_t n, uint32_t* out, unsigned long long* ws, uint32_t* total, hipStream_t st) {
     return launch<uint32_t>(in, n, out, ws, total, st);
diff --git a/line3dpp_amd/csrc/l3d_access.hip b/line3dpp_amd/csrc/l3d_access.hip
--- a/line3dpp_amd/csrc/l3d_access.hip
+++ b/line3dpp_amd/csrc/l3d_access.hip
@@ -158,6 +158,7 @@
     if (name && std::string(name) == "csr_global_launches") return g_csr_global_launches.load(std::memory_order_relaxed);
     if (name && std::string(name) == "knn_replay_calls") return g_knn_replay_calls.load(std::memory_order_relaxed);
     if (name && std::string(name) == "keep_all_repeats") return g_keep_all_repeats.load(std::memory_order_relaxed);
+    if (name && std::string(name) == "ordered_match_launches") return g_ordered_launches.load(std::memory_order_relaxed);
     if (name && std::string(name) == "lsd_images_detected") return g_lsd_images_detected.load(std::memory_order_relaxed);
     if (name && std::string(name) == "lsd_cache_loads") return g_lsd_cache_loads.load(std::memory_order_relaxed);
     return ~0ull;
diff --git a/line3dpp_amd/csrc/l3d_affinity_host.hip b/line3dpp_amd/csrc/l3d_affinity_host.hip
--- a/line3dpp_amd/csrc/l3d_affinity_host.hip
+++ b/line3dpp_amd/csrc/l3d_affinity_host.hip
@@ -136,7 +136,7 @@
     if (!(N > 0 && H > 0)) return L3D_OK;
     L3D_HIP_CHECK(launch_aff_sim(N, lo, hi, c->d_surv_sg.p, c->d_surv_tg.p, c->d_hyp_of_seg.p, c->d_hyps.p, c->d_vaff.p,
                                  (c->d_med + 8), (const float*)(c->d_vaff.p + V), c->two_sigA_sqr, c->d_simv.p, c->d_ca.p, c->d_cb.p,
-                                 c->stream));
+                                 c->d_first_touch.p, H, c->stream));
     return L3D_OK;
 }
 
@@ -154,25 +154,22 @@
             c->affinity_done = true;
             return L3D_OK;
         }
-        L3D_HIP_CHECK(c->d_touch_flag.reserve(2 * (size_t)N + 1));
-        L3D_HIP_CHECK(launch_aff_flag(N, c->d_surv_off.p, c->d_surv_sg.p, c->d_surv_tg.p, c->d_simv.p, c->d_ca.p,
-                                      c->d_cb.p, c->d_flag.p, c->d_first_touch.p, H, c->d_touch_flag.p, st));
-        L3D_HIP_CHECK(launch_scan(c->d_flag.p, N, c->d_epos.p, c->d_scan_ws.p, c->d_scal.p + 3, st));
-        {
-            L3D_HIP_CHECK(c->d_touch_flag.reserve(2 * (size_t)N + 1));
-            L3D_HIP_CHECK(c->d_touch_rank.reserve(2 * (size_t)N + 1));
-            L3D_HIP_CHECK(c->d_edges.reserve(2 * (size_t)N));
-            L3D_HIP_CHECK(c->d_l2g.reserve(H));
-            L3D_HIP_CHECK(launch_aff_touch(N, c->d_flag.p, c->d_epos.p, c->d_ca.p, c->d_cb.p, c->d_first_touch.p, st));
-            L3D_HIP_CHECK(launch_aff_mark(H, c->d_first_touch.p, c->d_touch_flag.p, st));
-            L3D_HIP_CHECK(launch_scan(c->d_touch_flag.p, 2 * N, c->d_touch_rank.p, c->d_scan_ws.p, c->d_scal.p + 4, st));
-            L3D_HIP_CHECK(launch_aff_emit(N, c->d_flag.p, c->d_epos.p, c->d_ca.p, c->d_cb.p, c->d_simv.p,
-                                          c->d_first_touch.p, c->d_touch_rank.p, c->d_hyps.p, c->d_edges.p,
-                                          c->d_l2g.p, st));
-            L3D_HIP_CHECK(c->h_cnt.reserve(16));
-            L3D_HIP_CHECK(hipMemcpyAsync(c->h_cnt.p + 12, c->d_scal.p + 3, 8, hipMemcpyDeviceToHost, st));
-            counts_pending = true;
-        }
+        L3D_HIP_CHECK(c->d_edge_cand.reserve(N));
+        L3D_HIP_CHECK(c->d_touch_rank.reserve(2 * (size_t)N + 1));
+        L3D_HIP_CHECK(c->d_edges.reserve(2 * (size_t)N));
+        L3D_HIP_CHECK(c->d_l2g.reserve(H));
+        L3D_HIP_CHECK(c->h_cnt.reserve(16));
+        void* h_dev = nullptr;
+        L3D_HIP_CHECK(hipHostGetDevicePointer(&h_dev, c->h_cnt.p, 0));
+        L3D_HIP_CHECK(launch_aff_edges(N, c->d_surv_off.p, c->d_surv_sg.p, c->d_surv_tg.p, c->d_simv.p, c->d_ca.p, c->d_cb.p,
+                                       c->d_flag.p, c->d_epos.p, c->d_edge_cand.p, c->d_first_touch.p, c->d_scal.p + 3,
+                                       c->d_scan_ws.p, st));
+        L3D_HIP_CHECK(launch_aff_rows(N, c->d_scal.p + 3, c->d_edge_cand.p, c->d_first_touch.p, c->d_ca.p, c->d_cb.p,
+                                      c->d_touch_rank.p, c->d_scal.p + 4, (uint32_t*)h_dev + 12, c->d_scan_ws.p, st));
+        L3D_HIP_CHECK(launch_aff_emit(N, c->d_flag.p, c->d_epos.p, c->d_ca.p, c->d_cb.p, c->d_simv.p,
+                                      c->d_first_touch.p, c->d_touch_rank.p, c->d_hyps.p, c->d_edges.p,
+                                      c->d_l2g.p, st));
+        counts_pending = true;
     }
     if (c->ev_on(7)) L3D_HIP_CHECK(hipEventRecord(c->ev[7], st));
     L3D_HIP_CHECK(hipStreamSynchronize(st));
diff --git a/line3dpp_amd/csrc/l3d_api.hip b/line3dpp_amd/csrc/l3d_api.hip
--- a/line3dpp_amd/csrc/l3d_api.hip
+++ b/line3dpp_amd/csrc/l3d_api.hip
@@ -276,6 +276,7 @@
     return ms;
 }
 std::atomic<uint64_t> g_keep_all_repeats{0};
+std::atomic<uint64_t> g_ordered_launches{0};
 std::atomic<uint64_t> g_knn_replay_calls{0};
 
 float ev_ms(const ::l3d_ctx* c, int a, int b) { return c->ev_on(a) && c->ev_on(b) ? ev_ms(c->ev[a], c->ev[b]) : 0.0f; }
@@ -348,7 +349,7 @@
     c->d_views.release(); c->d_pairs.release(); c->d_work.release(); c->d_slots.release(); c->d_slot_idx.release();
     c->h_views.release(); c->h_pairs.release(); c->h_cull.release(); c->h_work.release();
     c->h_segb.release(); c->h_cnt.release(); c->h_fin.release();
-    c->d_poff.release(); c->d_csr_dummy.release(); c->d_pair_present.release(); c->d_cnt64.release(); c->d_off64s.release(); c->d_scan_ws.release();
+    c->d_poff.release(); c->d_csr_dummy.release(); c->d_pair_present.release(); c->d_off64s.release(); c->d_scan_ws.release();
     c->d_huge_u64.release(); c->d_inv_refs.release(); c->d_lzero.release(); c->d_list2.release(); c->d_list4.release(); c->d_listH.release();
     c->d_seg_of_g.release(); c->d_huge_u32.release(); c->d_huge_f32.release(); c->d_ledges.release(); c->d_lhyps.release();
     c->d_lsegs.release(); c->d_lcands.release(); c->d_lchdrs.release(); c->d_ltab.release(); c->h_ltab.release();
@@ -366,7 +367,7 @@
     c->d_surv.release();
     c->d_hyp_of_seg.release(); c->d_depths.release(); c->d_med = nullptr; c->d_hyps.release();
     c->d_vaff.release(); c->d_simv.release(); c->h_vaff.release(); c->d_ca.release(); c->d_cb.release();
-    c->d_flag.release(); c->d_epos.release(); c->d_first_touch.release(); c->d_touch_flag.release();
+    c->d_flag.release(); c->d_epos.release(); c->d_first_touch.release(); c->d_edge_cand.release();
     c->d_touch_rank.release(); c->d_edges.release(); c->d_l2g.release();
     c->d_lopt.release(); c->h_lopt.release();
     for (auto& e : c->ev) if (e) (void)hipEventDestroy(e);
@@ -765,6 +766,7 @@
             pools.item_bucket = c->d_item_bucket.p; pools.item_order = c->d_item_order.p;
             pools.order_done = c->d_order_done.p;
             pools.w_base = c->cull[first].w_item0; pools.cost_max = maxMt;
+            l3d::g_ordered_launches.fetch_add(1, std::memory_order_relaxed);
         }
         L3D_HIP_CHECK(launch_cull_prepare(c->d_views.p, c->d_pairs.p, first, count, maxM, pools, layout, c->stream));
         L3D_HIP_CHECK(launch_order_items(c->d_pairs.p, first, count, maxMt, pools, (uint32_t)n_work, c->stream));
diff --git a/line3dpp_amd/csrc/l3d_ctx.h b/line3dpp_amd/csrc/l3d_ctx.h
--- a/line3dpp_amd/csrc/l3d_ctx.h
+++ b/line3dpp_amd/csrc/l3d_ctx.h
@@ -49,14 +49,14 @@
                              uint32_t* rb_host, uint32_t rb_words, uint32_t* rb_count, hipStream_t, uint32_t v0 = 0);
 hipError_t launch_aff_sim(uint32_t N, uint32_t lo, uint32_t hi, const uint32_t* surv_sg, const uint32_t* surv_tg, const int32_t* hyp_of_seg,
                           const HypRec*, const ViewAff*, const float* medians, const float* msdl, float two_sigA_sqr,
-                          float* simv, int32_t* ca, int32_t* cb, hipStream_t);
-hipError_t launch_aff_flag(uint32_t N, const uint32_t* surv_off, const uint32_t* surv_sg, const uint32_t* surv_tg,
-                           const float* simv, const int32_t* ca, const int32_t* cb, uint32_t* flag,
-                           uint32_t* first_touch, uint32_t H, uint32_t* touch_flag, hipStream_t);
-hipError_t launch_fill_u32(uint32_t*, uint32_t n, uint32_t val, hipStream_t);
-hipError_t launch_aff_touch(uint32_t N, const uint32_t* flag, const uint32_t* epos, const int32_t* ca,
-                            const int32_t* cb, uint32_t* first_touch, hipStream_t);
-hipError_t launch_aff_mark(uint32_t H, const uint32_t* first_touch, uint32_t* touch_flag, hipStream_t);
+                          float* simv, int32_t* ca, int32_t* cb, uint32_t* first_touch, uint32_t H, hipStream_t);
+hipError_t launch_aff_edges(uint32_t N, const uint32_t* surv_off, const uint32_t* surv_sg, const uint32_t* surv_tg,
+                            const float* simv, const int32_t* ca, const int32_t* cb, uint32_t* flag, uint32_t* epos,
+                            uint32_t* edge_cand, uint32_t* first_touch, uint32_t* n_edges, unsigned long long* ws,
+                            hipStream_t);
+hipError_t launch_aff_rows(uint32_t N, const uint32_t* n_edges, const uint32_t* edge_cand, const uint32_t* first_touch,
+                           const int32_t* ca, const int32_t* cb, uint32_t* touch_rank, uint32_t* n_rows,
+                           uint32_t* host_cnt, unsigned long long* ws, hipStream_t);
 hipError_t launch_aff_emit(uint32_t N, const uint32_t* flag, const uint32_t* epos, const int32_t* ca,
                            const int32_t* cb, const float* simv, const uint32_t* first_touch,
                            const uint32_t* touch_rank, const HypRec*, void* edges, void* local2global, hipStream_t);
@@ -199,7 +199,7 @@
     DevBuf<float> d_depths;
     float* d_med = nullptr;
     DevBuf<HypRec> d_hyps;
-    DevBuf<unsigned long long> d_cnt64, d_off64s, d_scan_ws, d_huge_u64;
+    DevBuf<unsigned long long> d_off64s, d_scan_ws, d_huge_u64;
     DevBuf<uint32_t> d_inv_refs;
     DevBuf<uint32_t> d_lzero, d_list2, d_list4, d_listH, d_seg_of_g, d_huge_u32;
     DevBuf<float> d_huge_f32;
@@ -234,7 +234,7 @@
     DevBuf<float> d_simv;
     PinnedBuf<ViewAff> h_vaff; UploadTag up_vaff;
     DevBuf<int32_t> d_ca, d_cb;
-    DevBuf<uint32_t> d_flag, d_epos, d_first_touch, d_touch_flag, d_touch_rank;
+    DevBuf<uint32_t> d_flag, d_epos, d_first_touch, d_edge_cand, d_touch_rank;
     DevBuf<l3d_cledge> d_edges;
     DevBuf<l3d_segment2d> d_l2g;
     std::vector<l3d_cledge> edges;
diff --git a/line3dpp_amd/csrc/l3d_kernels.h b/line3dpp_amd/csrc/l3d_kernels.h
--- a/line3dpp_amd/csrc/l3d_kernels.h
+++ b/line3dpp_amd/csrc/l3d_kernels.h
@@ -9,6 +9,7 @@
 
 extern std::atomic<uint64_t> g_knn_replay_calls;
 extern std::atomic<uint64_t> g_keep_all_repeats;
+extern std::atomic<uint64_t> g_ordered_launches;
 extern std::atomic<uint64_t> g_csr_global_launches;
 
 constexpr int kMatchRows = 64;
@@ -129,10 +130,12 @@
                               hipStream_t st);
 hipError_t launch_hyp_scores(ListPools lp, const uint8_t* positive, const uint32_t* gseg_view, Slot* slots,
                              const uint8_t* pair_present, uint32_t* max_score_bits, hipStream_t st);
-hipError_t launch_hyp_filter(ListPools lp, uint32_t g0, uint32_t g1, const uint32_t* gseg_view, const uint32_t* max_score_bits,
-                             uint32_t* kept_cnt, unsigned long long* best_pack, unsigned long long* cnt64,
-                             hipStream_t st);
-hipError_t launch_seg_write(uint32_t g0, uint32_t g1, unsigned long long base64, const ViewDev* views, const PairDesc* pairs, const uint32_t* seg_base,
+hipError_t launch_hyp_filter(ListPools lp, const uint32_t* gseg_view, const uint32_t* max_score_bits,
+                             uint32_t* kept_cnt, unsigned long long* best_pack, hipStream_t st);
+hipError_t launch_seg_offsets(ListPools lp, uint32_t g0, uint32_t g1, const uint32_t* kept_cnt, const unsigned long long* best_pack,
+                              unsigned long long* off64s, unsigned long long* total, unsigned long long* ws,
+                              uint32_t* surv_off, uint32_t* hyp_off, int32_t* hyp_of_seg, hipStream_t st);
+hipError_t launch_seg_write(bool segments, uint32_t g0, uint32_t g1, unsigned long long base64, const ViewDev* views, const PairDesc* pairs, const uint32_t* seg_base,
                             const uint32_t* gseg_view, const unsigned long long* off64s,
                             const unsigned long long* best_pack, const uint32_t* seg_of_g, ListPools lp,
                             const Slot* slots, uint32_t* surv_off, uint32_t* hyp_off, Match* surv, uint32_t* surv_tg,
diff --git a/line3dpp_amd/csrc/l3d_phase_b.hip b/line3dpp_amd/csrc/l3d_phase_b.hip
--- a/line3dpp_amd/csrc/l3d_phase_b.hip
+++ b/line3dpp_amd/csrc/l3d_phase_b.hip
@@ -175,7 +175,7 @@
     L3D_HIP_CHECK(c->d_seg_base.reserve(V + 1)); L3D_HIP_CHECK(c->d_gseg_view.reserve(G + 1));
     L3D_HIP_CHECK(c->d_surv_off.reserve(G + 2)); L3D_HIP_CHECK(c->d_hyp_off.reserve(G + 2));
     L3D_HIP_CHECK(c->d_hyp_of_seg.reserve(G + 1));
-    L3D_HIP_CHECK(c->d_cnt64.reserve(G + 2)); L3D_HIP_CHECK(c->d_off64s.reserve(G + 2));
+    L3D_HIP_CHECK(c->d_off64s.reserve(G + 2));
     L3D_HIP_CHECK(c->d_scan_ws.reserve_zeroed(scan_ws_words(G, 8), st));
     L3D_HIP_CHECK(c->d_seg_of_g.reserve(G + 1)); L3D_HIP_CHECK(c->d_list2.reserve(G + 1)); L3D_HIP_CHECK(c->d_list4.reserve(G + 1)); L3D_HIP_CHECK(c->d_listH.reserve(G + 1));
     L3D_HIP_CHECK(c->d_hyps.reserve(std::max<uint32_t>(G, 1))); L3D_HIP_CHECK(c->d_depths.reserve(2 * (size_t)G + 2));
@@ -321,7 +321,7 @@
 struct TailShard { uint32_t v0, v1, g0, g1, pool0, npools; };
 static TailShard whole_tail(const l3d_ctx* c) { return TailShard{0u, (uint32_t)c->order.size(), 0u, c->G, 0u, kListPools}; }
 
-static int tail_count_run(l3d_ctx* c, bool fresh, const TailShard& ts) {
+static int tail_count_run(l3d_ctx* c, bool fresh, const TailShard& ts, bool final_scan) {
     g_trace.mark("tail_run enter");
     hipStream_t st = c->stream;
     const uint32_t V = (uint32_t)c->order.size(), G = c->G;
@@ -349,20 +349,21 @@
     }
     L3D_HIP_CHECK(launch_hyp_scores(lps, positive_of(c), c->d_gseg_view.p, c->d_slots.p, present, max_score, st));
     g_trace.mark("hyp_scores enqueued");
-    L3D_HIP_CHECK(launch_hyp_filter(lps, ts.g0, ts.g1, c->d_gseg_view.p, max_score, kept, best, c->d_cnt64.p, st));
+    L3D_HIP_CHECK(launch_hyp_filter(lps, c->d_gseg_view.p, max_score, kept, best, st));
     g_trace.mark("hyp_filter enqueued");
-    L3D_HIP_CHECK(launch_scan64(c->d_cnt64.p + ts.g0, ts.g1 - ts.g0, c->d_off64s.p + ts.g0, c->d_scan_ws.p, tot64_of(c) + 1, st));
+    L3D_HIP_CHECK(launch_seg_offsets(lps, ts.g0, ts.g1, kept, best, c->d_off64s.p, tot64_of(c) + 1, c->d_scan_ws.p,
+                                     final_scan ? c->d_surv_off.p : nullptr, c->d_hyp_off.p, c->d_hyp_of_seg.p, st));
     g_trace.mark("scan enqueued");
     return L3D_OK;
 }
 
-static int tail_write_run(l3d_ctx* c, const TailShard& ts, unsigned long long base64, bool publish) {
+static int tail_write_run(l3d_ctx* c, const TailShard& ts, unsigned long long base64, bool publish, bool segments) {
     hipStream_t st = c->stream;
     const uint32_t V = (uint32_t)c->order.size(), G = c->G;
     const ZeroLayout z = zero_layout(V, G);
     const ListPools lps = list_pools(c, ts.pool0, ts.npools);
     unsigned long long* best = (unsigned long long*)(c->d_lzero.p + z.best);
-    L3D_HIP_CHECK(launch_seg_write(ts.g0, ts.g1, base64, c->d_views.p, c->d_pairs.p, c->d_seg_base.p, c->d_gseg_view.p,
+    L3D_HIP_CHECK(launch_seg_write(segments, ts.g0, ts.g1, base64, c->d_views.p, c->d_pairs.p, c->d_seg_base.p, c->d_gseg_view.p,
                                    c->d_off64s.p, best, c->d_seg_of_g.p, lps, c->d_slots.p, c->d_surv_off.p, c->d_hyp_off.p,
                                    c->d_surv.p, c->d_surv_tg.p, c->d_surv_sg.p, c->d_hyp_of_seg.p, c->d_hyps.p, c->d_depths.p, st));
     g_trace.mark("seg_write enqueued");
@@ -378,9 +379,9 @@
 
 static int tail_run(l3d_ctx* c, bool fresh) {
     const TailShard ts = whole_tail(c);
-    int rc = tail_count_run(c, fresh, ts);
+    int rc = tail_count_run(c, fresh, ts, true);
     if (rc) return rc;
-    rc = tail_write_run(c, ts, 0ull, true);
+    rc = tail_write_run(c, ts, 0ull, true, false);
     if (rc) return rc;
     if (c->ev_on(7)) L3D_HIP_CHECK(hipEventRecord(c->ev[7], c->stream));
     g_trace.mark("tail enqueued");
@@ -528,7 +529,7 @@
     hipStream_t st = c->stream;
     const uint32_t V = (uint32_t)c->order.size();
     auto run = [&](bool fresh) -> int {
-        const int rc = tail_count_run(c, fresh, ts);
+        const int rc = tail_count_run(c, fresh, ts, false);
         if (rc) return rc;
         L3D_HIP_CHECK(hipMemcpyAsync(c->h_fin.p, c->d_lzero.p, (kFinHead + fin_med(V)) * 4, hipMemcpyDeviceToHost, st));
         L3D_HIP_CHECK(hipStreamSynchronize(st));
@@ -609,7 +610,7 @@
         c->tail_base_n[world] = (uint32_t)n; c->tail_base_h[world] = (uint32_t)h;
         const uint32_t me = c->shard_rank;
         const TailShard ts{c->shard_v0, c->shard_v1, c->seg_base[c->shard_v0], c->seg_base[c->shard_v1], c->shard_pool0, c->shard_ppr};
-        const int r2 = tail_write_run(c, ts, (unsigned long long)c->tail_base_n[me] | ((unsigned long long)c->tail_base_h[me] << 32), false);
+        const int r2 = tail_write_run(c, ts, (unsigned long long)c->tail_base_n[me] | ((unsigned long long)c->tail_base_h[me] << 32), false, true);
         if (r2) return r2;
         if (!c->exch_ordered) L3D_HIP_CHECK(hipStreamSynchronize(c->stream));
         void* bp[9] = {c->d_surv.p, c->d_surv_tg.p, c->d_surv_sg.p, c->d_hyps.p, c->d_depths.p, c->d_surv_off.p, c->d_hyp_off.p,
diff --git a/line3dpp_amd/csrc/l3d_scan.h b/line3dpp_amd/csrc/l3d_scan.h
--- /dev/null
+++ b/line3dpp_amd/csrc/l3d_scan.h
@@ -0,0 +1,137 @@
+#pragma once
+#include <algorithm>
+#include "l3d_dev.h"
+
+namespace l3d {
+namespace scanmap {
+
+constexpr uint32_t kBlock = 1024, kItems = 4, kTile = kBlock * kItems;
+constexpr unsigned long long kAgg = 1ull << 32, kIncl = 2ull << 32;
+
+template <class T>
+__device__ __forceinline__ T block_exclusive_scan(T v, T* wsum , T& block_total) {
+    const uint32_t tid = threadIdx.x, lane = tid & 63u, wave = tid >> 6;
+    T x = v;
+#pragma unroll
+    for (int d = 1; d < 64; d <<= 1) {
+        const T y = __shfl_up(x, d);
+        if (lane >= (uint32_t)d) x += y;
+    }
+    if (lane == 63) wsum[wave] = x;
+    __syncthreads();
+    if (tid == 0) {
+        T acc = 0;
+        for (uint32_t w = 0; w < kBlock / 64; ++w) { const T t = wsum[w]; wsum[w] = acc; acc += t; }
+        wsum[16] = acc;
+    }
+    __syncthreads();
+    block_total = wsum[16];
+    return wsum[wave] + x - v;
+}
+
+__device__ __forceinline__ uint32_t wave_sum(uint32_t v) {
+#pragma unroll
+    for (int d = 32; d > 0; d >>= 1) v += __shfl_xor(v, d);
+    return v;
+}
+
+template <class T, class Load, class Store>
+__global__ __launch_bounds__(kBlock) void k_scan_map(const Load load, uint32_t n, const Store store,
+                                                     unsigned long long* __restrict__ ws) {
+    constexpr uint32_t LANES = sizeof(T) / 4;
+    __shared__ T wsum[17];
+    __shared__ T s_prefix;
+    __shared__ uint32_t s_last, s_tile;
+    const uint32_t nb = gridDim.x, tid = threadIdx.x, lane = tid & 63u;
+    if (tid == 0) s_tile = (uint32_t)__hip_atomic_fetch_add(&ws[1], 1ull, __ATOMIC_RELAXED, __HIP_MEMORY_SCOPE_AGENT);
+    __syncthreads();
+    const uint32_t tile = s_tile;
+    const uint32_t base = tile * kTile + tid * kItems;
+    T a[kItems];
+    T v = 0;
+#pragma unroll
+    for (uint32_t k = 0; k < kItems; ++k) { a[k] = (base + k < n) ? load(base + k) : (T)0; v += a[k]; }
+    T agg;
+    T ex = block_exclusive_scan(v, wsum, agg);
+    unsigned long long* state = ws + 2;
+    if (tid < 64) {
+        if (lane < LANES)
+            __hip_atomic_store(&state[(size_t)tile * LANES + lane],
+                               (tile == 0 ? kIncl : kAgg) | (uint32_t)((unsigned long long)agg >> (32 * lane)),
+                               __ATOMIC_RELAXED, __HIP_MEMORY_SCOPE_AGENT);
+        unsigned long long prefix = 0;
+        if (tile > 0) {
+#pragma unroll
+            for (uint32_t l = 0; l < LANES; ++l) {
+                uint32_t acc = 0;
+                for (int idx = (int)tile - 1;; idx -= 64) {
+                    const int t = idx - (int)lane;
+                    unsigned long long s = kIncl;
+                    if (t >= 0) {
+                        do s = __hip_atomic_load(&state[(size_t)t * LANES + l], __ATOMIC_RELAXED, __HIP_MEMORY_SCOPE_AGENT);
+                        while ((s >> 32) == 0);
+                    }
+                    const uint64_t incl = __builtin_amdgcn_ballot_w64((s >> 32) == 2);
+                    if (incl) {
+                        const uint32_t first = (uint32_t)__builtin_ctzll(incl);
+                        acc += wave_sum(lane <= first ? (uint32_t)s : 0u);
+                        break;
+                    }
+                    acc += wave_sum((uint32_t)s);
+                }
+                prefix |= (unsigned long long)acc << (32 * l);
+            }
+            if (lane < LANES)
+                __hip_atomic_store(&state[(size_t)tile * LANES + lane],
+                                   kIncl | (uint32_t)((prefix + (unsigned long long)agg) >> (32 * lane)),
+                                   __ATOMIC_RELAXED, __HIP_MEMORY_SCOPE_AGENT);
+        }
+        if (lane == 0) s_prefix = (T)prefix;
+    }
+    __syncthreads();
+    ex += s_prefix;
+#pragma unroll
+    for (uint32_t k = 0; k < kItems; ++k) {
+        if (base + k < n) store(base + k, ex, a[k]);
+        ex += a[k];
+    }
+    if (tile == nb - 1 && tid == 0) store.total(n, (T)(s_prefix + agg));
+    __syncthreads();
+    if (tid == 0) s_last = __hip_atomic_fetch_add(&ws[0], 1ull, __ATOMIC_ACQ_REL, __HIP_MEMORY_SCOPE_AGENT) == nb - 1;
+    __syncthreads();
+    if (s_last) {
+        for (uint32_t i = tid; i < nb * LANES; i += kBlock)
+            __hip_atomic_store(&state[i], 0ull, __ATOMIC_RELAXED, __HIP_MEMORY_SCOPE_AGENT);
+        if (tid == 0) {
+            __hip_atomic_store(&ws[0], 0ull, __ATOMIC_RELAXED, __HIP_MEMORY_SCOPE_AGENT);
+            __hip_atomic_store(&ws[1], 0ull, __ATOMIC_RELAXED, __HIP_MEMORY_SCOPE_AGENT);
+        }
+    }
+}
+
+template <class T>
+struct LoadArray {
+    const T* in;
+    __device__ __forceinline__ T operator()(uint32_t i) const { return in[i]; }
+};
+template <class T>
+struct StoreArray {
+    T* out;
+    T* total_out;
+    __device__ __forceinline__ void operator()(uint32_t i, T prefix, T) const { out[i] = prefix; }
+    __device__ __forceinline__ void total(uint32_t n, T total) const {
+        out[n] = total;
+        if (total_out) *total_out = total;
+    }
+};
+
+}
+
+template <class T, class Load, class Store>
+hipError_t launch_scan_map(const Load& load, uint32_t n, const Store& store, unsigned long long* ws, hipStream_t st) {
+    const uint32_t nb = std::max(1u, (n + scanmap::kTile - 1) / scanmap::kTile);
+    hipLaunchKernelGGL((scanmap::k_scan_map<T, Load, Store>), dim3(nb), dim3(scanmap::kBlock), 0, st, load, n, store, ws);
+    return hipGetLastError();
+}
+
+}
```

Result: slower. 973,700 (-1.8%).
